# Mamo1031/Multimodal-MTRSSM

Measured on AMD Instinct MI355X. Metric: seq-steps/s (BxT) MoPoE-MRSSM train step, higher is better.
Workload: dtype bf16x2-split, fp32 accumulate; 1 GPU; BASELINE configs[1]: MoPoE-MRSSM train step, B=64/GPU T=50 deter=200 stoch=30, vision 1x64x64 + audio 1x128x32 + action 4; global_batch=64, seq_len=50, parallelism=dp1, hidden=200, embed=256, categoricals_x_classes=6x5, residual_blocks=3, activation=ELU, optimizer=AdamW lr 1e-3 + clip 10 (fused HIP), params=4151600, streams=1, launch=eager (host enqueues every launch), backend=none, rccl_ranks=0, collective_ranks=0, noise=uniforms keyed by global batch row (parallel.GlobalRowNoise)

## Files before the change

include/mtrssm.h:

```cpp
#ifndef MTRSSM_H
#define MTRSSM_H

#include <stddef.h>
#include <stdint.h>

#ifdef __cplusplus
extern "C" {
#endif

#define MTRSSM_VERSION 100

#define MTRSSM_OK 0
#define MTRSSM_EINVAL (-1)
#define MTRSSM_ELAUNCH (-2)
#define MTRSSM_ELDS (-3)

#define MTRSSM_ACT_IDENTITY 0
#define MTRSSM_ACT_RELU 1
#define MTRSSM_ACT_ELU 2
#define MTRSSM_ACT_TANH 3

int mtrssm_version(void);
const char* mtrssm_last_error(void);
const char* mtrssm_last_kernel(void);
// ... 259 lines not shown
  float* d_lpl;
  float* d_la;
  float* d_lv;
  float* d_lph;
  float* d_lqh;
  const int32_t* modality;
} MtrssmMmtrssmBwdIO;

int mtrssm_mmtrssm_rollout_bwd(const MtrssmMmtrssmDims* dims, const MtrssmMmtrssmBwdWeights* w,
                               const MtrssmMmtrssmBwdIO* io, void* stream);

int mtrssm_mmtrssm_wide_supported(const MtrssmMmtrssmDims* dims, int32_t pieces);
int64_t mtrssm_mmtrssm_wide_workspace_bytes(const MtrssmMmtrssmDims* dims, int32_t pieces);
int64_t mtrssm_mmtrssm_wide_bwd_workspace_bytes(const MtrssmMmtrssmDims* dims, int32_t pieces);
int mtrssm_mmtrssm_rollout_fwd_wide(const MtrssmMmtrssmDims* dims, const MtrssmMmtrssmFwdWeights* w, const MtrssmMmtrssmFwdIO* io,
                                    int32_t pieces, void* workspace, int64_t workspace_bytes, void* stream);
int mtrssm_mmtrssm_rollout_bwd_wide(const MtrssmMmtrssmDims* dims, const MtrssmMmtrssmBwdWeights* w, const MtrssmMmtrssmBwdIO* io,
                                    int32_t pieces, void* workspace, int64_t workspace_bytes, void* stream);

typedef struct MtrssmConvGeom {
  int32_t N;
  int32_t C, Hs, Ws;
  int32_t C2;
  int32_t Cpad;
  int32_t KH, KW;
  int32_t SS, TS, OFFY, OFFX;
  int32_t Hq, Wq;
  int32_t OS, QY, QX;
  int32_t Ho, Wo;
  int32_t Cout, CoutPad;
  int32_t pre_act;
  int32_t act;
  int32_t mfma_split;
} MtrssmConvGeom;

int mtrssm_conv_gather_gemm(const MtrssmConvGeom* g, const float* src, const float* src2, const float* wp, const uint16_t* wq,
                            const float* bias, const float* actgrad_in, const float* add_in, float* out, void* stream);
int mtrssm_conv_gather_gemm_pair(const MtrssmConvGeom* ga, const float* srca, const float* src2a, const float* wpa, const uint16_t* wqa,
                                 const float* biasa, const float* actgrada, const float* adda, float* outa,
                                 const MtrssmConvGeom* gb, const float* srcb, const float* src2b, const float* wpb, const uint16_t* wqb,
                                 const float* biasb, const float* actgradb, const float* addb, float* outb, void* stream);
int mtrssm_conv_gather_pair_merges(const MtrssmConvGeom* ga, const MtrssmConvGeom* gb, int32_t has_wq);
int mtrssm_residual_block_fwd_supported(const MtrssmConvGeom* g3);
int mtrssm_residual_block_fwd(const MtrssmConvGeom* ga, const float* xa, const uint16_t* wq3a, const float* b3a, const float* w1a,
                              const float* b1a, float* ha, float* ya, const MtrssmConvGeom* gb, const float* xb, const uint16_t* wq3b,
                              const float* b3b, const float* w1b, const float* b1b, float* hb, float* yb, void* stream);
int mtrssm_pack_conv_weight(const float* w, int32_t O, int32_t I, int32_t KH, int32_t KW, int64_t so, int64_t si, int64_t sh,
                            int64_t sw, int32_t OPad, int32_t IPad, int32_t pieces, float* wp, uint16_t* wq, void* stream);
#define MTRSSM_PACK_DESC_WORDS 16
int mtrssm_pack_conv_weights(const int64_t* table, int32_t count, int32_t blocks_per_weight, void* stream);
int mtrssm_conv_weight_grad(const MtrssmConvGeom* g, const float* a, const float* src, const float* src2,
                            int32_t pre_act_a, float* dwp, float* dbias, void* workspace, int64_t workspace_bytes, void* stream);
int mtrssm_conv_weight_grad_deferred(const MtrssmConvGeom* g, const float* a, const float* src, const float* src2,
                                     int32_t pre_act_a, float* dwp, float* dbias, void* workspace, int64_t workspace_bytes, void* stream);
int mtrssm_conv_weight_grad_reduce(void* stream);
int mtrssm_conv_weight_grad_src_bias_supported(const MtrssmConvGeom* g, int32_t pre_act_a);
int mtrssm_residual_bwd1x1_supported(const MtrssmConvGeom* g);
int mtrssm_residual_bwd1x1(const MtrssmConvGeom* g, const float* gy, const float* h, const uint16_t* wq1t, float* gh, float* dwp,
                           float* dbias, void* workspace, int64_t workspace_bytes, int32_t defer, void* stream);
int mtrssm_conv_weight_grad_src_bias(const MtrssmConvGeom* g, const float* a, const float* src, int32_t pre_act_a, float* dwp,
                                     float* dsrc_bias, void* workspace, int64_t workspace_bytes, int32_t defer, void* stream);
int64_t mtrssm_conv_weight_grad_workspace_bytes(const MtrssmConvGeom* g, int32_t pre_act_a);
int mtrssm_unpack_conv_grads(const int64_t* table, int32_t count, int32_t blocks_per_entry, void* stream);
int mtrssm_convt_quad_supported(const MtrssmConvGeom* g4);
int mtrssm_convt_quad(const MtrssmConvGeom* ga4, const float* srca, const uint16_t* const* wqa4, const float* biasa, const float* actgrada,
                      float* outa, const MtrssmConvGeom* gb4, const float* srcb, const uint16_t* const* wqb4, const float* biasb,
                      const float* actgradb, float* outb, void* stream);
int mtrssm_convt_k4s2_thin(int32_t N, int32_t C, int32_t Hs, int32_t Ws, int32_t Cout, const float* src, const float* w,
                           const float* bias, int32_t pre_act, int32_t act, float* out, void* stream);
int mtrssm_convt_k4s2_band_supported(int32_t N, int32_t C, int32_t Hs, int32_t Ws, int32_t Cout);
int mtrssm_convt_k4s2_band(int32_t N, int32_t C, int32_t Hs, int32_t Ws, int32_t Cout, const float* src, const float* w,
                           const float* bias, int32_t pre_act, int32_t act, float* out, void* stream);
int mtrssm_conv_tgather_thin(int32_t N, int32_t O, int32_t Hs, int32_t Ws, int32_t Cout, int32_t KH, int32_t KW, int32_t stride, int32_t pad,
                             int32_t Ho, int32_t Wo, const float* y, const float* w, const float* bias, int32_t pre_act, int32_t act,
                             const float* actgrad_in, const float* add_in, float* out, void* stream);
int mtrssm_channel_sum(const float* x, int32_t N, int32_t C, int32_t HW, float* out, void* stream);

int mtrssm_episode_gather(const float* store, const int64_t* idx, const float* noise, int64_t n_episodes, int64_t B, int64_t T,
                          int64_t Tfull, int64_t E, float std_, float* input, float* target, void* stream);
int mtrssm_episode_gather_window(const float* store, const int64_t* idx, const int32_t* start, const float* noise, int64_t n_episodes,
                                 int64_t B, int64_t T, int64_t Tfull, int64_t E, float std_, float* input, float* target, void* stream);
int mtrssm_episode_gather_ragged(const float* store, const int64_t* idx, const int32_t* start, const int32_t* lengths, const float* noise,
                                 int64_t n_episodes, int64_t B, int64_t T, int64_t Tfull, int64_t E, float std_, float* input, float* target,
                                 int32_t* valid_out, void* stream);
int mtrssm_episode_gather_seeded(const float* store, const int64_t* idx, const int32_t* start, const int32_t* lengths, int32_t* valid_out,
                                 uint32_t key0, uint32_t key1, uint32_t epoch, int64_t n_episodes, int64_t B, int64_t T, int64_t Tfull,
                                 int64_t E, float std_, float* input, float* target, void* stream);

#define MTRSSM_STATE_MAX 6
typedef struct MtrssmStateTable {
  int32_t count;
  int32_t width[MTRSSM_STATE_MAX];
// ... 73 lines not shown
```

multimodal_mtrssm_amd/_lib.py:

```python

from __future__ import annotations

import ctypes as C
import os
from pathlib import Path

import torch
from torch import Tensor

_HERE = Path(__file__).resolve().parent
LIB_PATH = _HERE / "libmtrssm_hip.so"

ACT_IDS = {"Identity": 0, "ReLU": 1, "ELU": 2, "Tanh": 3}

_f = C.c_float
_i = C.c_int32
_p = C.c_void_p


def _struct(name: str, fields: list[tuple[str, type]]) -> type:
    return type(name, (C.Structure,), {"_fields_": fields})


def _ptrs(*names: str) -> list[tuple[str, type]]:
# ... 14 lines not shown
    "w1s_t", "wf_t", "bf", "whh_t", "bhh", "wh1_t", "b3", "w4", "b4", "wa2", "ba2", "wv2", "bv2"))
MrssmBwdWeights = _struct("MtrssmMrssmBwdWeights", _ptrs("w1s_t", "w2", "wih", "whh", "wh1", "w4", "wa2", "wv2"))
MrssmBwdIO = _struct("MtrssmMrssmBwdIO", _ptrs(
    "deter0", "deter", "prior_logits", "post_logits", "sv_h1", "sv_h2", "sv_gates", "sv_heads", "sv_la", "sv_lv",
    "g_deter", "g_post_stoch", "g_prior_stoch", "g_post_logits", "g_prior_logits", "g_kl",
    "g_deter0", "g_stoch0", "d_z1", "d_h2", "d_gi", "d_gh", "d_zh", "d_lp", "d_la", "d_lv", "modality"))

MmtrssmDims = _struct("MtrssmMmtrssmDims", [
    ("B", _i), ("T", _i), ("LD", _i), ("HD", _i), ("H", _i), ("KL", _i), ("CL", _i), ("KH", _i), ("CH", _i),
    ("act", _i), ("post", _i), ("tau_l", _f), ("tau_h", _f), ("keep_l", _f), ("keep_h", _f),
    ("kl_w_post", _f), ("kl_w_prior", _f), ("rows_per_block", _i), ("threads", _i),
])
MmtrssmFwdWeights = _struct("MtrssmMmtrssmFwdWeights", _ptrs(
    "wxl_s_t", "wdl_t", "wxh_t", "wdh_t", "bh", "wl1_t", "bl1", "wh1_t", "bh1",
    "wlp2", "blp2", "wa2", "ba2", "wv2", "bv2", "whp2", "bhp2", "whq2", "bhq2"))
MmtrssmFwdIO = _struct("MtrssmMmtrssmFwdIO", _ptrs(
    "xl", "pa", "pv", "deter_l0", "deter_h0", "hidden_l0", "hidden_h0", "stoch_l0", "stoch_h0",
    "u_post_l", "u_post_h", "u_prior_l", "u_prior_h",
    "deter_l", "deter_h", "hidden_l", "hidden_h", "prior_logits_l", "prior_logits_h", "prior_stoch_l", "prior_stoch_h",
    "post_logits_l", "post_logits_h", "post_stoch_l", "post_stoch_h", "kl_l", "kl_h",
    "sv_l1", "sv_h1", "sv_la", "sv_lv", "modality"))
MmtrssmBwdWeights = _struct("MtrssmMmtrssmBwdWeights", _ptrs(
    "wxl_s_t", "wdl", "wxh_t", "wdh", "wl1", "wh1", "wlp2", "wa2", "wv2", "whp2", "whq2"))
MmtrssmBwdIO = _struct("MtrssmMmtrssmBwdIO", _ptrs(
    "deter_l0", "deter_h0", "deter_l", "deter_h", "prior_logits_l", "prior_logits_h", "post_logits_l", "post_logits_h",
    "sv_l1", "sv_h1", "sv_la", "sv_lv",
    "g_deter_l", "g_deter_h", "g_hidden_l", "g_hidden_h", "g_post_stoch_l", "g_post_stoch_h", "g_prior_stoch_l",
    "g_prior_stoch_h", "g_post_logits_l", "g_post_logits_h", "g_prior_logits_l", "g_prior_logits_h", "g_kl_l", "g_kl_h",
    "g_deter_l0", "g_deter_h0", "g_hidden_l0", "g_hidden_h0", "g_stoch_l0", "g_stoch_h0",
    "d_ul", "d_uh", "d_zl1", "d_zh1", "d_lpl", "d_la", "d_lv", "d_lph", "d_lqh", "modality"))

ConvGeom = _struct("MtrssmConvGeom", [(n, _i) for n in (
    "N", "C", "Hs", "Ws", "C2", "Cpad", "KH", "KW", "SS", "TS", "OFFY", "OFFX", "Hq", "Wq", "OS", "QY", "QX", "Ho", "Wo",
    "Cout", "CoutPad", "pre_act", "act", "mfma_split")])

Gemm = _struct("MtrssmGemm", _ptrs("A", "B", "C", "bias", "zgrad", "colsum") + [(n, _i) for n in (
    "M", "N", "R", "lda", "ldb", "ldc", "ldz", "a_rmajor", "b_rmajor", "act_a", "act_b", "act_out", "act_z", "accumulate", "split_r")]
    + [("tickets", _p), ("n_tickets", _i), ("mfma_split", _i)])

STATE_MAX = 6
StateTable = _struct("MtrssmStateTable", [
    ("count", _i), ("width", _i * STATE_MAX), ("src_stride", C.c_int64 * STATE_MAX), ("src", _p * STATE_MAX), ("alt", _p * STATE_MAX),
    ("dst", _p * STATE_MAX)])

SYMBOLS: dict[str, tuple[type | None, list[type]]] = {
    "mtrssm_version": (C.c_int, []),
    "mtrssm_last_error": (C.c_char_p, []),
    "mtrssm_last_kernel": (C.c_char_p, []),
    "mtrssm_mrssm_rollout_fwd": (C.c_int, [C.POINTER(MrssmDims), C.POINTER(MrssmFwdWeights), C.POINTER(MrssmFwdIO), _p]),
    "mtrssm_mrssm_cluster_supported": (C.c_int, [C.POINTER(MrssmDims)]),
    "mtrssm_mrssm_cluster_workspace_bytes": (C.c_int64, [C.POINTER(MrssmDims)]),
    "mtrssm_mrssm_rollout_fwd_cluster": (C.c_int, [C.POINTER(MrssmDims), C.POINTER(MrssmClusterWeights), C.POINTER(MrssmFwdIO), _p, C.c_int64, _p]),
    "mtrssm_mrssm_cluster_bwd_workspace_bytes": (C.c_int64, [C.POINTER(MrssmDims)]),
    "mtrssm_mrssm_rollout_bwd_cluster": (C.c_int, [C.POINTER(MrssmDims), C.POINTER(MrssmClusterWeights), C.POINTER(MrssmBwdIO), _p, C.c_int64, _p]),
    "mtrssm_mrssm_wide_supported": (C.c_int, [C.POINTER(MrssmDims), _i]),
    "mtrssm_mrssm_wide_workspace_bytes": (C.c_int64, [C.POINTER(MrssmDims), _i]),
    "mtrssm_mrssm_wide_bwd_workspace_bytes": (C.c_int64, [C.POINTER(MrssmDims), _i]),
    "mtrssm_mrssm_rollout_fwd_wide": (C.c_int, [C.POINTER(MrssmDims), C.POINTER(MrssmClusterWeights), C.POINTER(MrssmFwdIO), _i, _p, C.c_int64, _p]),
    "mtrssm_mrssm_rollout_bwd_wide": (C.c_int, [C.POINTER(MrssmDims), C.POINTER(MrssmClusterWeights), C.POINTER(MrssmBwdIO), _i, _p, C.c_int64, _p]),
    "mtrssm_mrssm_rollout_bwd": (C.c_int, [C.POINTER(MrssmDims), C.POINTER(MrssmBwdWeights), C.POINTER(MrssmBwdIO), _p]),
    "mtrssm_mmtrssm_rollout_fwd": (C.c_int, [C.POINTER(MmtrssmDims), C.POINTER(MmtrssmFwdWeights), C.POINTER(MmtrssmFwdIO), _p]),
    "mtrssm_mmtrssm_rollout_bwd": (C.c_int, [C.POINTER(MmtrssmDims), C.POINTER(MmtrssmBwdWeights), C.POINTER(MmtrssmBwdIO), _p]),
    "mtrssm_mmtrssm_wide_supported": (C.c_int, [C.POINTER(MmtrssmDims), _i]),
    "mtrssm_mmtrssm_wide_workspace_bytes": (C.c_int64, [C.POINTER(MmtrssmDims), _i]),
    "mtrssm_mmtrssm_wide_bwd_workspace_bytes": (C.c_int64, [C.POINTER(MmtrssmDims), _i]),
    "mtrssm_mmtrssm_rollout_fwd_wide": (C.c_int, [C.POINTER(MmtrssmDims), C.POINTER(MmtrssmFwdWeights), C.POINTER(MmtrssmFwdIO), _i, _p, C.c_int64, _p]),
    "mtrssm_mmtrssm_rollout_bwd_wide": (C.c_int, [C.POINTER(MmtrssmDims), C.POINTER(MmtrssmBwdWeights), C.POINTER(MmtrssmBwdIO), _i, _p, C.c_int64, _p]),
    "mtrssm_conv_gather_gemm": (C.c_int, [C.POINTER(ConvGeom), _p, _p, _p, _p, _p, _p, _p, _p, _p]),
    "mtrssm_conv_gather_gemm_pair": (C.c_int, [C.POINTER(ConvGeom), _p, _p, _p, _p, _p, _p, _p, _p,
                                               C.POINTER(ConvGeom), _p, _p, _p, _p, _p, _p, _p, _p, _p]),
    "mtrssm_conv_gather_pair_merges": (C.c_int, [C.POINTER(ConvGeom), C.POINTER(ConvGeom), _i]),
    "mtrssm_residual_block_fwd_supported": (C.c_int, [C.POINTER(ConvGeom)]),
    "mtrssm_residual_block_fwd": (C.c_int, [C.POINTER(ConvGeom), _p, _p, _p, _p, _p, _p, _p, C.POINTER(ConvGeom), _p, _p, _p, _p, _p, _p, _p, _p]),
    "mtrssm_pack_conv_weight": (C.c_int, [_p, _i, _i, _i, _i, C.c_int64, C.c_int64, C.c_int64, C.c_int64, _i, _i, _i, _p, _p, _p]),
    "mtrssm_pack_conv_weights": (C.c_int, [_p, _i, _i, _p]),
    "mtrssm_unpack_conv_grads": (C.c_int, [_p, _i, _i, _p]),
    "mtrssm_conv_weight_grad": (C.c_int, [C.POINTER(ConvGeom), _p, _p, _p, _i, _p, _p, _p, C.c_int64, _p]),
    "mtrssm_conv_weight_grad_deferred": (C.c_int, [C.POINTER(ConvGeom), _p, _p, _p, _i, _p, _p, _p, C.c_int64, _p]),
    "mtrssm_residual_bwd1x1_supported": (C.c_int, [C.POINTER(ConvGeom)]),
    "mtrssm_residual_bwd1x1": (C.c_int, [C.POINTER(ConvGeom), _p, _p, _p, _p, _p, _p, _p, C.c_int64, _i, _p]),
    "mtrssm_conv_weight_grad_src_bias_supported": (C.c_int, [C.POINTER(ConvGeom), _i]),
    "mtrssm_conv_weight_grad_src_bias": (C.c_int, [C.POINTER(ConvGeom), _p, _p, _i, _p, _p, _p, C.c_int64, _i, _p]),
    "mtrssm_conv_weight_grad_reduce": (C.c_int, [_p]),
    "mtrssm_conv_weight_grad_workspace_bytes": (C.c_int64, [C.POINTER(ConvGeom), _i]),
    "mtrssm_channel_sum": (C.c_int, [_p, _i, _i, _i, _p, _p]),
    "mtrssm_convt_k4s2_thin": (C.c_int, [_i, _i, _i, _i, _i, _p, _p, _p, _i, _i, _p, _p]),
    "mtrssm_convt_k4s2_band_supported": (C.c_int, [_i, _i, _i, _i, _i]),
    "mtrssm_convt_k4s2_band": (C.c_int, [_i, _i, _i, _i, _i, _p, _p, _p, _i, _i, _p, _p]),
    "mtrssm_convt_quad_supported": (C.c_int, [C.POINTER(ConvGeom)]),
    "mtrssm_convt_quad": (C.c_int, [C.POINTER(ConvGeom), _p, C.POINTER(C.c_void_p), _p, _p, _p, C.POINTER(ConvGeom), _p, C.POINTER(C.c_void_p),
                                    _p, _p, _p, _p]),
    "mtrssm_conv_tgather_thin": (C.c_int, [_i] * 11 + [_p, _p, _p, _i, _i, _p, _p, _p, _p]),
    "mtrssm_episode_gather": (C.c_int, [_p, _p, _p, C.c_int64, C.c_int64, C.c_int64, C.c_int64, C.c_int64, _f, _p, _p, _p]),
    "mtrssm_episode_gather_window": (C.c_int, [_p, _p, _p, _p, C.c_int64, C.c_int64, C.c_int64, C.c_int64, C.c_int64, _f, _p, _p, _p]),
    "mtrssm_state_select": (C.c_int, [C.POINTER(StateTable), _p, C.c_int64, _p]),
    "mtrssm_state_save": (C.c_int, [C.POINTER(StateTable), C.c_int64, C.c_int64, _p]),
    "mtrssm_state_save_at": (C.c_int, [C.POINTER(StateTable), _p, C.c_int64, C.c_int64, _p]),
    "mtrssm_episode_gather_ragged": (C.c_int, [_p, _p, _p, _p, _p, C.c_int64, C.c_int64, C.c_int64, C.c_int64, C.c_int64, _f, _p, _p, _p, _p]),
    "mtrssm_episode_gather_seeded": (C.c_int, [_p, _p, _p, _p, _p, C.c_uint32, C.c_uint32, C.c_uint32, C.c_int64, C.c_int64, C.c_int64, C.c_int64,
                                               C.c_int64, _f, _p, _p, _p]),
    "mtrssm_step_mask_ragged": (C.c_int, [_p, _p, C.c_int64, C.c_int64, C.c_int64, _f, _f, C.c_int64, C.c_int64, _p, _p, _p, _p, _p, _p, _p, _p]),
    "mtrssm_elbo_combine_counted_fwd": (C.c_int, [_p, _p, _p, _p, _p, _p, C.c_int64, C.c_float, C.c_float, _p, _p, _p, _p, _p]),
    "mtrssm_elbo_combine_counted_bwd": (C.c_int, [_p, _p, _p, _p, _p, _p, C.c_int64, C.c_float, C.c_float, _p, _p, _p, _p, _p]),
    "mtrssm_elbo_combine_fwd": (C.c_int, [_p, _p, _p, _p, C.c_int64, C.c_float, C.c_float, _p, _p, _p, _p, _p]),
    "mtrssm_elbo_combine_bwd": (C.c_int, [_p, _p, _p, _p, C.c_int64, C.c_float, C.c_float, _p, _p, _p, _p, _p]),
    "mtrssm_categorical_sample_fwd": (C.c_int, [_p, _p, C.c_int64, _i, _i, _p, _p, _p, _p]),
    "mtrssm_categorical_sample_bwd": (C.c_int, [_p, _p, _p, C.c_int64, _i, _i, _p, _p]),
    "mtrssm_gaussian_nll_fwd": (C.c_int, [_p, _p, C.c_int64, C.c_int64, _i, _p, _p]),
    "mtrssm_gaussian_nll_bwd": (C.c_int, [_p, _p, _p, C.c_int64, C.c_int64, _i, _p, _p]),
    "mtrssm_gaussian_nll_masked_fwd": (C.c_int, [_p, _p, _p, _p, C.c_int64, C.c_int64, _i, _p, _p]),
    "mtrssm_gaussian_nll_masked_bwd": (C.c_int, [_p, _p, _p, _p, _p, C.c_int64, C.c_int64, _i, _p, _p]),
    "mtrssm_modality_dropout": (C.c_int, [_p, C.c_int64, C.c_int64, C.c_int64, _f, _f, C.c_int64, C.c_int64, _p, _p, _p, _p, _p, _p]),
    "mtrssm_sumsq": (C.c_int, [_p, C.c_int64, _p, _p]),
# ... 128 lines not shown
```

multimodal_mtrssm_amd/conv.py:

```python

from __future__ import annotations

import ctypes as C
import os
import weakref

import torch
from torch import Tensor

from multimodal_mtrssm_amd import _lib
from multimodal_mtrssm_amd.linear import grad_target, grad_target_owner


def _pad_to(n: int, m: int) -> int:
    return (n + m - 1) // m * m


def _pads(cout: int, cin: int) -> tuple[int, int]:
    return _pad_to(cout, 64 if cout > 32 else 32), _pad_to(cin, 16)


_PACK_BUFFERS: dict[tuple, tuple[Tensor, Tensor | None]] = {}

PAIR_LAUNCH = os.environ.get("MTRSSM_PAIR_LAUNCH", "1") != "0"
# ... 130 lines not shown
def gemm_pieces() -> int:
    return {0: 0, 3: 3, 2: 2, 1: 2}[_MFMA_SPLIT]


def _geom(**kw: int) -> C.Structure:
    g = _lib.ConvGeom()
    for k, v in kw.items():
        setattr(g, k, int(v))
    g.mfma_split = _MFMA_SPLIT
    return g


def _gather_gemm(geom: C.Structure, src: Tensor, src2: Tensor | None, wpq: tuple[Tensor, Tensor | None], bias: Tensor | None,
                 actgrad_in: Tensor | None, out: Tensor, add_in: Tensor | None = None) -> None:
    wp, wq = wpq
    lib = _lib.load()
    job = (geom, src, src2, wp, wq, bias, actgrad_in, add_in, out)
    if _DEFER is not None:
        _DEFER.append(job)
        return
    _launch_gather(job)


def _job_work(job: tuple) -> tuple[float, float]:
    geom, actgrad_in, add_in = job[0], job[6], job[7]
    pixels = geom.N * geom.Hq * geom.Wq
    flops = 2.0 * pixels * geom.Cout * geom.KH * geom.KW * (geom.C + geom.C2)
    nbytes = 4.0 * (geom.N * geom.C * geom.Hs * geom.Ws + pixels * geom.Cout * (1 + (actgrad_in is not None) + (add_in is not None)))
    return flops, nbytes


def _job_args(job: tuple) -> tuple:
    geom, src, src2, wp, wq, bias, actgrad_in, add_in, out = job
    return (C.byref(geom), _lib.ptr(src), _lib.ptr(src2), _lib.ptr(wp), _lib.raw_ptr(wq), _lib.ptr(bias), _lib.ptr(actgrad_in),
            _lib.ptr(add_in), _lib.ptr(out))


def _quad_args(job: tuple) -> tuple:
    _, geoms, y, wqs, bias, out, actgrad = job
    arr = (C.c_void_p * 4)(*[_lib.raw_ptr(wq) for wq in wqs])
    return (geoms, _lib.ptr(y), arr, _lib.ptr(bias), _lib.ptr(actgrad), _lib.ptr(out))


def _quad_work(job: tuple) -> tuple[float, float]:
    g = job[1][0]
    pixels = g.N * g.Ho * g.Wo
    return 2.0 * pixels * g.Cout * 4 * g.C, 4.0 * (g.N * g.C * g.Hs * g.Ws + pixels * g.Cout * (2 if job[6] is not None else 1))


def _launch_quad(ja: tuple, jb: tuple | None) -> None:
    lib = _lib.load()
    fa, ba = _quad_work(ja)
    fb, bb = _quad_work(jb) if jb is not None else (0.0, 0.0)
    args_b = _quad_args(jb) if jb is not None else (None, None, None, None, None, None)
    _lib.check(_lib.TIMERS.call("mtrssm_convt_quad", lib.mtrssm_convt_quad, *_quad_args(ja), *args_b, _lib.stream_ptr(ja[2].device),
                                flops=fa + fb, nbytes=ba + bb), "mtrssm_convt_quad")


def _launch_gather(job: tuple) -> None:
    if job[0] == "quad":
        _launch_quad(job, None)
        return
    lib = _lib.load()
    flops, nbytes = _job_work(job)
    _lib.check(_lib.TIMERS.call("mtrssm_conv_gather_gemm", lib.mtrssm_conv_gather_gemm, *_job_args(job),
                                _lib.stream_ptr(job[1].device), flops=flops, nbytes=nbytes), "mtrssm_conv_gather_gemm")

# ... 25 lines not shown
                _launch_gather(jb)
            continue
        if not lib.mtrssm_conv_gather_pair_merges(C.byref(ja[0]), C.byref(jb[0]), int(ja[4] is not None and jb[4] is not None)):
            _launch_gather(ja)
            _launch_gather(jb)
            continue
        fa, ba = _job_work(ja)
        fb, bb = _job_work(jb)
        _lib.check(_lib.TIMERS.call("mtrssm_conv_gather_gemm_pair", lib.mtrssm_conv_gather_gemm_pair, *_job_args(ja), *_job_args(jb),
                                    _lib.stream_ptr(ja[1].device), flops=fa + fb, nbytes=ba + bb), "mtrssm_conv_gather_gemm_pair")
    return ra, rb


def _conv_forward_gather(x: Tensor, coords: Tensor | None, w: Tensor, bias: Tensor | None, stride: int, pad: int,
                         pre_act: bool, act: int, actgrad_in: Tensor | None = None, add_in: Tensor | None = None) -> Tensor:
    n, c, hs, ws = x.shape
    o, i, kh, kw = w.shape
    c2 = 0 if coords is None else coords.shape[0]
    if i != c + c2:
        msg = f"weight expects {i} input channels, got {c}+{c2}"
        raise ValueError(msg)
    ho = (hs + 2 * pad - kh) // stride + 1
    wo = (ws + 2 * pad - kw) // stride + 1
    wpq = pack_weight(w)
    wp = wpq[0]
    out = torch.empty(n, o, ho, wo, device=x.device, dtype=torch.float32)
    geom = _geom(N=n, C=c, Hs=hs, Ws=ws, C2=c2, Cpad=wp.shape[2], KH=kh, KW=kw, SS=stride, TS=1, OFFY=-pad, OFFX=-pad,
                 Hq=ho, Wq=wo, OS=1, QY=0, QX=0, Ho=ho, Wo=wo, Cout=o, CoutPad=wp.shape[0], pre_act=int(pre_act), act=act)
    _gather_gemm(geom, x, coords, wpq, bias, actgrad_in, out, add_in)
    return out


def _conv_transposed_gather(y: Tensor, w: Tensor, bias: Tensor | None, stride: int, pad: int, out_hw: tuple[int, int],
                            pre_act: bool, act: int, actgrad_in: Tensor | None = None, add_in: Tensor | None = None) -> Tensor:
    n, o, hs, ws = y.shape
    o2, c, kh, kw = w.shape
    if o2 != o:
        msg = f"weight expects {o2} gathered channels, got {o}"
        raise ValueError(msg)
    ho, wo = out_hw
    out = torch.empty(n, c, ho, wo, device=y.device, dtype=torch.float32)
    if (stride == 2 and kh == 4 and kw == 4 and pad == 1 and c <= 2 and (ho, wo) == (2 * hs, 2 * ws) and actgrad_in is None
            and add_in is None and o * ((8 + 2) * (32 + 2) + 1) * 4 <= 64 * 1024):
        lib = _lib.load()
        wc = w.contiguous()
        if _MFMA_SPLIT == 2 and CONVT_BAND and lib.mtrssm_convt_k4s2_band_supported(n, o, hs, ws, c):
            _lib.check(_lib.TIMERS.call(
                "mtrssm_convt_k4s2_band", lib.mtrssm_convt_k4s2_band, n, o, hs, ws, c, _lib.ptr(y), _lib.ptr(wc), _lib.ptr(bias),
                int(pre_act), act, _lib.ptr(out), _lib.stream_ptr(y.device), flops=2.0 * n * ho * wo * c * 4 * o,
                nbytes=4.0 * (y.numel() + out.numel())), "mtrssm_convt_k4s2_band")
            return out
        _lib.check(_lib.TIMERS.call(
            "mtrssm_convt_k4s2_thin", lib.mtrssm_convt_k4s2_thin, n, o, hs, ws, c, _lib.ptr(y), _lib.ptr(wc), _lib.ptr(bias),
            int(pre_act), act, _lib.ptr(out), _lib.stream_ptr(y.device), flops=2.0 * n * ho * wo * c * 4 * o,
            nbytes=4.0 * (y.numel() + out.numel())), "mtrssm_convt_k4s2_thin")
        return out
    quad_fwd = kh == 4 and kw == 4 and actgrad_in is None and (o, c, hs * ws) in ((64, 32, 64), (32, 16, 256))
    quad_bwd = (CONVT_QUAD_BWD and kh == 3 and kw == 3 and actgrad_in is not None and bias is None
                and (o, c, hs * ws) in ((32, 16, 64), (16, 8, 256)))
    if (stride == 2 and pad == 1 and (ho, wo) == (2 * hs, 2 * ws) and add_in is None and _MFMA_SPLIT == 2 and CONVT_QUAD
            and (quad_fwd or quad_bwd)):
        geoms = (_lib.ConvGeom * 4)()
        wqs = []
        for q in range(4):
            qy, qx = q >> 1, q & 1
            ky0, kx0 = (qy + pad) % stride, (qx + pad) % stride
            wsub = w[:, :, ky0::stride, kx0::stride].permute(1, 0, 2, 3)
            wp, wq = pack_weight(wsub, sub=q, grid=(2, 2))
            geoms[q] = _geom(N=n, C=o, Hs=hs, Ws=ws, C2=0, Cpad=wp.shape[2], KH=2, KW=2, SS=1, TS=-1,
                             OFFY=(qy + pad - ky0) // stride, OFFX=(qx + pad - kx0) // stride, Hq=hs, Wq=ws, OS=stride, QY=qy, QX=qx,
                             Ho=ho, Wo=wo, Cout=c, CoutPad=wp.shape[0], pre_act=int(pre_act), act=act)
            wqs.append(wq)
        if _lib.load().mtrssm_convt_quad_supported(geoms):
            job = ("quad", geoms, y, wqs, bias, out, actgrad_in)
            if _DEFER is not None:
                _DEFER.append(job)
            else:
                _launch_gather(job)
            return out
    if stride == 2 and c <= 8 and kh * kw * o <= 256 and ho % 2 == 0 and wo % 2 == 0 and TGATHER_THIN:
        lib = _lib.load()
        wc = w.contiguous()
        taps_used = kh * kw / (stride * stride)
        _lib.check(_lib.TIMERS.call(
            "mtrssm_conv_tgather_thin", lib.mtrssm_conv_tgather_thin, n, o, hs, ws, c, kh, kw, stride, pad, ho, wo, _lib.ptr(y),
            _lib.ptr(wc), _lib.ptr(bias), int(pre_act), act, _lib.ptr(actgrad_in), _lib.ptr(add_in), _lib.ptr(out),
            _lib.stream_ptr(y.device), flops=2.0 * n * ho * wo * c * taps_used * o,
            nbytes=4.0 * (y.numel() + out.numel() * (1 + (actgrad_in is not None) + (add_in is not None)))), "mtrssm_conv_tgather_thin")
        return out
    for qy in range(min(stride, ho)):
        ky0 = (qy + pad) % stride
        for qx in range(min(stride, wo)):
            kx0 = (qx + pad) % stride
            wsub = w[:, :, ky0::stride, kx0::stride].permute(1, 0, 2, 3)
            wpq = pack_weight(wsub)
            wp = wpq[0]
            geom = _geom(N=n, C=o, Hs=hs, Ws=ws, C2=0, Cpad=wp.shape[2], KH=wsub.shape[2], KW=wsub.shape[3], SS=1, TS=-1,
                         OFFY=(qy + pad - ky0) // stride, OFFX=(qx + pad - kx0) // stride,
                         Hq=(ho - qy + stride - 1) // stride, Wq=(wo - qx + stride - 1) // stride, OS=stride, QY=qy, QX=qx,
                         Ho=ho, Wo=wo, Cout=c, CoutPad=wp.shape[0], pre_act=int(pre_act), act=act)
            _gather_gemm(geom, y, None, wpq, bias, actgrad_in, out, add_in)
    return out


TGATHER_THIN = os.environ.get("MTRSSM_TGATHER_THIN", "1") != "0"
CONVT_QUAD = os.environ.get("MTRSSM_CONVT_QUAD", "1") != "0"
CONVT_QUAD_BWD = os.environ.get("MTRSSM_CONVT_QUAD_BWD", "1") != "0"
CONVT_BAND = os.environ.get("MTRSSM_CONVT_BAND", "1") != "0"
_ZERO_CHUNK_FLOATS = 2 << 20
_ZERO_CHUNKS: dict[tuple, list] = {}


def _zeros(n: int, device: torch.device) -> Tensor:
    need = (n + 63) // 64 * 64
    key = (device, torch.cuda.current_stream(device).cuda_stream if device.type == "cuda" else 0)
    st = _ZERO_CHUNKS.get(key)
    if st is None or st[1] + need > st[0].numel():
        st = _ZERO_CHUNKS[key] = [torch.zeros(max(_ZERO_CHUNK_FLOATS, need), device=device, dtype=torch.float32), 0]
    out = st[0][st[1] : st[1] + n]
    st[1] += need
    return out


class _ConvGradSink:

    def __init__(self) -> None:
        self.entries: dict[tuple, tuple] = {}
        self.table: Tensor | None = None
        self.retired: list[Tensor] = []
        self.pending = False

    def target(self, weight: Tensor | None, o: int, i: int, taps: int, opad: int, ipad: int) -> Tensor | None:
        if weight is None or not weight.is_contiguous():
# ... 78 lines not shown
            _WGRAD_SLOT_NEXT[(device, stream)] = 0
            _lib.check(_lib.TIMERS.call("mtrssm_conv_weight_grad_reduce", _lib.load().mtrssm_conv_weight_grad_reduce, C.c_void_p(stream)),
                       "mtrssm_conv_weight_grad_reduce")


def _wgrad_workspace(geom: C.Structure, pre_act_a: int, device: torch.device, *, own: bool = False) -> Tensor | None:
    gkey = (tuple(getattr(geom, n) for n, _ in geom._fields_), pre_act_a)
    need = _WGRAD_NEED.get(gkey)
    if need is None:
        need = _WGRAD_NEED[gkey] = max(0, int(_lib.load().mtrssm_conv_weight_grad_workspace_bytes(C.byref(geom), pre_act_a)))
    if need == 0:
        return None
    key = (device, torch.cuda.current_stream(device).cuda_stream)
    if own:
        slots = _WGRAD_SLOTS.setdefault(key, [])
        k = _WGRAD_SLOT_NEXT.get(key, 0)
        _WGRAD_SLOT_NEXT[key] = k + 1
        if k == len(slots):
            slots.append(torch.empty((need + 3) // 4 + 64, device=device, dtype=torch.float32))
        elif slots[k].numel() * 4 < need:
            _WGRAD_WS_RETIRED.append(slots[k])
            slots[k] = torch.empty((need + 3) // 4 + 64, device=device, dtype=torch.float32)
        return slots[k]
    ws = _WGRAD_WS.get(key)
    if ws is None or ws.numel() * 4 < need:
        if ws is not None:
            _WGRAD_WS_RETIRED.append(ws)
        ws = _WGRAD_WS[key] = torch.empty((need + 3) // 4 + 64, device=device, dtype=torch.float32)
    return ws


def _weight_grad(a: Tensor, src: Tensor, coords: Tensor | None, kh: int, kw: int, stride: int, pad: int, pre_act_a: bool,
                 pre_act_src: bool, act: int, *, want_bias: bool = False, weight: Tensor | None = None,
                 bias: Tensor | None = None, want_src_bias: bool = False) -> tuple[Tensor | None, Tensor | None]:
    lib = _lib.load()
    n, o, hq, wq = a.shape
    _, c, hs, ws = src.shape
    c2 = 0 if coords is None else coords.shape[0]
    opad, ipad = _pads(o, c + c2)
    sunk = _GRAD_SINK.target(weight, o, c + c2, kh * kw, opad, ipad)
    dwp = sunk if sunk is not None else _zeros(opad * kh * kw * ipad, a.device).view(opad, kh * kw, ipad)
    fuse_src_bias = want_src_bias and CONVT_BIAS_FUSE and coords is None and a.data_ptr() % 16 == 0 and src.data_ptr() % 16 == 0
    dbias = bias_sunk = None
    if want_bias or fuse_src_bias:
        bias_sunk = grad_target(bias) if bias is not None and bias.is_contiguous() else None
    geom = _geom(N=n, C=c, Hs=hs, Ws=ws, C2=c2, Cpad=ipad, KH=kh, KW=kw, SS=stride, TS=1, OFFY=-pad, OFFX=-pad, Hq=hq, Wq=wq,
                 OS=1, QY=0, QX=0, Ho=hq, Wo=wq, Cout=o, CoutPad=opad, pre_act=int(pre_act_src), act=act)
    flops = 2.0 * n * hq * wq * o * kh * kw * (c + c2)
    nbytes = 4.0 * (a.numel() + src.numel())
    fuse_src_bias = fuse_src_bias and bool(lib.mtrssm_conv_weight_grad_src_bias_supported(C.byref(geom), int(pre_act_a)))
    if want_bias or fuse_src_bias:
        dbias = bias_sunk if bias_sunk is not None else _zeros(c if fuse_src_bias else o, a.device)
    defer = DEFER_WGRAD_REDUCE and sunk is not None and (dbias is None or bias_sunk is not None)
    ws = _wgrad_workspace(geom, int(pre_act_a), a.device, own=defer)
    if fuse_src_bias:
        _lib.check(_lib.TIMERS.call(
            "mtrssm_conv_weight_grad", lib.mtrssm_conv_weight_grad_src_bias, C.byref(geom), _lib.ptr(a), _lib.ptr(src), int(pre_act_a),
            _lib.ptr(dwp), _lib.ptr(dbias), _lib.raw_ptr(ws), 0 if ws is None else ws.numel() * 4, int(defer and ws is not None),
            _lib.stream_ptr(a.device), flops=flops, nbytes=nbytes), "mtrssm_conv_weight_grad_src_bias")
        g_w = None if sunk is not None else dwp[:o, :, : c + c2].reshape(o, kh, kw, c + c2).permute(0, 3, 1, 2)
        return g_w, (None if bias_sunk is not None else dbias)
    entry = lib.mtrssm_conv_weight_grad_deferred if defer and ws is not None else lib.mtrssm_conv_weight_grad
    _lib.check(_lib.TIMERS.call(
        "mtrssm_conv_weight_grad", entry, C.byref(geom), _lib.ptr(a), _lib.ptr(src), _lib.ptr(coords),
        int(pre_act_a), _lib.ptr(dwp), _lib.ptr(dbias), _lib.raw_ptr(ws), 0 if ws is None else ws.numel() * 4, _lib.stream_ptr(a.device),
        flops=flops, nbytes=nbytes), "mtrssm_conv_weight_grad")
    g_w = None if sunk is not None else dwp[:o, :, : c + c2].reshape(o, kh, kw, c + c2).permute(0, 3, 1, 2)
    if want_src_bias:
        return g_w, _channel_sum(src, bias)
    return g_w, (None if bias_sunk is not None else dbias)


def _channel_sum(x: Tensor, bias: Tensor | None = None) -> Tensor | None:
    lib = _lib.load()
    n, c, h, w = x.shape
    sunk = grad_target(bias) if bias is not None and bias.is_contiguous() else None
    out = sunk if sunk is not None else _zeros(c, x.device)
    _lib.check(_lib.TIMERS.call("mtrssm_channel_sum", lib.mtrssm_channel_sum, _lib.ptr(x), n, c, h * w, _lib.ptr(out),
                                _lib.stream_ptr(x.device)), "mtrssm_channel_sum")
    return None if sunk is not None else out


class _Conv2d(torch.autograd.Function):
    @staticmethod
    def forward(ctx, x, weight, bias, coords, stride, pad, pre_act, act):
        x, weight = x.contiguous(), weight.contiguous()
        bias = None if bias is None else bias.contiguous()
        coords = None if coords is None else coords.contiguous()
        out = _conv_forward_gather(x, coords, weight, bias, stride, pad, pre_act, act)
        ctx.save_for_backward(x, weight, coords if coords is not None else x.new_zeros(0))
        ctx.cfg = (stride, pad, pre_act, act, coords is not None, bias is not None)
        ctx.bias = bias
        return out

    @staticmethod
    def backward(ctx, g_out):
        x, weight, coords = ctx.saved_tensors
# ... 74 lines not shown
        g = job[0]
        pixels = g.N * g.Hq * g.Wq
        return 2.0 * pixels * g.Cout * (9 * g.C + g.C), 4.0 * pixels * (2 * g.C + g.Cout)

    def args(job: tuple | None) -> tuple:
        if job is None:
            return (None,) * 8
        geom, x, wq, b3, w1, b1, h, y = job
        return (C.byref(geom), _lib.ptr(x), _lib.raw_ptr(wq), _lib.ptr(b3), _lib.ptr(w1), _lib.ptr(b1), _lib.ptr(h), _lib.ptr(y))

    fa, ba = work(ja)
    fb, bb = work(jb) if jb is not None else (0.0, 0.0)
    lib = _lib.load()
    _lib.check(_lib.TIMERS.call("mtrssm_residual_block_fwd", lib.mtrssm_residual_block_fwd, *args(ja), *args(jb),
                                _lib.stream_ptr(ja[1].device), flops=fa + fb, nbytes=ba + bb), "mtrssm_residual_block_fwd")


RESBLOCK_BWD1X1_FUSE = True


def _bwd1x1_geom(g_y: Tensor, h: Tensor, w1: Tensor, act: int) -> C.Structure | None:
    if not RESBLOCK_BWD1X1_FUSE or _MFMA_SPLIT != 2 or w1.shape[2:] != (1, 1) or not g_y.is_cuda:
        return None
    n, o, hq, wq = g_y.shape
    c = h.shape[1]
    if w1.shape[:2] != (o, c) or h.shape != (n, c, hq, wq) or g_y.data_ptr() % 16 or h.data_ptr() % 16:
        return None
    opad, ipad = _pads(o, c)
    geom = _geom(N=n, C=c, Hs=hq, Ws=wq, C2=0, Cpad=ipad, KH=1, KW=1, SS=1, TS=1, OFFY=0, OFFX=0, Hq=hq, Wq=wq, OS=1, QY=0, QX=0,
                 Ho=hq, Wo=wq, Cout=o, CoutPad=opad, pre_act=1, act=act)
    return geom if _lib.load().mtrssm_residual_bwd1x1_supported(C.byref(geom)) else None


def _bwd1x1_fused(geom: C.Structure, g_y: Tensor, h: Tensor, w1: Tensor, b1: Tensor) -> tuple[Tensor, Tensor | None, Tensor | None]:
    lib = _lib.load()
    n, o, hq, wq = g_y.shape
    c = h.shape[1]
    _, wq1t = pack_weight(w1.permute(1, 0, 2, 3))
    sunk = _GRAD_SINK.target(w1, o, c, 1, geom.CoutPad, geom.Cpad)
    dwp = sunk if sunk is not None else _zeros(geom.CoutPad * geom.Cpad, g_y.device).view(geom.CoutPad, 1, geom.Cpad)
    bias_sunk = grad_target(b1) if b1.is_contiguous() else None
    dbias = bias_sunk if bias_sunk is not None else _zeros(o, g_y.device)
    defer = DEFER_WGRAD_REDUCE and sunk is not None and bias_sunk is not None
    ws = _wgrad_workspace(geom, 0, g_y.device, own=defer)
    g_h = torch.empty_like(h)
    pixels = n * hq * wq
    _lib.check(_lib.TIMERS.call(
        "mtrssm_residual_bwd1x1", lib.mtrssm_residual_bwd1x1, C.byref(geom), _lib.ptr(g_y), _lib.ptr(h), _lib.raw_ptr(wq1t), _lib.ptr(g_h),
        _lib.ptr(dwp), _lib.ptr(dbias), _lib.raw_ptr(ws), 0 if ws is None else ws.numel() * 4, int(defer and ws is not None),
        _lib.stream_ptr(g_y.device), flops=2.0 * 2.0 * pixels * o * c, nbytes=4.0 * (g_y.numel() + 2 * h.numel())), "mtrssm_residual_bwd1x1")
    g_w = None if sunk is not None else dwp[:o, :, :c].reshape(o, 1, 1, c).permute(0, 3, 1, 2)
    return g_h, g_w, (None if bias_sunk is not None else dbias)


class _ResidualBlock(torch.autograd.Function):

    @staticmethod
    def forward(ctx, x, w3, b3, w1, b1, act):
        x, w3, b3, w1, b1 = (t.contiguous() for t in (x, w3, b3, w1, b1))
        p3, p1 = w3.shape[2] // 2, w1.shape[2] // 2
        job = _residual_job(x, w3, b3, w1, b1, act)
        if job is not None:
            _residual_launch(job, None)
            h, y = job[6], job[7]
        else:
            h = _conv_forward_gather(x, None, w3, b3, 1, p3, True, act)
            y = _conv_forward_gather(h, None, w1, b1, 1, p1, True, act, add_in=x)
        ctx.save_for_backward(x, h, w3, w1)
        ctx.act, ctx.biases = act, (b3, b1)
        return y

    @staticmethod
    def backward(ctx, g_y):
        x, h, w3, w1 = ctx.saved_tensors
        act = ctx.act
        g_y = g_y.contiguous()
        p3, p1 = w3.shape[2] // 2, w1.shape[2] // 2
        b3, b1 = ctx.biases
        g1 = _bwd1x1_geom(g_y, h, w1, act)
        if g1 is not None:
            g_h, g_w1, g_b1 = _bwd1x1_fused(g1, g_y, h, w1, b1)
        else:
            g_h = _conv_transposed_gather(g_y, w1, None, 1, p1, (h.shape[2], h.shape[3]), False, act, actgrad_in=h)
            g_w1, g_b1 = _weight_grad(g_y, h, None, w1.shape[2], w1.shape[3], 1, p1, False, True, act, want_bias=True, weight=w1, bias=b1)
        g_x = None
        if ctx.needs_input_grad[0]:
            g_x = _conv_transposed_gather(g_h, w3, None, 1, p3, (x.shape[2], x.shape[3]), False, act, actgrad_in=x, add_in=g_y)
        g_w3, g_b3 = _weight_grad(g_h, x, None, w3.shape[2], w3.shape[3], 1, p3, False, True, act, want_bias=True, weight=w3, bias=b3)
        return g_x, g_w3, g_b3, g_w1, g_b1, None


class _PairResidualBlock(torch.autograd.Function):

    @staticmethod
    def forward(ctx, xa, w3a, b3a, w1a, b1a, xv, w3v, b3v, w1v, b1v, act):
        xa, w3a, b3a, w1a, b1a, xv, w3v, b3v, w1v, b1v = (t.contiguous() for t in (xa, w3a, b3a, w1a, b1a, xv, w3v, b3v, w1v, b1v))
        p3, p1 = w3a.shape[2] // 2, w1a.shape[2] // 2
        ja = _residual_job(xa, w3a, b3a, w1a, b1a, act)
        jv = _residual_job(xv, w3v, b3v, w1v, b1v, act, sub=1) if ja is not None else None
        if ja is not None and jv is not None:
            _residual_launch(ja, jv)
            ha, ya, hv, yv = ja[6], ja[7], jv[6], jv[7]
        else:
            ha, hv = paired(lambda: _conv_forward_gather(xa, None, w3a, b3a, 1, p3, True, act),
                            lambda: _conv_forward_gather(xv, None, w3v, b3v, 1, p3, True, act))
            ya, yv = paired(lambda: _conv_forward_gather(ha, None, w1a, b1a, 1, p1, True, act, add_in=xa),
                            lambda: _conv_forward_gather(hv, None, w1v, b1v, 1, p1, True, act, add_in=xv))
        ctx.save_for_backward(xa, ha, w3a, w1a, xv, hv, w3v, w1v)
        ctx.act, ctx.biases = act, (b3a, b1a, b3v, b1v)
        return ya, yv

    @staticmethod
    def backward(ctx, g_ya, g_yv):
        xa, ha, w3a, w1a, xv, hv, w3v, w1v = ctx.saved_tensors
        act = ctx.act
        g_ya, g_yv = g_ya.contiguous(), g_yv.contiguous()
        p3, p1 = w3a.shape[2] // 2, w1a.shape[2] // 2
        b3a, b1a, b3v, b1v = ctx.biases
        g1a = _bwd1x1_geom(g_ya, ha, w1a, act)
        g1v = _bwd1x1_geom(g_yv, hv, w1v, act) if g1a is not None else None
        if g1a is not None and g1v is not None:
            g_ha, g_w1a, g_b1a = _bwd1x1_fused(g1a, g_ya, ha, w1a, b1a)
            g_hv, g_w1v, g_b1v = _bwd1x1_fused(g1v, g_yv, hv, w1v, b1v)
        else:
            g_ha, g_hv = paired(lambda: _conv_transposed_gather(g_ya, w1a, None, 1, p1, (ha.shape[2], ha.shape[3]), False, act, actgrad_in=ha),
                                lambda: _conv_transposed_gather(g_yv, w1v, None, 1, p1, (hv.shape[2], hv.shape[3]), False, act, actgrad_in=hv))
            g_w1a, g_b1a = _weight_grad(g_ya, ha, None, w1a.shape[2], w1a.shape[3], 1, p1, False, True, act, want_bias=True, weight=w1a, bias=b1a)
            g_w1v, g_b1v = _weight_grad(g_yv, hv, None, w1v.shape[2], w1v.shape[3], 1, p1, False, True, act, want_bias=True, weight=w1v, bias=b1v)
        g_xa, g_xv = paired(
            lambda: _conv_transposed_gather(g_ha, w3a, None, 1, p3, (xa.shape[2], xa.shape[3]), False, act, actgrad_in=xa, add_in=g_ya),
            lambda: _conv_transposed_gather(g_hv, w3v, None, 1, p3, (xv.shape[2], xv.shape[3]), False, act, actgrad_in=xv, add_in=g_yv))
        g_w3a, g_b3a = _weight_grad(g_ha, xa, None, w3a.shape[2], w3a.shape[3], 1, p3, False, True, act, want_bias=True, weight=w3a, bias=b3a)
        g_w3v, g_b3v = _weight_grad(g_hv, xv, None, w3v.shape[2], w3v.shape[3], 1, p3, False, True, act, want_bias=True, weight=w3v, bias=b3v)
        return g_xa, g_w3a, g_b3a, g_w1a, g_b1a, g_xv, g_w3v, g_b3v, g_w1v, g_b1v, None


def residual_block_pair(xa: Tensor, pa: tuple[Tensor, Tensor, Tensor, Tensor], xv: Tensor, pv: tuple[Tensor, Tensor, Tensor, Tensor],
                        *, act: int) -> tuple[Tensor, Tensor]:
    return _PairResidualBlock.apply(xa, *pa, xv, *pv, int(act))


def residual_block(x: Tensor, w3: Tensor, b3: Tensor, w1: Tensor, b1: Tensor, *, act: int) -> Tensor:
    return _ResidualBlock.apply(x, w3, b3, w1, b1, int(act))


class _BranchCtx:

    def __init__(self, needs: tuple = ()) -> None:
        self.needs_input_grad = needs
        self.saved_tensors: tuple = ()
        self.cfg: tuple = ()

    def save_for_backward(self, *tensors: Tensor) -> None:
        self.saved_tensors = tensors


def _pair_function(base: type) -> type:

    class _Pair(torch.autograd.Function):
        @staticmethod
        def forward(ctx, n, *args):
            ca, cb = _BranchCtx(), _BranchCtx()
            ya, yb = paired(lambda: base.forward(ca, *args[:n]), lambda: base.forward(cb, *args[n:]))
            ctx.n, ctx.na, ctx.cfgs = n, len(ca.saved_tensors), (ca.cfg, cb.cfg)
            ctx.biases = (getattr(ca, "bias", None), getattr(cb, "bias", None))
            ctx.save_for_backward(*ca.saved_tensors, *cb.saved_tensors)
# ... 41 lines not shown
```

multimodal_mtrssm_amd/csrc/capi.hip:

```cpp
#include <stdarg.h>
#include <stdio.h>

#include "scan_common.h"

namespace mtrssm {

static thread_local char g_err[512] = "";
static thread_local const char* g_kernel = "";

void set_last_kernel(const char* name) { g_kernel = name; }

void set_error(const char* fmt, ...) {
  va_list ap;
  va_start(ap, fmt);
  vsnprintf(g_err, sizeof(g_err), fmt, ap);
  va_end(ap);
}

int mrssm_fwd_launch(const MtrssmMrssmDims*, const MtrssmMrssmFwdWeights*, const MtrssmMrssmFwdIO*, hipStream_t);
int mrssm_bwd_launch(const MtrssmMrssmDims*, const MtrssmMrssmBwdWeights*, const MtrssmMrssmBwdIO*, hipStream_t);
int mmtrssm_fwd_launch(const MtrssmMmtrssmDims*, const MtrssmMmtrssmFwdWeights*, const MtrssmMmtrssmFwdIO*, hipStream_t);
int mmtrssm_bwd_launch(const MtrssmMmtrssmDims*, const MtrssmMmtrssmBwdWeights*, const MtrssmMmtrssmBwdIO*, hipStream_t);
int conv_gather_gemm_launch(const MtrssmConvGeom*, const float*, const float*, const float*, const unsigned short*, const float*, const float*, const float*, float*, hipStream_t);
int episode_gather_launch(const float*, const int64_t*, const float*, int64_t, int64_t, int64_t, int64_t, int64_t, float, float*, float*, hipStream_t);
int episode_gather_window_launch(const float*, const int64_t*, const int32_t*, const float*, int64_t, int64_t, int64_t, int64_t, int64_t, float, float*,
                                 float*, hipStream_t);
int state_select_launch(const MtrssmStateTable*, const unsigned char*, int64_t, hipStream_t);
int state_save_launch(const MtrssmStateTable*, int64_t, int64_t, hipStream_t);
int state_save_at_launch(const MtrssmStateTable*, const int32_t*, int64_t, int64_t, hipStream_t);
int episode_gather_ragged_launch(const float*, const int64_t*, const int32_t*, const int32_t*, const float*, int64_t, int64_t, int64_t, int64_t,
                                 int64_t, float, float*, float*, int32_t*, hipStream_t);
int episode_gather_seeded_launch(const float*, const int64_t*, const int32_t*, const int32_t*, int32_t*, uint32_t, uint32_t, uint32_t, int64_t, int64_t,
                                 int64_t, int64_t, int64_t, float, float*, float*, hipStream_t);
int step_mask_ragged_launch(const int32_t*, const float*, int64_t, int64_t, int64_t, float, float, int64_t, int64_t, int32_t*, float*, float*, float*,
                            unsigned char*, int32_t*, float*, hipStream_t);
int elbo_combine_counted_fwd_launch(const float*, const float*, const float*, const float*, const float*, const float*, int64_t, float, float, float*,
                                    float*, float*, float*, hipStream_t);
int elbo_combine_counted_bwd_launch(const float*, const float*, const float*, const float*, const float*, const float*, int64_t, float, float, float*,
                                    float*, float*, float*, hipStream_t);
int conv_gather_gemm_pair_launch(const MtrssmConvGeom*, const float*, const float*, const float*, const unsigned short*, const float*, const float*, const float*, float*,
                                 const MtrssmConvGeom*, const float*, const float*, const float*, const unsigned short*, const float*, const float*, const float*, float*, hipStream_t);
int conv_residual_fwd_supported(const MtrssmConvGeom*);
int conv_residual_fwd_launch(const MtrssmConvGeom*, const float*, const unsigned short*, const float*, const float*, const float*, float*, float*,
                             const MtrssmConvGeom*, const float*, const unsigned short*, const float*, const float*, const float*, float*, float*, hipStream_t);
int pack_conv_weight_launch(const float*, int, int, int, int, long, long, long, long, int, int, int, float*, unsigned short*, hipStream_t);
int pack_conv_weights_launch(const int64_t*, int, int, hipStream_t);
int conv_gather_pair_merges(const MtrssmConvGeom*, const MtrssmConvGeom*, bool);
int conv_weight_grad_launch(const MtrssmConvGeom*, const float*, const float*, const float*, int, float*, float*, void*, size_t, size_t*, hipStream_t);
int conv_weight_grad_deferred_launch(const MtrssmConvGeom*, const float*, const float*, const float*, int, float*, float*, void*, size_t, hipStream_t);
int conv_weight_grad_reduce_flush(hipStream_t);
int conv_residual_bwd1x1_supported(const MtrssmConvGeom*);
int conv_residual_bwd1x1_launch(const MtrssmConvGeom*, const float*, const float*, const unsigned short*, float*, float*, float*, void*, size_t, int,
                                hipStream_t);
int conv_weight_grad_src_bias_supported(const MtrssmConvGeom*, int);
int conv_weight_grad_src_bias_launch(const MtrssmConvGeom*, const float*, const float*, int, float*, float*, void*, size_t, int, hipStream_t);
int channel_sum_launch(const float*, int, int, int, float*, hipStream_t);
int convt_k4s2_band_supported(int, int, int, int, int);
int convt_k4s2_band_launch(int, int, int, int, int, const float*, const float*, const float*, int, int, float*, hipStream_t);
int convt_k4s2_thin_launch(int, int, int, int, int, const float*, const float*, const float*, int, int, float*, hipStream_t);
int conv_convt_quad_supported(const MtrssmConvGeom*);
int conv_convt_quad_launch(const MtrssmConvGeom*, const float*, const unsigned short* const*, const float*, const float*, float*,
                           const MtrssmConvGeom*, const float*, const unsigned short* const*, const float*, const float*, float*, hipStream_t);
int conv_tgather_thin_launch(int, int, int, int, int, int, int, int, int, int, int, const float*, const float*, const float*, int, int, const float*,
                             const float*, float*, hipStream_t);
int categorical_sample_fwd_launch(const float*, const float*, int64_t, int, int, float*, float*, float*, hipStream_t);
int categorical_sample_bwd_launch(const float*, const float*, const float*, int64_t, int, int, float*, hipStream_t);
int elbo_combine_fwd_launch(const float*, const float*, const float*, const float*, int64_t, float, float, float*, float*, float*, float*, hipStream_t);
int elbo_combine_bwd_launch(const float*, const float*, const float*, const float*, int64_t, float, float, float*, float*, float*, float*, hipStream_t);
int nll_fwd_launch(const float*, const float*, int64_t, int64_t, int, float*, hipStream_t);
int nll_bwd_launch(const float*, const float*, const float*, int64_t, int64_t, int, float*, hipStream_t);
int nll_masked_fwd_launch(const float*, const float*, const float*, const float*, int64_t, int64_t, int, float*, hipStream_t);
int nll_masked_bwd_launch(const float*, const float*, const float*, const float*, const float*, int64_t, int64_t, int, float*, hipStream_t);
int modality_dropout_launch(const float*, int64_t, int64_t, int64_t, float, float, int64_t, int64_t, int32_t*, float*, float*, unsigned char*, float*,
                            hipStream_t);
int sumsq_launch(const float*, int64_t, float*, hipStream_t);
int adamw_launch(float*, const float*, float*, float*, int64_t, const float*, float, float, float, float, float, float, float, int, hipStream_t);
int gemm_launch(const MtrssmGemm*, hipStream_t);
int gemm_group_launch(const MtrssmGemm*, int, hipStream_t);
int debug_set_cluster_profile(void*);
int debug_set_resident_profile(void*);
int debug_set_wide_profile(void*);
int debug_set_mmt_profile(void*);
int mrssm_cluster_supported(const MtrssmMrssmDims*);
size_t mrssm_cluster_workspace_bytes(const MtrssmMrssmDims*);
size_t mrssm_cluster_bwd_workspace_bytes(const MtrssmMrssmDims*);
// ... 212 lines not shown
                                            const float* biasb, const float* actgradb, const float* addb, float* outb, void* stream) {
  return conv_gather_gemm_pair_launch(ga, srca, src2a, wpa, wqa, biasa, actgrada, adda, outa, gb, srcb, src2b, wpb, wqb, biasb, actgradb, addb,
                                      outb, static_cast<hipStream_t>(stream));
}
MTRSSM_API int mtrssm_residual_block_fwd_supported(const MtrssmConvGeom* g3) { return conv_residual_fwd_supported(g3) != 0; }
MTRSSM_API int mtrssm_residual_block_fwd(const MtrssmConvGeom* ga, const float* xa, const uint16_t* wq3a, const float* b3a, const float* w1a,
                                         const float* b1a, float* ha, float* ya, const MtrssmConvGeom* gb, const float* xb, const uint16_t* wq3b,
                                         const float* b3b, const float* w1b, const float* b1b, float* hb, float* yb, void* stream) {
  return conv_residual_fwd_launch(ga, xa, wq3a, b3a, w1a, b1a, ha, ya, gb, xb, wq3b, b3b, w1b, b1b, hb, yb, static_cast<hipStream_t>(stream));
}
MTRSSM_API int mtrssm_pack_conv_weight(const float* w, int32_t O, int32_t I, int32_t KH, int32_t KW, int64_t so, int64_t si, int64_t sh,
                                       int64_t sw, int32_t OPad, int32_t IPad, int32_t pieces, float* wp, uint16_t* wq, void* stream) {
  return pack_conv_weight_launch(w, O, I, KH, KW, so, si, sh, sw, OPad, IPad, pieces, wp, wq, static_cast<hipStream_t>(stream));
}
MTRSSM_API int mtrssm_conv_gather_pair_merges(const MtrssmConvGeom* ga, const MtrssmConvGeom* gb, int32_t has_wq) {
  return conv_gather_pair_merges(ga, gb, has_wq != 0);
}
MTRSSM_API int mtrssm_pack_conv_weights(const int64_t* table, int32_t count, int32_t blocks_per_weight, void* stream) {
  return pack_conv_weights_launch(table, count, blocks_per_weight, static_cast<hipStream_t>(stream));
}
MTRSSM_API int mtrssm_conv_weight_grad(const MtrssmConvGeom* g, const float* a, const float* src, const float* src2, int32_t pre_act_a,
                                       float* dwp, float* dbias, void* workspace, int64_t workspace_bytes, void* stream) {
  return conv_weight_grad_launch(g, a, src, src2, pre_act_a, dwp, dbias, workspace, workspace_bytes < 0 ? 0 : (size_t)workspace_bytes, nullptr,
                                 static_cast<hipStream_t>(stream));
}
MTRSSM_API int mtrssm_conv_weight_grad_deferred(const MtrssmConvGeom* g, const float* a, const float* src, const float* src2, int32_t pre_act_a,
                                               float* dwp, float* dbias, void* workspace, int64_t workspace_bytes, void* stream) {
  return conv_weight_grad_deferred_launch(g, a, src, src2, pre_act_a, dwp, dbias, workspace, workspace_bytes < 0 ? 0 : (size_t)workspace_bytes,
                                          static_cast<hipStream_t>(stream));
}
MTRSSM_API int mtrssm_residual_bwd1x1_supported(const MtrssmConvGeom* g) { return conv_residual_bwd1x1_supported(g) != 0; }
MTRSSM_API int mtrssm_residual_bwd1x1(const MtrssmConvGeom* g, const float* gy, const float* h, const uint16_t* wq1t, float* gh, float* dwp,
                                      float* dbias, void* workspace, int64_t workspace_bytes, int32_t defer, void* stream) {
  return conv_residual_bwd1x1_launch(g, gy, h, wq1t, gh, dwp, dbias, workspace, workspace_bytes < 0 ? 0 : (size_t)workspace_bytes, defer,
                                     static_cast<hipStream_t>(stream));
}
MTRSSM_API int mtrssm_conv_weight_grad_src_bias_supported(const MtrssmConvGeom* g, int32_t pre_act_a) {
  return conv_weight_grad_src_bias_supported(g, pre_act_a);
}
MTRSSM_API int mtrssm_conv_weight_grad_src_bias(const MtrssmConvGeom* g, const float* a, const float* src, int32_t pre_act_a, float* dwp,
                                                float* dsrc_bias, void* workspace, int64_t workspace_bytes, int32_t defer, void* stream) {
  return conv_weight_grad_src_bias_launch(g, a, src, pre_act_a, dwp, dsrc_bias, workspace, workspace_bytes < 0 ? 0 : (size_t)workspace_bytes,
                                          defer, static_cast<hipStream_t>(stream));
}
MTRSSM_API int mtrssm_conv_weight_grad_reduce(void* stream) { return conv_weight_grad_reduce_flush(static_cast<hipStream_t>(stream)); }
MTRSSM_API int64_t mtrssm_conv_weight_grad_workspace_bytes(const MtrssmConvGeom* g, int32_t pre_act_a) {
  size_t need = 0;
  if (conv_weight_grad_launch(g, nullptr, nullptr, nullptr, pre_act_a, nullptr, nullptr, nullptr, 0, &need, nullptr) != MTRSSM_OK) return -1;
  return (int64_t)need;
}
MTRSSM_API int mtrssm_channel_sum(const float* x, int32_t N, int32_t C, int32_t HW, float* out, void* stream) {
  return channel_sum_launch(x, N, C, HW, out, static_cast<hipStream_t>(stream));
}
MTRSSM_API int mtrssm_conv_tgather_thin(int32_t N, int32_t O, int32_t Hs, int32_t Ws, int32_t Cout, int32_t KH, int32_t KW, int32_t stride,
                                        int32_t pad, int32_t Ho, int32_t Wo, const float* y, const float* w, const float* bias, int32_t pre_act,
                                        int32_t act, const float* actgrad_in, const float* add_in, float* out, void* stream) {
  return conv_tgather_thin_launch(N, O, Hs, Ws, Cout, KH, KW, stride, pad, Ho, Wo, y, w, bias, pre_act, act, actgrad_in, add_in, out,
                                  static_cast<hipStream_t>(stream));
}
MTRSSM_API int mtrssm_convt_quad_supported(const MtrssmConvGeom* g4) { return conv_convt_quad_supported(g4); }
MTRSSM_API int mtrssm_convt_quad(const MtrssmConvGeom* ga4, const float* srca, const uint16_t* const* wqa4, const float* biasa,
                                 const float* actgrada, float* outa, const MtrssmConvGeom* gb4, const float* srcb,
                                 const uint16_t* const* wqb4, const float* biasb, const float* actgradb, float* outb, void* stream) {
  return conv_convt_quad_launch(ga4, srca, reinterpret_cast<const unsigned short* const*>(wqa4), biasa, actgrada, outa, gb4, srcb,
                                reinterpret_cast<const unsigned short* const*>(wqb4), biasb, actgradb, outb,
                                static_cast<hipStream_t>(stream));
}
MTRSSM_API int mtrssm_convt_k4s2_band_supported(int32_t N, int32_t C, int32_t Hs, int32_t Ws, int32_t Cout) {
  return convt_k4s2_band_supported(N, C, Hs, Ws, Cout);
// ... 10 lines not shown
```

multimodal_mtrssm_amd/csrc/conv.hip:

```cpp
#include <map>
#include <mutex>
#include <unordered_map>
#include <utility>

#include "scan_common.h"

namespace mtrssm {

void set_error(const char* fmt, ...);
void set_last_kernel(const char* name);

using f32x16 = __attribute__((ext_vector_type(16))) float;

constexpr int kKC = 16;
constexpr int kTP = 128;
constexpr int kConvThreads = 256;

__device__ __forceinline__ float act_grad_from_in(float x, int act) {
  switch (act) {
    case MTRSSM_ACT_RELU: return x > 0.f ? 1.f : 0.f;
    case MTRSSM_ACT_ELU: return x > 0.f ? 1.f : expf(x);
    case MTRSSM_ACT_TANH: { const float t = tanhf(x); return 1.f - t * t; }
    default: return 1.f;
  }
// ... 538 lines not shown
      const size_t base = (size_t)n * g.Cout * plane_o + (size_t)(oy * g.OS + g.QY) * g.Wo + (ox * g.OS + g.QX);
#pragma unroll
      for (int j = 0; j < NT; ++j) {
#pragma unroll
        for (int r = 0; r < 16; ++r) {
          const int co = co0 + j * 32 + (r & 3) + 8 * (r >> 2) + 4 * kl;
          if (co < g.Cout) {
            float v = acc[i][j][r] + (bias ? bias[co] : 0.f);
            const size_t o = base + (size_t)co * plane_o;
            if (actgrad_in) v *= act_grad_from_in(actgrad_in[o], g.act);
            if (add_in) v += add_in[o];
            out[o] = v;
          }
        }
      }
    }
  }
}

}
#include "conv_split.h"
#include "conv_resident.h"
#include "conv_s2_band.h"
#include "conv_wgrad_resident.h"

namespace mtrssm {

static int launched(const char* who);
enum ReduceVariant { kRedRes64, kRedRes32, kRed1x1_64, kRed1x1_128, kRedThin, kRedThinT, kRedS2, kRedT4, kRedT4b, kRedS2c };
struct ReduceJob {
  const float4* part;
  float* dwp;
  float* dbias;
  int S, cpad, variant, gx, gy;
  __host__ int variant_gy() const { return gy; }
};
constexpr int kReduceBatchMax = 48;
struct ReduceBatch {
  int count;
  int first[kReduceBatchMax + 1];
  ReduceJob job[kReduceBatchMax];
};
__device__ __forceinline__ void wgrad_reduce_dispatch(const ReduceJob& j, int bx, int by) {
  switch (j.variant) {
    case kRedRes64: wgrad_reduce_partials_body<64>(j.part, j.S, j.cpad, j.dwp, j.dbias, bx, by); break;
    case kRedRes32: wgrad_reduce_partials_body<32>(j.part, j.S, j.cpad, j.dwp, j.dbias, bx, by); break;
    case kRed1x1_64: wgrad_reduce_partials1x1_body<64>(j.part, j.S, j.cpad, j.dwp, j.dbias, bx, by); break;
    case kRed1x1_128: wgrad_reduce_partials1x1_body<128>(j.part, j.S, j.cpad, j.dwp, j.dbias, bx, by); break;
    case kRedThin: wgrad_reduce_partials_thin_body(j.part, j.S, j.cpad, j.dwp, j.dbias, bx, by); break;
    case kRedThinT: wgrad_reduce_partials_thint_body(j.part, j.S, j.cpad, j.dwp, j.dbias, bx, by); break;
    case kRedS2: wgrad_reduce_partials_s2_body(j.part, j.S, j.cpad, j.dwp, j.dbias, bx, by); break;
    case kRedT4: wgrad_reduce_partials_t4_body(j.part, j.S, j.cpad, j.dwp, j.dbias, bx, by); break;
    case kRedT4b: wgrad_reduce_partials_t4b_body(j.part, j.S, j.cpad, j.dwp, j.dbias, bx, by); break;
    default: wgrad_reduce_partials_s2c_body(j.part, j.S, j.cpad, j.dwp, j.dbias, bx, by); break;
  }
}
__global__ __launch_bounds__(256) void wgrad_reduce_batch_kernel(const ReduceBatch b) {
  int j = 0;
  while (j + 1 < b.count && (int)blockIdx.x >= b.first[j + 1]) ++j;
  const int lb = (int)blockIdx.x - b.first[j], gx = b.job[j].gx;
  wgrad_reduce_dispatch(b.job[j], lb % gx, lb / gx);
}

static thread_local bool tl_defer_reduce = false;
static std::mutex g_reduce_mutex;
static std::map<std::pair<int, hipStream_t>, std::vector<ReduceJob>> g_reduce_jobs;
static std::pair<int, hipStream_t> reduce_key(hipStream_t stream) {
  int dev = 0;
  (void)hipGetDevice(&dev);
  return {dev, stream};
}

static int reduce_flush_locked(std::vector<ReduceJob>& jobs, hipStream_t stream) {
  size_t at = 0;
  while (at < jobs.size()) {
    ReduceBatch b{};
    int blocks = 0;
    while (at < jobs.size() && b.count < kReduceBatchMax) {
      b.first[b.count] = blocks;
      b.job[b.count] = jobs[at];
      blocks += jobs[at].gx * jobs[at].variant_gy();
      ++b.count;
      ++at;
    }
    b.first[b.count] = blocks;
    set_last_kernel("mtrssm::wgrad_reduce_batch_kernel");
    hipLaunchKernelGGL(wgrad_reduce_batch_kernel, dim3((unsigned)blocks), dim3(256), 0, stream, b);
  }
  jobs.clear();
  return launched("conv_weight_grad_reduce");
}

int conv_weight_grad_reduce_flush(hipStream_t stream) {
  std::lock_guard<std::mutex> lock(g_reduce_mutex);
  auto it = g_reduce_jobs.find(reduce_key(stream));
  if (it == g_reduce_jobs.end() || it->second.empty()) return MTRSSM_OK;
  return reduce_flush_locked(it->second, stream);
}

static int reduce_now_or_later(int variant, dim3 rgrid, const float* part, int S, int cpad, float* dwp, float* dbias, hipStream_t stream) {
  ReduceJob j{reinterpret_cast<const float4*>(part), dwp, dbias, S, cpad, variant, (int)rgrid.x, (int)rgrid.y};
  if (tl_defer_reduce) {
    std::lock_guard<std::mutex> lock(g_reduce_mutex);
    auto& jobs = g_reduce_jobs[reduce_key(stream)];
    for (const ReduceJob& o : jobs)
      if (o.dwp == dwp || o.part == j.part) {
        if (int rc = reduce_flush_locked(jobs, stream)) return rc;
        break;
      }
    jobs.push_back(j);
    return MTRSSM_OK;
  }
  ReduceBatch b{};
  b.count = 1;
  b.first[0] = 0;
  b.first[1] = (int)(rgrid.x * rgrid.y);
  b.job[0] = j;
  hipLaunchKernelGGL(wgrad_reduce_batch_kernel, dim3(rgrid.x * rgrid.y), dim3(256), 0, stream, b);
  return MTRSSM_OK;
}

}
namespace mtrssm {

constexpr int kThinMaxK = 256;

template <int COT>
__global__ __launch_bounds__(kConvThreads) void conv_gather_thin_kernel(
    const MtrssmConvGeom g, const float* __restrict__ src, const float* __restrict__ src2, const float* __restrict__ wp,
    const float* __restrict__ bias, const float* __restrict__ actgrad_in, const float* __restrict__ add_in, float* __restrict__ out) {
  __shared__ __attribute__((aligned(16))) float w_lds[kThinMaxK * COT];
  const int tid = threadIdx.x;
  const int taps = g.KH * g.KW, ctot = g.C + g.C2;
  const int K = taps * ctot;
// ... 461 lines not shown
  if ((threadIdx.x & 63) == 0) red[threadIdx.x >> 6] = acc;
  __syncthreads();
  if (threadIdx.x == 0) atomicAdd(&out[c], red[0] + red[1] + red[2] + red[3]);
}

static bool plane_fits_26bit(const MtrssmConvGeom* g) { return (long)g->Hs * g->Ws < (1L << 26); }

static int check_geom(const MtrssmConvGeom* g, const char* who) {
  if (!g || g->N <= 0 || g->C <= 0 || g->Hs <= 0 || g->Ws <= 0 || g->C2 < 0 || g->KH < 0 || g->KW < 0 || g->Hq <= 0 || g->Wq <= 0 ||
      g->Ho <= 0 || g->Wo <= 0 || g->Cout <= 0 || g->OS <= 0) {
    set_error("%s: bad geometry", who);
    return MTRSSM_EINVAL;
  }
  if (g->Cpad % kKC || g->Cpad < g->C + g->C2 || g->CoutPad % 32 || g->CoutPad < g->Cout) {
    set_error("%s: Cpad must be a multiple of 16 covering C+C2, CoutPad a multiple of 32 covering Cout", who);
    return MTRSSM_EINVAL;
  }
  if ((g->Hq - 1) * g->OS + g->QY >= g->Ho || (g->Wq - 1) * g->OS + g->QX >= g->Wo || g->QY < 0 || g->QX < 0) {
    set_error("%s: output sub-grid exceeds the output plane", who);
    return MTRSSM_EINVAL;
  }
  if (g->Cout > 32 && g->CoutPad % 64) {
    set_error("%s: CoutPad must be a multiple of 64 when Cout > 32", who);
    return MTRSSM_EINVAL;
  }
  if (g->act < MTRSSM_ACT_IDENTITY || g->act > MTRSSM_ACT_TANH) {
    set_error("%s: unknown activation id %d", who, g->act);
    return MTRSSM_EINVAL;
  }
  if (g->mfma_split < 0 || g->mfma_split > 3) {
    set_error("%s: mfma_split must be 0 (fp32 MFMA) or 1..3 bf16 pieces, got %d", who, g->mfma_split);
    return MTRSSM_EINVAL;
  }
  return MTRSSM_OK;
}

static int launched(const char* who) {
  hipError_t e = hipGetLastError();
  if (e != hipSuccess) {
    set_error("%s launch failed: %s", who, hipGetErrorString(e));
    return MTRSSM_ELAUNCH;
  }
  return MTRSSM_OK;
}

struct SplitPlan {
  int kind = 0;
  int tco = 0, ny = 0, nx = 0, sp = 0, pit = 0, tgs = 0, ngroups = 0;
  int res = 0;
  int stream = 0;
  size_t lds = 0;
  bool same_kernel(const SplitPlan& o) const {
    if (kind == 3) return o.kind == 3 && res == o.res;
    return kind == o.kind && kind != 0 && tco == o.tco && ny == o.ny && sp == o.sp && pit == o.pit && tgs == o.tgs && ngroups == o.ngroups;
  }
};

static bool resident_enabled() {
  static const bool on = [] { const char* e = getenv("MTRSSM_CONV_RESIDENT"); return !(e && e[0] == '0'); }();
  return on;
}

static bool patch_limit_768() {
  static const bool on = [] { const char* e = getenv("MTRSSM_PATCH_768"); return !(e && e[0] == '0'); }();
  return on;
}

static int device_slot() {
  int dev = 0;
  (void)hipGetDevice(&dev);
  return dev & 63;
}

static int cu_count() {
  static const int n = [] {
    int dev = 0, v = 0;
    if (hipGetDevice(&dev) != hipSuccess || hipDeviceGetAttribute(&v, hipDeviceAttributeMultiprocessorCount, dev) != hipSuccess || v <= 0) v = 256;
    return v;
  }();
  return n;
}

static SplitPlan plan_split(const MtrssmConvGeom* g, bool has_wq) {
  SplitPlan pl;
  if (!(g->mfma_split > 0 && has_wq) || !((g->TS == 1 || g->TS == -1) && g->KH * g->KW > 0 && plane_fits_26bit(g))) return pl;
  if (g->Wq > kTP || kTP % g->Wq) return pl;
  const PatchGeom pg(*g, kTP);
  const bool tiles = (g->Hq % pg.rpg == 0) || (pg.rpg % g->Hq == 0);
  if (!tiles || pg.ipg >= 32) return pl;
  const long ptot = (long)g->N * g->Hq * g->Wq;
  const int sp = g->mfma_split, taps = g->KH * g->KW;
  pl.tco = g->Cout > 32 ? 64 : 32;
  pl.ny = g->CoutPad / pl.tco;
  pl.nx = (int)((ptot + kTP - 1) / kTP);
  pl.sp = sp;
  if ((long)g->N * g->Cout * g->Ho * g->Wo >= (1L << 31)) return pl;
  if (sp == 2 && resident_enabled() && g->KH == 3 && g->KW == 3 && g->SS == 1 && g->OS == 1 && g->QY == 0 && g->QX == 0 && g->C2 == 0 &&
      (g->Ws == 4 || g->Ws == 8 || g->Ws == 16) && g->Hs * g->Ws == 64 && g->Hq == g->Hs && g->Wq == g->Ws && g->Ho == g->Hs && g->Wo == g->Ws && g->Cpad == g->C && g->OFFY == -g->TS &&
      g->OFFX == -g->TS && (long)g->N * g->C * 64 < (1L << 31) && g->act != MTRSSM_ACT_TANH) {
    const int key = g->C * 1000 + g->Cout;
    const int fpt = key == 64064 || key == 32064 || key == 64032 ? 2 : 1;
    if ((key == 64064 || key == 64128 || key == 128064 || key == 32064 || key == 64032) && g->N % fpt == 0) {
      pl.kind = 3;
      pl.res = key;
      pl.nx = g->N;
      pl.lds = key == 64032 ? res_lds_bytes<64, 1, 2>() : key == 64064 ? res_lds_bytes<64, 2, 1>() : key == 64128 ? res_lds_bytes<64, 4, 1>() : key == 128064 ? res_lds_bytes<128, 2, 2>()
                                                                                                     : res_lds_bytes<32, 2, 1>();
      return pl;
    }
  }
  if (taps == 1 && g->SS == 1 && g->OS == 1 && g->OFFY == 0 && g->OFFX == 0 && g->C2 == 0 && g->Hs == g->Hq && g->Ws == g->Wq &&
      g->Ho == g->Hq && g->Wo == g->Wq && g->Cpad % 64 == 0) {
    pl.kind = 1;
    pl.lds = (size_t)sp * (kTP + pl.tco) * 128;
    const int key = g->C * 1000 + g->Cout;
    if (sp == 2 && resident_enabled() && (key == 64064 || key == 128064 || key == 64128) && g->Cpad == g->C && g->CoutPad == g->Cout &&
        (g->Hq * g->Wq) % 32 == 0 && g->act != MTRSSM_ACT_TANH && (long)g->N * g->C * g->Hq * g->Wq < (1L << 31))
      pl.stream = key;
    return pl;
  }
  auto lds_of = [&](int t) { return (size_t)sp * ((size_t)pg.ps_raw * kRowB + (size_t)t * pl.tco * kRowB); };
  int tgs = 1;
  for (int t = 1; t <= split_tg(sp) && t <= taps; ++t)
    if (taps % t == 0 && lds_of(t) <= 80 * 1024) tgs = t;
  pl.tgs = tgs;
  pl.ngroups = taps / tgs;
  pl.lds = lds_of(tgs);
  pl.pit = pg.ps_raw <= 384 ? 3 : 6;
  if (pl.lds <= 80 * 1024 && pg.ps_raw <= (patch_limit_768() ? 768 : 640) && (long)pg.ipg * g->C * g->Hs * g->Ws < (1L << 31) &&
      (long)sp * g->CoutPad * taps * g->Cpad < (1L << 31))
    pl.kind = 2;
  return pl;
}

static GatherProblem make_problem(const MtrssmConvGeom* g, const SplitPlan& pl, const float* src, const float* src2, const unsigned short* wq,
                                  const float* bias, const float* actgrad_in, const float* add_in, float* out) {
  GatherProblem p;
  p.g = *g; p.src = src; p.src2 = src2; p.wq = wq; p.bias = bias; p.actgrad_in = actgrad_in; p.add_in = add_in; p.out = out;
  p.tg = pl.tgs; p.ngroups = pl.ngroups; p.nx = pl.nx;
  return p;
}

static int launch_split(const SplitPlan& pl, size_t lds, const GatherProblem& pa, const GatherProblem& pb, hipStream_t stream) {
  if (pl.kind == 3) {
    const bool epi_a = pa.actgrad_in || pa.add_in, epi_b = pb.actgrad_in || pb.add_in;
    if (pb.nx > 0 && epi_a != epi_b) {
      GatherProblem none{};
      none.nx = 0;
      if (int rc = launch_split(pl, lds, pa, none, stream)) return rc;
      return launch_split(pl, lds, pb, none, stream);
    }
    const int fpt = pl.res == 64064 || pl.res == 32064 || pl.res == 64032 ? 2 : 1;
    const long ta = (pa.nx + fpt - 1) / fpt, tb = (pb.nx + fpt - 1) / fpt;
    const int ncu = cu_count();
    GatherProblem qa = pa, qb = pb;
    if (tb == 0) {
      qa.nx = (int)(ta < ncu ? ta : ncu);
      qb.nx = 0;
    } else {
      long na = (ncu * ta + (ta + tb) / 2) / (ta + tb);
      na = na < 1 ? 1 : (na > ncu - 1 ? ncu - 1 : na);
      qa.nx = (int)(na < ta ? na : ta);
      qb.nx = (int)(ncu - na < tb ? ncu - na : tb);
    }
    const dim3 rgrid((unsigned)(qa.nx + qb.nx));
#define MTRSSM_RES_LAUNCH_E(CIN_, NCT_, KS_, EPI_)                                                                   \
  {                                                                                                                   \
    static bool attr_done_dev[64] = {}; bool& attr_done = attr_done_dev[device_slot()];                                                                                    \
    const size_t rl = res_lds_bytes<CIN_, NCT_, KS_>();                                                               \
    if (!attr_done) {                                                                                                 \
      (void)hipFuncSetAttribute(reinterpret_cast<const void*>(conv3x3_resident_kernel<CIN_, NCT_, KS_, EPI_>),        \
                                hipFuncAttributeMaxDynamicSharedMemorySize, (int)rl);                                 \
      attr_done = true;                                                                                               \
    }                                                                                                                 \
    set_last_kernel("mtrssm::conv3x3_resident_kernel<" #CIN_ ", " #NCT_ ", " #KS_ ", " #EPI_ ">");                      \
    hipLaunchKernelGGL((conv3x3_resident_kernel<CIN_, NCT_, KS_, EPI_>), rgrid, dim3(kResThreads), rl, stream, qa, qb); \
    return launched("conv_gather_gemm(resident)");                                                                    \
  }
#define MTRSSM_RES_LAUNCH(CIN_, NCT_, KS_) \
  { if (epi_a) MTRSSM_RES_LAUNCH_E(CIN_, NCT_, KS_, true) else MTRSSM_RES_LAUNCH_E(CIN_, NCT_, KS_, false) }
    if (pl.res == 64064) MTRSSM_RES_LAUNCH(64, 2, 1)
    if (pl.res == 64128) MTRSSM_RES_LAUNCH(64, 4, 1)
    if (pl.res == 128064) MTRSSM_RES_LAUNCH(128, 2, 2)
    if (pl.res == 32064) MTRSSM_RES_LAUNCH(32, 2, 1)
    if (pl.res == 64032) MTRSSM_RES_LAUNCH(64, 1, 2)
#undef MTRSSM_RES_LAUNCH_E
#undef MTRSSM_RES_LAUNCH
    set_error("conv_gather_gemm: no resident kernel for this plan");
    return MTRSSM_EINVAL;
  }
  if (pl.kind == 1 && pl.stream != 0) {
    auto dir = [](const GatherProblem& q) { return q.add_in && !q.actgrad_in ? 1 : (q.actgrad_in && !q.add_in && !q.bias ? 2 : 0); };
    const int da = dir(pa), db = pb.nx > 0 ? dir(pb) : da;
    const bool same_shape = pb.nx == 0 || (pb.g.C == pa.g.C && pb.g.Cout == pa.g.Cout);
    if (da != 0 && da == db && same_shape) {
      const long ta = (long)pa.g.N * (pa.g.Hq * pa.g.Wq / 32), tb = pb.nx > 0 ? (long)pb.g.N * (pb.g.Hq * pb.g.Wq / 32) : 0;
      const long wa = (ta + 3) / 4, wb = (tb + 3) / 4;
      const int ncu = cu_count();
      GatherProblem qa = pa, qb = pb;
      if (tb == 0) {
        qa.nx = (int)(wa < ncu ? wa : ncu);
        qb.nx = 0;
      } else {
        long na = (ncu * ta + (ta + tb) / 2) / (ta + tb);
        na = na < 1 ? 1 : (na > ncu - 1 ? ncu - 1 : na);
        qa.nx = (int)(na < wa ? na : wa);
        qb.nx = (int)(ncu - na < wb ? ncu - na : wb);
      }
      const dim3 sgrid((unsigned)(qa.nx + qb.nx));
#define MTRSSM_STREAM_LAUNCH(CIN_, COUT_, FWD_)                                                                      \
  {                                                                                                                   \
    set_last_kernel("mtrssm::conv1x1_stream_kernel<" #CIN_ ", " #COUT_ ", " #FWD_ ">");                                \
    hipLaunchKernelGGL((conv1x1_stream_kernel<CIN_, COUT_, FWD_>), sgrid, dim3(kResThreads), 0, stream, qa, qb);      \
// ... 136 lines not shown
    qa.nx = (int)(ta < slots ? ta : slots);
    qb.nx = 0;
  } else {
    long na = (slots * ta + (ta + tb) / 2) / (ta + tb);
    na = na < 1 ? 1 : (na > slots - 1 ? slots - 1 : na);
    qa.nx = (int)(na < ta ? na : ta);
    qb.nx = (int)(slots - na < tb ? slots - na : tb);
  }
  const int kind = s2k4_band_covers(&pa.g, true, false);
  const int oct = pa.g.C / 8;
  auto lds_of = [&](const MtrssmConvGeom& q) { return 2 * oct * ((q.Hs + 2) * (q.Ws + 2) + 1) * 16; };
  const int la = lds_of(pa.g), lb = pb ? lds_of(pb->g) : 0;
  const size_t lds = (size_t)(la > lb ? la : lb);
  static bool attr_done_dev[64][2] = {};
  bool& attr_done = attr_done_dev[device_slot()][kind - 1];
  if (kind == 1) {
    if (!attr_done) {
      (void)hipFuncSetAttribute(reinterpret_cast<const void*>(conv4s2_band_kernel<16, 32, 1024>), hipFuncAttributeMaxDynamicSharedMemorySize, 80 * 1024);
      attr_done = true;
    }
    set_last_kernel("mtrssm::conv4s2_band_kernel<16, 32, 1024>");
    hipLaunchKernelGGL((conv4s2_band_kernel<16, 32, 1024>), dim3((unsigned)(qa.nx + qb.nx)), dim3(512), lds, stream, qa, qb);
  } else {
    if (!attr_done) {
      (void)hipFuncSetAttribute(reinterpret_cast<const void*>(conv4s2_band_kernel<32, 64, 256>), hipFuncAttributeMaxDynamicSharedMemorySize, 80 * 1024);
      attr_done = true;
    }
    set_last_kernel("mtrssm::conv4s2_band_kernel<32, 64, 256>");
    hipLaunchKernelGGL((conv4s2_band_kernel<32, 64, 256>), dim3((unsigned)(qa.nx + qb.nx)), dim3(256), lds, stream, qa, qb);
  }
  return launched("conv_gather_gemm(s2 k4 band)");
}

int conv_gather_gemm_launch(const MtrssmConvGeom* g, const float* src, const float* src2, const float* wp, const unsigned short* wq,
                            const float* bias, const float* actgrad_in, const float* add_in, float* out, hipStream_t stream) {
  if (int rc = check_geom(g, "conv_gather_gemm")) return rc;
  if (!src || !wp || !out || (g->C2 > 0 && !src2)) { set_error("conv_gather_gemm: null pointer"); return MTRSSM_EINVAL; }
  if ((uintptr_t)wp & 15) { set_error("conv_gather_gemm: packed weights must be 16-byte aligned"); return MTRSSM_EINVAL; }
  const long ptot = (long)g->N * g->Hq * g->Wq;
  if (s2_band_covers(g, wq != nullptr, actgrad_in || add_in)) {
    GatherProblem p{};
    p.g = *g; p.src = src; p.src2 = src2; p.wq = wq; p.bias = bias; p.out = out;
    return launch_s2_band(p, nullptr, stream);
  }
  if (s2k4_band_covers(g, wq != nullptr, add_in != nullptr)) {
    GatherProblem p{};
    p.g = *g; p.src = src; p.wq = wq; p.bias = bias; p.actgrad_in = actgrad_in; p.out = out;
    return launch_s2k4_band(p, nullptr, stream);
  }
  static const bool thin16_pairs = [] { const char* e = getenv("MTRSSM_THIN16_PAIRS"); return !(e && e[0] == '0'); }();
  if (thin16_pairs && g->C == 1 && g->C2 == 0 && g->Cout == 16 && g->KH == 4 && g->KW == 4 && g->SS == 2 && g->TS == 1 && g->OFFY == -1 && g->OFFX == -1 &&
      g->OS == 1 && g->QY == 0 && g->QX == 0 && g->pre_act == 0 && !add_in && g->Hs == 2 * g->Hq && g->Ws == 2 * g->Wq && g->Ho == g->Hq &&
      g->Wo == g->Wq && g->Wq % 2 == 0 && g->Ws % 2 == 0 && g->act != MTRSSM_ACT_TANH && !((uintptr_t)src & 7) && !((uintptr_t)out & 7) && !((uintptr_t)actgrad_in & 7) &&
      kConvThreads == 256) {
    const long pairs = (long)g->N * g->Hq * (g->Wq / 2);
    set_last_kernel("mtrssm::conv4s2_c1_thin16_kernel");
    hipLaunchKernelGGL(conv4s2_c1_thin16_kernel, dim3((unsigned)((pairs + 255) / 256)), dim3(256), 0, stream, *g, src, wp, bias, actgrad_in, out);
    return launched("conv_gather_gemm(thin16 pairs)");
  }
  if ((g->Cout <= 8 || g->C + g->C2 <= 2) && g->Cout <= 16 && g->KH * g->KW * (g->C + g->C2) <= kThinMaxK) {
    const dim3 grid((unsigned)((ptot + kConvThreads - 1) / kConvThreads));
    if (g->Cout <= 2)
      { set_last_kernel("mtrssm::conv_gather_thin_kernel<2>"); hipLaunchKernelGGL(conv_gather_thin_kernel<2>, grid, dim3(kConvThreads), 0, stream, *g, src, src2, wp, bias, actgrad_in, add_in, out); }
    else if (g->Cout <= 8)
      { set_last_kernel("mtrssm::conv_gather_thin_kernel<8>"); hipLaunchKernelGGL(conv_gather_thin_kernel<8>, grid, dim3(kConvThreads), 0, stream, *g, src, src2, wp, bias, actgrad_in, add_in, out); }
    else
      { set_last_kernel("mtrssm::conv_gather_thin_kernel<16>"); hipLaunchKernelGGL(conv_gather_thin_kernel<16>, grid, dim3(kConvThreads), 0, stream, *g, src, src2, wp, bias, actgrad_in, add_in, out); }
    return launched("conv_gather_gemm(thin)");
  }
  const int gx = (int)((ptot + kTP - 1) / kTP);
  if ((g->TS == 1 || g->TS == -1) && g->KH * g->KW > 0 && plane_fits_26bit(g)) {
    const int tco = g->Cout > 32 ? 64 : 32;
// ... 209 lines not shown
}
int conv_weight_grad_src_bias_supported(const MtrssmConvGeom* g, int pre_act_a) {
  WgradSrcBias sb;
  size_t need = 0;
  const int rc = conv_weight_grad_launch_ex(g, nullptr, nullptr, nullptr, pre_act_a, nullptr, nullptr, nullptr, 0, &need, &sb, nullptr);
  return rc == MTRSSM_OK && sb.fused;
}
int conv_weight_grad_src_bias_launch(const MtrssmConvGeom* g, const float* a, const float* src, int pre_act_a, float* dwp,
                                     float* dsrcbias, void* workspace, size_t workspace_bytes, int defer, hipStream_t stream) {
  if (!dsrcbias) { set_error("conv_weight_grad_src_bias: null dsrc_bias"); return MTRSSM_EINVAL; }
  if (((uintptr_t)a & 15) || ((uintptr_t)src & 15)) {
    set_error("conv_weight_grad_src_bias: a and src must be 16-byte aligned");
    return MTRSSM_EINVAL;
  }
  if (!conv_weight_grad_src_bias_supported(g, pre_act_a)) {
    set_error("conv_weight_grad_src_bias: this geometry's kernel has no fused source sums (query mtrssm_conv_weight_grad_src_bias_supported first)");
    return MTRSSM_EINVAL;
  }
  WgradSrcBias sb;
  sb.target = dsrcbias;
  tl_defer_reduce = defer != 0;
  const int rc = conv_weight_grad_launch_ex(g, a, src, nullptr, pre_act_a, dwp, nullptr, workspace, workspace_bytes, nullptr, &sb, stream);
  tl_defer_reduce = false;
  return rc;
}
int conv_weight_grad_deferred_launch(const MtrssmConvGeom* g, const float* a, const float* src, const float* src2, int pre_act_a,
                                     float* dwp, float* dbias, void* workspace, size_t workspace_bytes, hipStream_t stream) {
  tl_defer_reduce = true;
  const int rc = conv_weight_grad_launch(g, a, src, src2, pre_act_a, dwp, dbias, workspace, workspace_bytes, nullptr, stream);
  tl_defer_reduce = false;
  return rc;
}

int conv_residual_bwd1x1_supported(const MtrssmConvGeom* g) {
  static const bool on = [] { const char* e = getenv("MTRSSM_BWD1X1_FUSED"); return !(e && e[0] == '0'); }();
  if (!g || !on || !wgrad_1x1_staged_enabled()) return 0;
  return g->mfma_split == 2 && g->KH == 1 && g->KW == 1 && g->SS == 1 && g->OFFY == 0 && g->OFFX == 0 && g->C2 == 0 && g->Hs == g->Hq &&
         g->Ws == g->Wq && g->Hq * g->Wq == 64 && (g->C == 64 || g->C == 128) && g->Cout == 64 && g->Cpad >= g->C && g->N >= 1 &&
         g->OS == 1 && g->QY == 0 && g->QX == 0 && g->pre_act != 0 &&
         (g->act == MTRSSM_ACT_IDENTITY || g->act == MTRSSM_ACT_ELU || g->act == MTRSSM_ACT_RELU);
}
int conv_residual_bwd1x1_launch(const MtrssmConvGeom* g, const float* gy, const float* h, const unsigned short* wq1t, float* gh, float* dwp,
                                float* dbias, void* workspace, size_t workspace_bytes, int defer, hipStream_t stream) {
  if (!conv_residual_bwd1x1_supported(g)) {
    set_error("residual_bwd1x1: shape without a fused kernel (query mtrssm_residual_bwd1x1_supported first)");
    return MTRSSM_EINVAL;
  }
  if (!gy || !h || !wq1t || !gh || !dwp) { set_error("residual_bwd1x1: null pointer"); return MTRSSM_EINVAL; }
  if (((uintptr_t)gy & 15) || ((uintptr_t)h & 15) || ((uintptr_t)wq1t & 15) || ((uintptr_t)gh & 3) || ((uintptr_t)workspace & 255)) {
    set_error("residual_bwd1x1: g_y, h and the weight pieces must be 16-byte aligned, the workspace 256-byte aligned");
    return MTRSSM_EINVAL;
  }
  int wgs = cu_count();
  if (wgs > g->N) wgs = g->N;
  const int per = (g->N + wgs - 1) / wgs;
  const dim3 grid((unsigned)((g->N + per - 1) / per));
  float* part = nullptr;
  if (wgrad_partials_enabled() && workspace && workspace_bytes >= (size_t)grid.x * kWg1x1SetFloats * sizeof(float)) part = static_cast<float*>(workspace);
#define MTRSSM_BW1_LAUNCH(C_)                                                                                                   \
  {                                                                                                                             \
    static bool attr_done_dev[64] = {}; bool& attr_done = attr_done_dev[device_slot()];                                         \
    constexpr int lds_b = bwd1x1_lds_bytes<C_>();                                                                               \
    if (!attr_done) {                                                                                                           \
      (void)hipFuncSetAttribute(reinterpret_cast<const void*>(conv1x1_bwd_fused_kernel<C_>),                                    \
                                hipFuncAttributeMaxDynamicSharedMemorySize, lds_b);                                             \
      attr_done = true;                                                                                                         \
    }                                                                                                                           \
    set_last_kernel("mtrssm::conv1x1_bwd_fused_kernel<" #C_ ">");                                                               \
    hipLaunchKernelGGL((conv1x1_bwd_fused_kernel<C_>), grid, dim3(512), lds_b, stream, *g, gy, h, wq1t, gh, dwp, part, dbias,   \
                       per);                                                                                                    \
  }
  if (g->C == 64) MTRSSM_BW1_LAUNCH(64) else MTRSSM_BW1_LAUNCH(128)
#undef MTRSSM_BW1_LAUNCH
  if (part) {
    const dim3 rgrid((unsigned)(2 * (g->C / 32) * 256 / 32 + (dbias ? 1 : 0)), 1);
    tl_defer_reduce = defer != 0;
    const int rc = reduce_now_or_later(g->C == 64 ? kRed1x1_64 : kRed1x1_128, rgrid, part, (int)grid.x, g->Cpad, dwp, dbias, stream);
    tl_defer_reduce = false;
    if (rc) return rc;
  }
  return launched("residual_bwd1x1");
}

int conv_weight_grad_launch_ex(const MtrssmConvGeom* g, const float* a, const float* src, const float* src2, int pre_act_a, float* dwp,
                               float* dbias, void* workspace, size_t workspace_bytes, size_t* query, WgradSrcBias* sb, hipStream_t stream) {
  if (int rc = check_geom(g, "conv_weight_grad")) return rc;
  if (!query && (!a || !src || !dwp || (g->C2 > 0 && !src2))) { set_error("conv_weight_grad: null pointer"); return MTRSSM_EINVAL; }
  if (workspace && ((uintptr_t)workspace & 255)) { set_error("conv_weight_grad: workspace must be 256-byte aligned"); return MTRSSM_EINVAL; }
  if (dbias && pre_act_a) { set_error("conv_weight_grad: the fused bias gradient sums the RAW a tensor; pass dbias only with pre_act_a = 0"); return MTRSSM_EINVAL; }
  if (g->OS != 1 || g->QY != 0 || g->QX != 0 || g->KH * g->KW <= 0) { set_error("conv_weight_grad: needs a plain (OS=1) geometry with taps"); return MTRSSM_EINVAL; }
  const long ptot = (long)g->N * g->Hq * g->Wq;
  const int taps = g->KH * g->KW;
  const int ctot = g->C + g->C2;
  if ((g->mfma_split == 1 || g->mfma_split == 2) && taps == 1 && g->SS == 1 && g->OFFY == 0 && g->OFFX == 0 && g->C2 == 0 && g->Hs == g->Hq &&
      g->Ws == g->Wq && g->Hq * g->Wq == 64 && (g->C == 64 || g->C == 128) && g->Cout % 64 == 0 && g->Cout <= 65535 * 64 && g->Cpad >= g->C &&
      !pre_act_a && (g->act == MTRSSM_ACT_IDENTITY || g->act == MTRSSM_ACT_ELU || g->act == MTRSSM_ACT_RELU) && !((uintptr_t)a & 15) &&
      !((uintptr_t)src & 15) && wgrad_1x1_staged_enabled()) {
    const int cogroups = g->Cout / 64;
    int wgs = cu_count() / cogroups;
    if (wgs < 1) wgs = 1;
    if (wgs > g->N) wgs = g->N;
    const int per = (g->N + wgs - 1) / wgs;
    const dim3 grid((unsigned)((g->N + per - 1) / per), cogroups);
    MTRSSM_WGRAD_PART((size_t)grid.x * cogroups * kWg1x1SetFloats * sizeof(float))
#define MTRSSM_WG1_LAUNCH(SP_, C_)                                                                                              \
  {                                                                                                                             \
    static bool attr_done_dev[64] = {}; bool& attr_done = attr_done_dev[device_slot()];        \
    constexpr int lds_b = wg1x1_lds_bytes<SP_, C_>();                                                                           \
    if (!attr_done) {                                                                                                           \
      (void)hipFuncSetAttribute(reinterpret_cast<const void*>(conv1x1_wgrad_staged_kernel<SP_, C_>),                            \
                                hipFuncAttributeMaxDynamicSharedMemorySize, lds_b);                                             \
      attr_done = true;                                                                                                         \
    }                                                                                                                           \
    set_last_kernel("mtrssm::conv1x1_wgrad_staged_kernel<" #SP_ ", " #C_ ">");                                                  \
    hipLaunchKernelGGL((conv1x1_wgrad_staged_kernel<SP_, C_>), grid, dim3(512), lds_b, stream, *g, a, src, dwp, part, dbias,    \
                       per);                                                                                                    \
  }
    const int sp = g->mfma_split;
    if (g->C == 64) { if (sp == 2) MTRSSM_WG1_LAUNCH(2, 64) else MTRSSM_WG1_LAUNCH(1, 64) }
    else { if (sp == 2) MTRSSM_WG1_LAUNCH(2, 128) else MTRSSM_WG1_LAUNCH(1, 128) }
#undef MTRSSM_WG1_LAUNCH
    if (part) {
      const dim3 rgrid((unsigned)(2 * (g->C / 32) * 256 / 32 + (dbias ? 1 : 0)), cogroups);
      if (int rc = reduce_now_or_later(g->C == 64 ? kRed1x1_64 : kRed1x1_128, rgrid, part, (int)grid.x, g->Cpad, dwp, dbias, stream)) return rc;
    }
    return launched("conv_weight_grad(1x1 staged)");
  }
  if (g->mfma_split >= 1 && taps == 1 && g->SS == 1 && g->OFFY == 0 && g->OFFX == 0 && g->C2 == 0 && g->Hs == g->Hq && g->Ws == g->Wq &&
      (g->Hq * g->Wq) % 16 == 0 && g->Cout <= 128 && g->C <= 128 && g->C >= 8 && !((uintptr_t)a & 15) && !((uintptr_t)src & 15) &&
      ptot < (1L << 31)) {
    MTRSSM_WGRAD_NO_PART
    const int tiles_co = (g->Cout + 31) / 32, tiles_ci = (g->C + 31) / 32;
    const int total = (int)(ptot / 16);
    int splits = 256;
    if (splits > total) splits = total;
    const int per = (total + splits - 1) / splits;
    const dim3 grid((unsigned)((total + per - 1) / per));
    const dim3 block(64 * tiles_co * tiles_ci);
    const int sp = g->mfma_split;
    set_last_kernel(sp == 3 ? "mtrssm::conv1x1_weight_grad_split_kernel<3>" : sp == 2 ? "mtrssm::conv1x1_weight_grad_split_kernel<2>" : "mtrssm::conv1x1_weight_grad_split_kernel<1>");
    if (sp == 3) hipLaunchKernelGGL((conv1x1_weight_grad_split_kernel<3>), grid, block, 0, stream, *g, a, src, pre_act_a, dwp, dbias, tiles_ci, per);
    else if (sp == 2) hipLaunchKernelGGL((conv1x1_weight_grad_split_kernel<2>), grid, block, 0, stream, *g, a, src, pre_act_a, dwp, dbias, tiles_ci, per);
    else hipLaunchKernelGGL((conv1x1_weight_grad_split_kernel<1>), grid, block, 0, stream, *g, a, src, pre_act_a, dwp, dbias, tiles_ci, per);
    return launched("conv_weight_grad(1x1 split)");
  }
  if ((g->mfma_split == 1 || g->mfma_split == 2) && g->KH == 3 && g->KW == 3 && g->SS == 1 && g->TS == 1 && g->OFFY == -1 && g->OFFX == -1 &&
      g->C2 == 0 && g->Hs == g->Hq && g->Ws == g->Wq && (g->Wq == 8 || g->Wq == 4) && g->Hq * g->Wq == 64 && (g->C == 64 || (g->C == 32 && wgrad_resident_c32())) &&
      g->Cout % 64 == 0 && g->Cout <= 65535 * 64 && g->Cpad >= g->C && !pre_act_a &&
      (g->act == MTRSSM_ACT_IDENTITY || g->act == MTRSSM_ACT_ELU || g->act == MTRSSM_ACT_RELU) && !((uintptr_t)a & 15) &&
      !((uintptr_t)src & 15) && !((uintptr_t)dwp & 15) && wgrad_resident_enabled() && !no_direct_wgrad()) {
    const int cogroups = g->Cout / 64;
    int wgs = (g->C == 64 ? cu_count() : 2 * cu_count()) / cogroups;
    if (wgs < 1) wgs = 1;
    if (wgs > g->N) wgs = g->N;
    const int per = (g->N + wgs - 1) / wgs;
    const dim3 grid((unsigned)((g->N + per - 1) / per), cogroups);
    const size_t set_floats = (size_t)wgres_set_floats(g->C);
    MTRSSM_WGRAD_PART((size_t)grid.x * cogroups * set_floats * sizeof(float))
#define MTRSSM_WGRES_LAUNCH(SP_, C_, W_)                                                                                         \
  {                                                                                                                             \
    static bool attr_done_dev[64] = {}; bool& attr_done = attr_done_dev[device_slot()];        \
    constexpr int lds_b = wgres_lds_bytes<SP_, C_, W_>();                                                                       \
    if (!attr_done) {                                                                                                           \
      (void)hipFuncSetAttribute(reinterpret_cast<const void*>(conv3x3_wgrad_resident_kernel<SP_, C_, W_>),                       \
                                hipFuncAttributeMaxDynamicSharedMemorySize, lds_b);                                             \
      attr_done = true;                                                                                                         \
    }                                                                                                                           \
    set_last_kernel("mtrssm::conv3x3_wgrad_resident_kernel<" #SP_ ", " #C_ ", " #W_ ">");                                        \
    hipLaunchKernelGGL((conv3x3_wgrad_resident_kernel<SP_, C_, W_>), grid, dim3(64 * 2 * (C_ / 32)), lds_b, stream, *g, a, src,  \
                       dwp, part, dbias, per);                                                                                  \
  }
    const int sp = g->mfma_split;
    if (g->C == 64) {
      if (g->Wq == 8) { if (sp == 2) MTRSSM_WGRES_LAUNCH(2, 64, 8) else MTRSSM_WGRES_LAUNCH(1, 64, 8) }
      else { if (sp == 2) MTRSSM_WGRES_LAUNCH(2, 64, 4) else MTRSSM_WGRES_LAUNCH(1, 64, 4) }
    } else {
      if (g->Wq == 8) { if (sp == 2) MTRSSM_WGRES_LAUNCH(2, 32, 8) else MTRSSM_WGRES_LAUNCH(1, 32, 8) }
      else { if (sp == 2) MTRSSM_WGRES_LAUNCH(2, 32, 4) else MTRSSM_WGRES_LAUNCH(1, 32, 4) }
    }
#undef MTRSSM_WGRES_LAUNCH
    if (part) {
      const dim3 rgrid((unsigned)(wgres_tile_floats(g->C) / 4 / 32 + (dbias ? 1 : 0)), cogroups);
      if (int rc = reduce_now_or_later(g->C == 64 ? kRedRes64 : kRedRes32, rgrid, part, (int)grid.x, g->Cpad, dwp, dbias, stream)) return rc;
    }
    return launched("conv_weight_grad(3x3 resident)");
  }
  if (g->mfma_split >= 1 && g->KH == 3 && g->KW == 3 && g->SS == 1 && g->TS == 1 && g->OFFY == -1 && g->OFFX == -1 && g->C2 == 0 &&
      g->Hs == g->Hq && g->Ws == g->Wq && (g->Wq == 8 || g->Wq == 4) && (g->Hq * g->Wq) % 16 == 0 && g->C <= 64 && g->C >= 8 &&
      g->Cout <= 65535 * 64 && !((uintptr_t)a & 15) && !((uintptr_t)src & 15) && ptot < (1L << 31) && !no_direct_wgrad()) {
    MTRSSM_WGRAD_NO_PART
    const int cogroups = (g->Cout + 63) / 64;
    const int tiles_co = g->Cout > 32 ? 2 : 1, tiles_ci = (g->C + 31) / 32;
    const int nt = tiles_co * tiles_ci;
    const int total = (int)(ptot / 16);
    int splits = 1024 / (nt * cogroups);
    if (splits < 1) splits = 1;
    if (splits > total) splits = total;
    const int per = (total + splits - 1) / splits;
    const dim3 grid((unsigned)((total + per - 1) / per), cogroups);
    const dim3 block(64 * nt);
    const int sp = g->mfma_split;
#define MTRSSM_W33_LAUNCH(SP_, W_)                                                                                               \
  {                                                                                                                             \
    set_last_kernel("mtrssm::conv3x3_weight_grad_split_kernel<" #SP_ ", " #W_ ">");                                              \
    hipLaunchKernelGGL((conv3x3_weight_grad_split_kernel<SP_, W_>), grid, block, 0, stream, *g, a, src, pre_act_a, dwp, dbias, tiles_ci, per); \
  }
    if (g->Wq == 8) { if (sp == 3) MTRSSM_W33_LAUNCH(3, 8) else if (sp == 2) MTRSSM_W33_LAUNCH(2, 8) else MTRSSM_W33_LAUNCH(1, 8) }
    else { if (sp == 3) MTRSSM_W33_LAUNCH(3, 4) else if (sp == 2) MTRSSM_W33_LAUNCH(2, 4) else MTRSSM_W33_LAUNCH(1, 4) }
#undef MTRSSM_W33_LAUNCH
    return launched("conv_weight_grad(3x3 split)");
  }
  if ((g->mfma_split == 1 || g->mfma_split == 2) && g->KH == 3 && g->KW == 3 && g->SS == 2 && g->TS == 1 && g->OFFY == -1 && g->OFFX == -1 &&
      g->C == 1 && g->C2 == 2 && g->Cout == 8 && g->Hq * g->Wq == 1024 && (g->Wq == 32 || g->Wq == 16) && g->Hs == 2 * g->Hq && g->Ws == 2 * g->Wq &&
// ... 488 lines not shown
```

multimodal_mtrssm_amd/csrc/conv_resident.h:

```cpp
#pragma once

namespace mtrssm {

constexpr int kResThreads = 256;
constexpr int kResPos = 108;

__device__ unsigned long long* g_res_prof = nullptr;
#define MTRSSM_RES_STAMP(i)                                                          \
  do {                                                                               \
    if (prof && it_no < 6) prof[2 + it_no * 8 + (i)] = __builtin_readcyclecounter(); \
  } while (0)
#define MTRSSM_SGB(mask_, n_) __builtin_amdgcn_sched_group_barrier(mask_, n_, 0)

__host__ __device__ constexpr int res_row_bytes(int cin) { return cin * 2 + 16; }

__host__ __device__ constexpr int res_wrow_bytes(int cin) { return 9 * cin * 2 + 16; }
__host__ __device__ constexpr int res_group_rows(int cin) { return cin >= 128 ? 32 : 64; }

template <int IMGB>
__device__ __forceinline__ void res_read_pair(bf16x8& hi, bf16x8& lo, unsigned addr, int cb) {
  switch (cb) {
    case 0: asm volatile("ds_read_b128 %0, %2\n\tds_read_b128 %1, %2 offset:%3" : "=&v"(hi), "=&v"(lo) : "v"(addr), "n"(IMGB)); break;
    case 1: asm volatile("ds_read_b128 %0, %2 offset:32\n\tds_read_b128 %1, %2 offset:%3" : "=&v"(hi), "=&v"(lo) : "v"(addr), "n"(IMGB + 32)); break;
    case 2: asm volatile("ds_read_b128 %0, %2 offset:64\n\tds_read_b128 %1, %2 offset:%3" : "=&v"(hi), "=&v"(lo) : "v"(addr), "n"(IMGB + 64)); break;
    default: asm volatile("ds_read_b128 %0, %2 offset:96\n\tds_read_b128 %1, %2 offset:%3" : "=&v"(hi), "=&v"(lo) : "v"(addr), "n"(IMGB + 96)); break;
  }
}
template <int N>
__device__ __forceinline__ void res_wait(bf16x8& b0, bf16x8& b1) {
  asm volatile("s_waitcnt lgkmcnt(%2)" : "+v"(b0), "+v"(b1) : "n"(N));
}

template <int CIN, int NCT, int KS>
__host__ __device__ constexpr size_t res_lds_bytes() {
  constexpr int NPG = 4 / (NCT * KS);
  constexpr size_t run = (size_t)4 * NPG * kResPos * res_row_bytes(CIN) + (size_t)NCT * 32 * sizeof(float) +
                         (KS == 2 ? (size_t)NPG * NCT * 2 * 16 * 64 * sizeof(float) : 0);
  constexpr size_t stage = (size_t)res_group_rows(CIN) * res_wrow_bytes(CIN);
  return run > stage ? run : stage;
}

template <int CIN, int NCT>
__host__ __device__ constexpr size_t res_fuse_bytes() {
  return (size_t)NCT * (CIN / 32) * 2 * 2 * 64 * 16 + (size_t)4 * (NCT == 2 ? 16 : CIN / 2) * 64 * sizeof(float);
}

template <int CIN, int NCT, int KS, bool EPI, bool FUSE = false>
__global__ __launch_bounds__(kResThreads, 1) void conv3x3_resident_kernel(const GatherProblem pa, const GatherProblem pb) {
  static_assert(NCT * KS == 4 || NCT * KS == 2 || NCT * KS == 1, "4 waves");
  static_assert(!FUSE || (KS == 1 && !EPI && CIN % 32 == 0), "fused block: whole K per wave, no epilogue operands");
  constexpr int NPG = 4 / (NCT * KS);
  constexpr int CW = CIN / KS;
  constexpr int CB = CW / 16;
  constexpr int KB = 9 * CB;
  constexpr int RB = res_row_bytes(CIN);
  constexpr int IMG = NPG * kResPos * RB;
  constexpr int OCT = CIN / 8;
  constexpr int NIT = NPG * OCT / 4;
  static_assert(NIT >= 1 && CB >= 1, "shape");
  const bool second = blockIdx.x >= (unsigned)pa.nx;
  const GatherProblem P = second ? pb : pa;
  const MtrssmConvGeom g = P.g;
  const float* __restrict__ src = P.src;
  const unsigned short* __restrict__ wq = P.wq;
  const float* __restrict__ bias = P.bias;
  const float* __restrict__ actgrad_in = P.actgrad_in;
  const float* __restrict__ add_in = P.add_in;
  float* __restrict__ out = P.out;
  const int wg = second ? (int)blockIdx.x - pa.nx : (int)blockIdx.x, nwg = P.nx;
  const int nframes = g.N;
  const int ntiles = nframes / NPG;
  if (wg >= ntiles) return;

  extern __shared__ __attribute__((aligned(16))) unsigned char lds_raw[];
  unsigned char* patch = lds_raw;
  float* red = reinterpret_cast<float*>(lds_raw + (size_t)4 * IMG);
  const int tid = threadIdx.x, lane = tid & 63, wave = __builtin_amdgcn_readfirstlane(tid >> 6);
  const int kl = lane >> 5, il = lane & 31;
  const int ct = wave % NCT;
  const int kh = (wave / NCT) % KS;
  const int pgi = wave / (NCT * KS);

  unsigned long long* prof = (blockIdx.x == 0 && tid == 0) ? g_res_prof : nullptr;
// ... 99 lines not shown
    asm volatile("" : "+v"(e));
    const float neg = act_elu ? e : (act_relu ? 0.f : x);
    return (x > 0.f || !pre) ? x : neg;
  };
  auto act_grad_sel = [&](float x) {
    float e = __expf(x);
    asm volatile("" : "+v"(e));
    const float neg = act_elu ? e : (act_relu ? 0.f : 1.f);
    return x > 0.f ? 1.f : neg;
  };
  auto act_mid_sel = [&](float x) {
    const float e = __expf(x) - 1.f;
    const float neg = act_elu ? e : (act_relu ? 0.f : x);
    return x > 0.f ? x : neg;
  };

  float pv[NIT][8];
  auto stage_load_part = [&](int tile, int part, int nparts) {
    constexpr int TOT = NIT * 8;
    const int per = TOT / nparts;
    int opaque = 0;
    asm volatile("" : "+s"(opaque));
#pragma unroll
    for (int j = 0; j < TOT; ++j) {
      if (j / per != part) continue;
      const int it = j / 8, u = j % 8;
      const int q = wave * NIT + it, fi = q / OCT, o = q % OCT;
      pv[it][u] = src[((size_t)(tile * NPG + fi + opaque) * CIN + o * 8 + u) * 64 + lane];
    }
  };
  auto stage_store_chunk = [&](int buf, int c) {
    const int it = c / 4, u2 = c % 4;
    const int q = wave * NIT + it, fi = q / OCT, o = q % OCT;
    unsigned short p0[2], p1[2];
    split_bf16<2>(act_fwd_sel(pv[it][2 * u2]), p0);
    split_bf16<2>(act_fwd_sel(pv[it][2 * u2 + 1]), p1);
    int opaque = 0;
    asm volatile("" : "+s"(opaque));
    unsigned char* dst = patch + (size_t)buf * 2 * IMG + (fi * kResPos + spos + opaque) * RB + o * 16 + u2 * 4;
    *reinterpret_cast<unsigned*>(dst) = (unsigned)p0[0] | ((unsigned)p1[0] << 16);
    *reinterpret_cast<unsigned*>(dst + IMG) = (unsigned)p0[1] | ((unsigned)p1[1] << 16);
  };
  constexpr int NSC = NIT * 4;

  if (prof) prof[57] = __builtin_readcyclecounter();
  stage_load_part(wg, 0, 1);
  __syncthreads();
#pragma unroll
  for (int c = 0; c < NSC; ++c) stage_store_chunk(0, c);
  __syncthreads();
  if (prof) prof[1] = __builtin_readcyclecounter();

  constexpr int ROWS = KS == 2 ? 8 : 16;
  constexpr int RPE = (EPI && KB >= 36) ? 1 : 2;
  constexpr int NES = ROWS / RPE;
  constexpr int NLD = EPI ? 4 : 0;
  constexpr int S0 = 1 + NES;
  constexpr int CPS = KB >= 36 ? 1 : 2;
  static_assert((1 + (KB - S0)) * CPS >= NSC, "the staging chunks fit in one unit");
  static_assert(S0 <= KB, "the epilogue fits in one unit");
  f32x16 acc;
  float fin[ROWS];
  float gvs[2][16], avs[2][16], part[8];
  unsigned ob_prev = (unsigned)(wg * NPG + pgi) * (unsigned)(NCT * 32 * 64) + (unsigned)(cbase * 64 + il) + 32u;
#pragma unroll
  for (int r = 0; r < 16; ++r) gvs[0][r] = gvs[1][r] = avs[0][r] = avs[1][r] = 0.f;
#pragma unroll
  for (int r = 0; r < ROWS; ++r) fin[r] = 0.f;
#pragma unroll
  for (int r = 0; r < 8; ++r) part[r] = 0.f;
  const float* gsrc = EPI ? (actgrad_in ? actgrad_in : add_in) : nullptr;
  const float* asrc = EPI ? (add_in ? add_in : actgrad_in) : nullptr;
  const bool has_g = actgrad_in != nullptr, has_a = add_in != nullptr;
  auto row_off = [](int r) { return (unsigned)(((r & 3) + 8 * (r >> 2)) * 64); };
// ... 529 lines not shown
```

multimodal_mtrssm_amd/csrc/conv_wgrad_resident.h:

```cpp
#pragma once

namespace mtrssm {

template <int W>
__host__ __device__ constexpr int wgres_pitch() { return (64 / W + 1) * 2 * W; }
constexpr int kWgresAPitch = 144;
template <int SPLIT, int C, int W>
__host__ __device__ constexpr int wgres_xbuf_bytes() { return SPLIT * C * wgres_pitch<W>() + 16; }
template <int SPLIT>
__host__ __device__ constexpr int wgres_abuf_bytes() { return SPLIT * 64 * kWgresAPitch; }
template <int SPLIT, int C, int W>
__host__ __device__ constexpr int wgres_lds_bytes() { return 2 * (wgres_xbuf_bytes<SPLIT, C, W>() + wgres_abuf_bytes<SPLIT>()); }
__host__ __device__ constexpr int wgres_tile_floats(int c) { return 2 * (c / 32) * 9 * 1024; }
__host__ __device__ constexpr int wgres_set_floats(int c) { return wgres_tile_floats(c) + 64; }
constexpr int kWg1x1SetFloats = 8 * 1024 + 64;

using wg_bf16x2 = __attribute__((ext_vector_type(2))) __bf16;
using wg_f32x2 = __attribute__((ext_vector_type(2))) float;
using wg_f32x4 = __attribute__((ext_vector_type(4))) float;
template <int SPLIT>
__device__ __forceinline__ void wg_split_pair(const float f0, const float f1, unsigned (&d)[SPLIT]) {
  d[0] = __builtin_bit_cast(unsigned, __builtin_convertvector(wg_f32x2{f0, f1}, wg_bf16x2));
  if constexpr (SPLIT >= 2) {
    const float r0 = f0 - __builtin_bit_cast(float, d[0] << 16), r1 = f1 - __builtin_bit_cast(float, d[0] & 0xffff0000u);
    d[1] = __builtin_bit_cast(unsigned, __builtin_convertvector(wg_f32x2{r0, r1}, wg_bf16x2));
  }
}

template <int SPLIT, int C, int W>
__global__ __launch_bounds__(64 * 2 * (C / 32), 1) void conv3x3_wgrad_resident_kernel(
    const MtrssmConvGeom g, const float* __restrict__ a, const float* __restrict__ src, float* __restrict__ dwp,
    float* __restrict__ part, float* __restrict__ dbias, const int frames_per_wg) {
  static_assert(SPLIT == 1 || SPLIT == 2, "one or two bf16 pieces");
  constexpr int NW = 2 * (C / 32), NT = 64 * NW;
  constexpr int RB = 2 * W;
  constexpr int PITCH = wgres_pitch<W>(), COPYB = C * PITCH, XBUFB = wgres_xbuf_bytes<SPLIT, C, W>();
  constexpr int APIECEB = 64 * kWgresAPitch, ABUFB = wgres_abuf_bytes<SPLIT>();
  constexpr int XI = 4, AI = 1024 / NT;
  extern __shared__ __attribute__((aligned(16))) unsigned char wgres_lds[];
  unsigned char* const lds = wgres_lds;
  unsigned char* const lds_a = wgres_lds + 2 * XBUFB;
  const int tid = threadIdx.x, lane = tid & 63, wave = tid >> 6;
  const int il = lane & 31, kl = lane >> 5;
  const int tci = wave >> 1, half = wave & 1;
  const int n0 = blockIdx.x * frames_per_wg;
  const int n1 = n0 + frames_per_wg < g.N ? n0 + frames_per_wg : g.N;
  if (n0 >= n1) return;
  const int nlast = n1 - 1;
  const int cob = blockIdx.y * 64;
  unsigned long long* const prof = (tid == 0 && blockIdx.y == 0 && g_res_prof) ? (blockIdx.x == 0 ? g_res_prof + 32 : (blockIdx.x == gridDim.x / 2 ? g_res_prof + 40 : nullptr)) : nullptr;
  if (prof) prof[0] = __builtin_readcyclecounter();

  const bool act_elu = g.act == MTRSSM_ACT_ELU, act_relu = g.act == MTRSSM_ACT_RELU, pre = g.pre_act != 0;
  auto act_sel = [&](float x) __attribute__((always_inline)) {
    float e = __expf(x) - 1.f;
    asm volatile("" : "+v"(e));
    const float neg = act_elu ? e : (act_relu ? 0.f : x);
    return (x > 0.f || !pre) ? x : neg;
  };

  for (int o = tid * 16; o < wgres_lds_bytes<SPLIT, C, W>(); o += NT * 16) *reinterpret_cast<uint4*>(lds + o) = make_uint4(0u, 0u, 0u, 0u);

  const float4* const xsrc = reinterpret_cast<const float4*>(src) + tid;
  const float4* const asrc = reinterpret_cast<const float4*>(a + (size_t)cob * 64) + tid;
  const size_t xfr = (size_t)C * 16, afr = (size_t)g.Cout * 16;
  const int xi = tid & 15;
  const int xrow = (xi * 4) / W, xcol = (xi * 4) % W;
  const unsigned wofs = (unsigned)((tid >> 4) * PITCH + (xrow + 1) * RB + xcol * 2);
  const unsigned wofs_a = (unsigned)((tid >> 4) * kWgresAPitch + xi * 8);
  auto stage_x = [&](const float4 v, const int j, const unsigned bufoff) __attribute__((always_inline)) {
    unsigned d0[SPLIT], d1[SPLIT];
    wg_split_pair<SPLIT>(act_sel(v.x), act_sel(v.y), d0);
    wg_split_pair<SPLIT>(act_sel(v.z), act_sel(v.w), d1);
#pragma unroll
    for (int p = 0; p < SPLIT; ++p)
      *reinterpret_cast<uint2*>(lds + bufoff + wofs + (unsigned)(j * (NT / 16) * PITCH) + (unsigned)(p * COPYB)) = make_uint2(d0[p], d1[p]);
  };
  float bsum[AI];
#pragma unroll
  for (int j = 0; j < AI; ++j) bsum[j] = 0.f;
  auto stage_a = [&](const float4 v, const int j, const unsigned bufoff, const float keep) __attribute__((always_inline)) {
    bsum[j] += keep * ((v.x + v.y) + (v.z + v.w));
    unsigned d0[SPLIT], d1[SPLIT];
    wg_split_pair<SPLIT>(v.x, v.y, d0);
    wg_split_pair<SPLIT>(v.z, v.w, d1);
#pragma unroll
    for (int p = 0; p < SPLIT; ++p)
      *reinterpret_cast<uint2*>(lds_a + bufoff + wofs_a + (unsigned)(j * (NT / 16) * kWgresAPitch) + (unsigned)(p * APIECEB)) = make_uint2(d0[p], d1[p]);
  };

  const int coA = half, coB = half ^ 1;
  const int tyo = half ? 2 : 0;
  const unsigned lane_b = (unsigned)((tci * 32 + il) * PITCH + kl * 16);
  const unsigned lane_a0 = (unsigned)((coA * 32 + il) * kWgresAPitch + kl * 16), lane_a1 = (unsigned)((coB * 32 + il) * kWgresAPitch + kl * 16);
  const unsigned outer_off = lane_b + (unsigned)(tyo * RB);
  const unsigned ext_off = lane_b + (W == 8 ? 16u : (half ? 8u : 16u));

  f32x16 acc[9];
#pragma unroll
  for (int t = 0; t < 9; ++t)
#pragma unroll
    for (int r = 0; r < 16; ++r) acc[t][r] = 0.f;

  u32x4 qa[2][2][SPLIT];
  u32x4 ro[2][SPLIT], rc[2][SPLIT];
  auto operands = [&](const int q, const int set, const unsigned xoff, const unsigned aoff) __attribute__((always_inline)) {
#pragma unroll
    for (int p = 0; p < SPLIT; ++p) {
      qa[set][0][p] = *reinterpret_cast<const u32x4*>(lds_a + aoff + lane_a0 + (unsigned)(p * APIECEB + q * 32));
      qa[set][1][p] = *reinterpret_cast<const u32x4*>(lds_a + aoff + lane_a1 + (unsigned)(p * APIECEB + q * 32));
      ro[set][p] = *reinterpret_cast<const u32x4*>(lds + xoff + outer_off + (unsigned)(p * COPYB + q * 32));
      if (W == 8) {
        rc[set][p] = *reinterpret_cast<const u32x4*>(lds + xoff + ext_off + (unsigned)(p * COPYB + q * 32));
      } else {
        const uint2 e = *reinterpret_cast<const uint2*>(lds + xoff + ext_off + (unsigned)(p * COPYB + q * 32));
        rc[set][p] = u32x4{e.x, e.y, 0u, 0u};
      }
    }
// ... 90 lines not shown
        __builtin_amdgcn_sched_group_barrier(0x402, 5, 0);
        if ((i & 1) == 0) __builtin_amdgcn_sched_group_barrier(0x080, 1, 0);
      }
    }
  };
#pragma unroll 1
  for (int n = n0; n < n1; n += 2) {
    frame(n, 0);
    if (n + 1 < n1) frame(n + 1, 1);
  }
  asm volatile("s_waitcnt vmcnt(0)" ::: "memory");
  if (prof) prof[2] = __builtin_readcyclecounter();

  if (part) {
    float4* const ps = reinterpret_cast<float4*>(part) + ((size_t)blockIdx.y * gridDim.x + blockIdx.x) * (wgres_set_floats(C) / 4) + (size_t)wave * (9 * 4 * 64) + lane;
#pragma unroll
    for (int j = 0; j < 9; ++j)
#pragma unroll
      for (int gq = 0; gq < 4; ++gq) ps[(j * 4 + gq) * 64] = make_float4(acc[j][4 * gq], acc[j][4 * gq + 1], acc[j][4 * gq + 2], acc[j][4 * gq + 3]);
  } else {
    const int ci = tci * 32 + il;
#pragma unroll
    for (int j = 0; j < 9; ++j) {
      const int k = j < 5 ? j : j - 5;
      const int tap = k < 3 ? tyo * 3 + k : (k == 3 ? (half ? 5 : 3) : 4);
      const int cot = cob + (j < 5 ? coA : coB) * 32;
#pragma unroll
      for (int r = 0; r < 16; ++r) {
        const int row = cot + (r & 3) + 8 * (r >> 2) + 4 * kl;
        atomicAdd(&dwp[((size_t)row * 9 + tap) * g.Cpad + ci], acc[j][r]);
      }
    }
  }
  if (dbias != nullptr) {
#pragma unroll
    for (int j = 0; j < AI; ++j) {
      float v = bsum[j];
      v += dpp_move<0xB1, 0xF>(0.f, v);
      v += dpp_move<0x4E, 0xF>(0.f, v);
      v += dpp_move<0x141, 0xF>(0.f, v);
      v += dpp_move<0x140, 0xF>(0.f, v);
      if (xi == 0) {
        const int ch = (tid >> 4) + j * (NT / 16);
        if (part) part[((size_t)blockIdx.y * gridDim.x + blockIdx.x) * wgres_set_floats(C) + wgres_tile_floats(C) + ch] = v;
        else atomicAdd(&dbias[cob + ch], v);
      }
    }
  }
  if (prof) {
    asm volatile("s_waitcnt vmcnt(0)" ::: "memory");
    prof[3] = __builtin_readcyclecounter();
  }
}

template <int C>
__device__ __forceinline__ void wgrad_reduce_partials_body(const float4* __restrict__ part, const int S, const int cpad,
                                                                    float* __restrict__ dwp, float* __restrict__ dbias, const int bx, const int by) {
  constexpr int SET4 = wgres_set_floats(C) / 4, TILE4 = wgres_tile_floats(C) / 4;
  constexpr int NL = 32, NG = 8;
  static_assert(TILE4 % NL == 0, "whole blocks");
  __shared__ float4 red[NG][NL];
  const int li = threadIdx.x & (NL - 1), sg = threadIdx.x / NL;
  const int f = bx * NL + li;
  const float4* const p = part + (size_t)by * S * SET4 + (f < SET4 ? f : SET4 - 1);
  float4 acc4[4];
#pragma unroll
  for (int u = 0; u < 4; ++u) acc4[u] = make_float4(0.f, 0.f, 0.f, 0.f);
// ... 161 lines not shown
#pragma unroll
    for (int gq = 0; gq < 4; ++gq) ps[gq * 64] = make_float4(acc[4 * gq], acc[4 * gq + 1], acc[4 * gq + 2], acc[4 * gq + 3]);
  } else {
    const int ci = tci * 32 + il;
#pragma unroll
    for (int r = 0; r < 16; ++r) {
      const int row = cob + tco * 32 + (r & 3) + 8 * (r >> 2) + 4 * kl;
      atomicAdd(&dwp[(size_t)row * g.Cpad + ci], acc[r]);
    }
  }
  if (dbias != nullptr) {
#pragma unroll
    for (int j = 0; j < AI; ++j) {
      float v = bsum[j];
      v += dpp_move<0xB1, 0xF>(0.f, v);
      v += dpp_move<0x4E, 0xF>(0.f, v);
      v += dpp_move<0x141, 0xF>(0.f, v);
      v += dpp_move<0x140, 0xF>(0.f, v);
      if ((tid & 15) == 0) {
        const int ch = (tid >> 4) + j * 32;
        if (part) part[((size_t)blockIdx.y * gridDim.x + blockIdx.x) * kWg1x1SetFloats + 8 * 1024 + ch] = v;
        else atomicAdd(&dbias[cob + ch], v);
      }
    }
  }
  if (prof) {
    asm volatile("s_waitcnt vmcnt(0)" ::: "memory");
    prof[3] = __builtin_readcyclecounter();
  }
}

template <int C>
__device__ __forceinline__ void wgrad_reduce_partials1x1_body(const float4* __restrict__ part, const int S, const int cpad,
                                                                       float* __restrict__ dwp, float* __restrict__ dbias, const int bx, const int by) {
  constexpr int NTILE = 2 * (C / 32), KS = 8 / NTILE, TILE4 = 256, SET4 = kWg1x1SetFloats / 4;
  constexpr int NL = 32, NG = 8;
  __shared__ float4 red[NG][NL];
  const int li = threadIdx.x & (NL - 1), sg = threadIdx.x / NL;
  const int f = bx * NL + li;
  const bool bias = f >= NTILE * TILE4;
  const int tile = f / TILE4, ft = f - tile * TILE4;
  const float4* const p = part + (size_t)by * S * SET4 + (bias ? (size_t)(8 * TILE4 + (f - NTILE * TILE4 < 16 ? f - NTILE * TILE4 : 15)) : (size_t)tile * TILE4 + ft);
  float4 acc4[4];
#pragma unroll
  for (int u = 0; u < 4; ++u) acc4[u] = make_float4(0.f, 0.f, 0.f, 0.f);
  const int ks = bias ? 1 : KS;
  const int slices = S * ks;
  int i = sg;
  for (; i + 3 * NG < slices; i += 4 * NG) {
#pragma unroll
    for (int u = 0; u < 4; ++u) {
      const int ii = i + NG * u;
      const float4 v = p[(size_t)(ii / ks) * SET4 + (size_t)(ii % ks) * (NTILE * TILE4)];
      acc4[u].x += v.x; acc4[u].y += v.y; acc4[u].z += v.z; acc4[u].w += v.w;
    }
  }
  for (; i < slices; i += NG) {
    const float4 v = p[(size_t)(i / ks) * SET4 + (size_t)(i % ks) * (NTILE * TILE4)];
    acc4[0].x += v.x; acc4[0].y += v.y; acc4[0].z += v.z; acc4[0].w += v.w;
  }
  red[sg][li] = make_float4((acc4[0].x + acc4[1].x) + (acc4[2].x + acc4[3].x), (acc4[0].y + acc4[1].y) + (acc4[2].y + acc4[3].y),
                            (acc4[0].z + acc4[1].z) + (acc4[2].z + acc4[3].z), (acc4[0].w + acc4[1].w) + (acc4[2].w + acc4[3].w));
  __syncthreads();
  if (sg == 0) {
    float4 v = red[0][li];
#pragma unroll
    for (int k = 1; k < NG; ++k) { v.x += red[k][li].x; v.y += red[k][li].y; v.z += red[k][li].z; v.w += red[k][li].w; }
    if (bias) {
      if (f - NTILE * TILE4 < 16) {
        float* const o = dbias + by * 64 + 4 * (f - NTILE * TILE4);
        o[0] += v.x; o[1] += v.y; o[2] += v.z; o[3] += v.w;
      }
      return;
    }
    const int lane = ft & 63, gq = ft >> 6, il = lane & 31, kl = lane >> 5;
    const int tco = tile & 1, tci = tile >> 1;
    float* const o = dwp + (size_t)(by * 64 + tco * 32 + 8 * gq + 4 * kl) * cpad + tci * 32 + il;
    o[0] += v.x; o[cpad] += v.y; o[2 * (size_t)cpad] += v.z; o[3 * (size_t)cpad] += v.w;
  }
}
template <int C>
__global__ __launch_bounds__(256) void wgrad_reduce_partials1x1_kernel(const float4* __restrict__ part, const int S, const int cpad,
                                                                       float* __restrict__ dwp, float* __restrict__ dbias) {
  wgrad_reduce_partials1x1_body<C>(part, S, cpad, dwp, dbias, (int)blockIdx.x, (int)blockIdx.y);
}

template <int C>
__host__ __device__ constexpr int bwd1x1_lds_bytes() { return wg1x1_lds_bytes<2, C>() + 2 * 2 * 64 * kWgresAPitch; }

template <int C>
__global__ __launch_bounds__(512, 1) void conv1x1_bwd_fused_kernel(
    const MtrssmConvGeom g, const float* __restrict__ a, const float* __restrict__ src, const unsigned short* __restrict__ wq,
    float* __restrict__ gh, float* __restrict__ dwp, float* __restrict__ part, float* __restrict__ dbias, const int frames_per_wg) {
  static_assert(C == 64 || C == 128, "mid channels");
  constexpr int SPLIT = 2, NT = 512, P = kWgresAPitch;
  constexpr int XI = C * 16 / NT, AI = 2, NI = XI + AI;
  constexpr int NTILE = 2 * (C / 32), KS = 8 / NTILE;
  constexpr int APB = 64 * P, XPB = C * P;
  constexpr int BUFB = SPLIT * (APB + XPB);
  constexpr int PMB = 64 * P, PMBUF = SPLIT * PMB;
  constexpr int PM0 = 2 * BUFB;
  extern __shared__ __attribute__((aligned(16))) unsigned char bw1_lds[];
  unsigned char* const lds = bw1_lds;
  const int tid = threadIdx.x, lane = tid & 63, wave = tid >> 6;
  const int il = lane & 31, kl = lane >> 5;
  const int tile = wave % NTILE, kpart = wave / NTILE;
  const int tco = tile & 1, tci = tile >> 1;
  const int n0 = blockIdx.x * frames_per_wg;
  const int n1 = n0 + frames_per_wg < g.N ? n0 + frames_per_wg : g.N;
  if (n0 >= n1) return;
  const int nlast = n1 - 1;

  const bool act_elu = g.act == MTRSSM_ACT_ELU, act_relu = g.act == MTRSSM_ACT_RELU;
  auto act_sel = [&](float x) __attribute__((always_inline)) {
    float e = __expf(x) - 1.f;
    asm volatile("" : "+v"(e));
    const float neg = act_elu ? e : (act_relu ? 0.f : x);
    return x > 0.f ? x : neg;
  };

  const int bct = (wave >> 1) % (C / 32), bhalf = wave & 1;
  const bool bstore = C == 128 || wave < 4;
  u32x4 wa[4][2];
#pragma unroll
  for (int cb = 0; cb < 4; ++cb)
#pragma unroll
    for (int sp = 0; sp < 2; ++sp) {
      wa[cb][sp] = *reinterpret_cast<const u32x4*>(wq + (size_t)sp * (C * 64) + (size_t)(bct * 32 + il) * 64 + cb * 16 + 8 * kl);
      asm volatile("" : "+v"(wa[cb][sp]));
    }

  const float4* const xsrc = reinterpret_cast<const float4*>(src) + tid;
  const float4* const asrc = reinterpret_cast<const float4*>(a) + tid;
  constexpr size_t xfr = (size_t)C * 16, afr = (size_t)64 * 16;
  const unsigned wofs = (unsigned)((tid >> 4) * P + (tid & 15) * 8);
  const unsigned pofs = (unsigned)(PM0 + 4 * (tid & 15) * P + (tid >> 4) * 2);
  float bsum[AI];
#pragma unroll
  for (int j = 0; j < AI; ++j) bsum[j] = 0.f;
  wg_f32x4 raw[3][NI];
  auto raw_load = [&](const int rs, const int n) __attribute__((always_inline)) {
#pragma unroll
    for (int it = 0; it < NI; ++it) {
      const float4* const ptr = it < AI ? asrc + (size_t)n * afr + NT * it : xsrc + (size_t)n * xfr + NT * (it - AI);
      asm volatile("global_load_dwordx4 %0, %1, off" : "=v"(raw[rs][it]) : "v"(ptr));
    }
  };
  auto raw_wait = [&](const int rs) __attribute__((always_inline)) {
    if constexpr (NI == 4) asm volatile("s_waitcnt vmcnt(40)" : "+v"(raw[rs][0]), "+v"(raw[rs][1]), "+v"(raw[rs][2]), "+v"(raw[rs][3]));
    else asm volatile("s_waitcnt vmcnt(44)" : "+v"(raw[rs][0]), "+v"(raw[rs][1]), "+v"(raw[rs][2]), "+v"(raw[rs][3]), "+v"(raw[rs][4]), "+v"(raw[rs][5]));
  };
  const float* const hop = src + (size_t)(bct * 32 + 4 * kl) * 64 + bhalf * 32 + il;
  float* const ghp = gh + (size_t)(bct * 32 + 4 * kl) * 64 + bhalf * 32 + il;
  float opv[2][16];
  auto op_load = [&](const int os, const int n) __attribute__((always_inline)) {
#pragma unroll
    for (int r = 0; r < 16; ++r) {
      const float* const ptr = hop + (size_t)n * (C * 64) + ((r & 3) + 8 * (r >> 2)) * 64;
      asm volatile("global_load_dword %0, %1, off" : "=v"(opv[os][r]) : "v"(ptr));
    }
  };
  auto op_wait = [&](const int os) __attribute__((always_inline)) {
#define MTRSSM_OPV(os_, b_) "+v"(opv[os_][b_]), "+v"(opv[os_][b_ + 1]), "+v"(opv[os_][b_ + 2]), "+v"(opv[os_][b_ + 3]), "+v"(opv[os_][b_ + 4]), \
                            "+v"(opv[os_][b_ + 5]), "+v"(opv[os_][b_ + 6]), "+v"(opv[os_][b_ + 7])
    if constexpr (NI == 4) asm volatile("s_waitcnt vmcnt(24)" : MTRSSM_OPV(os, 0));
    else asm volatile("s_waitcnt vmcnt(28)" : MTRSSM_OPV(os, 0));
    asm volatile("" : MTRSSM_OPV(os, 8));
#undef MTRSSM_OPV
  };
  auto stage = [&](const int rs, const unsigned bufoff, const unsigned pmoff) __attribute__((always_inline)) {
#pragma unroll
    for (int it = 0; it < NI; ++it) {
      const wg_f32x4 v = raw[rs][it];
      unsigned d0[SPLIT], d1[SPLIT];
      if (it < AI) {
        bsum[it] += (v.x + v.y) + (v.z + v.w);
        wg_split_pair<SPLIT>(v.x, v.y, d0);
        wg_split_pair<SPLIT>(v.z, v.w, d1);
#pragma unroll
        for (int p = 0; p < SPLIT; ++p) {
          unsigned char* const q = lds + pmoff + pofs + (unsigned)(it * 64 + p * PMB);
          *reinterpret_cast<unsigned short*>(q) = (unsigned short)(d0[p] & 0xffffu);
          *reinterpret_cast<unsigned short*>(q + P) = (unsigned short)(d0[p] >> 16);
          *reinterpret_cast<unsigned short*>(q + 2 * P) = (unsigned short)(d1[p] & 0xffffu);
          *reinterpret_cast<unsigned short*>(q + 3 * P) = (unsigned short)(d1[p] >> 16);
        }
      } else {
// ... 23 lines not shown
    raw_load((rs + 2) % 3, n + 2 < nlast ? n + 2 : nlast);
    raw_wait(rs);
    stage(rs, bufoff, pmoff);
    lds_barrier();
#pragma unroll
    for (int qq = 0; qq < 4 / KS; ++qq) {
      const int q = kpart * (4 / KS) + qq;
      u32x4 qa[SPLIT], qb[SPLIT];
#pragma unroll
      for (int p = 0; p < SPLIT; ++p) {
        qa[p] = *reinterpret_cast<const u32x4*>(lds + bufoff + lane_a + (unsigned)(p * APB) + (unsigned)(q * 32));
        qb[p] = *reinterpret_cast<const u32x4*>(lds + bufoff + lane_b + (unsigned)(p * XPB) + (unsigned)(q * 32));
      }
#pragma unroll
      for (int ord = SPLIT - 1; ord >= 0; --ord)
#pragma unroll
        for (int sa = 0; sa <= ord; ++sa)
          acc = __builtin_amdgcn_mfma_f32_32x32x16_bf16(__builtin_bit_cast(bf16x8, qa[sa]), __builtin_bit_cast(bf16x8, qb[ord - sa]), acc, 0, 0, 0);
    }
    f32x16 accb;
#pragma unroll
    for (int r = 0; r < 16; ++r) accb[r] = 0.f;
#pragma unroll
    for (int cb = 0; cb < 4; ++cb) {
      const bf16x8 bh = __builtin_bit_cast(bf16x8, *reinterpret_cast<const u32x4*>(lds + pmoff + lane_p + (unsigned)(cb * 32)));
      const bf16x8 bl = __builtin_bit_cast(bf16x8, *reinterpret_cast<const u32x4*>(lds + pmoff + lane_p + (unsigned)(PMB + cb * 32)));
      accb = __builtin_amdgcn_mfma_f32_32x32x16_bf16(__builtin_bit_cast(bf16x8, wa[cb][0]), bl, accb, 0, 0, 0);
      accb = __builtin_amdgcn_mfma_f32_32x32x16_bf16(__builtin_bit_cast(bf16x8, wa[cb][1]), bh, accb, 0, 0, 0);
      accb = __builtin_amdgcn_mfma_f32_32x32x16_bf16(__builtin_bit_cast(bf16x8, wa[cb][0]), bh, accb, 0, 0, 0);
    }
    op_wait(par);
    if (bstore) {
      float* const o = ghp + (size_t)n * (C * 64);
#pragma unroll
      for (int r = 0; r < 16; ++r) {
        const float x = opv[par][r];
        const float e = __expf(x);
        const float neg = act_elu ? e : (act_relu ? 0.f : 1.f);
        o[((r & 3) + 8 * (r >> 2)) * 64] = accb[r] * (x > 0.f ? 1.f : neg);
      }
    }
  };
#pragma unroll 1
  for (int n = n0; n < n1; n += 6) {
    frame(n, 0, 0);
    if (n + 1 < n1) frame(n + 1, 1, 1);
    if (n + 2 < n1) frame(n + 2, 2, 0);
    if (n + 3 < n1) frame(n + 3, 0, 1);
    if (n + 4 < n1) frame(n + 4, 1, 0);
    if (n + 5 < n1) frame(n + 5, 2, 1);
  }
  asm volatile("s_waitcnt vmcnt(0)" ::: "memory");

  if (part) {
    float4* const ps = reinterpret_cast<float4*>(part) + (size_t)blockIdx.x * (kWg1x1SetFloats / 4) + (size_t)wave * 256 + lane;
#pragma unroll
    for (int gq = 0; gq < 4; ++gq) ps[gq * 64] = make_float4(acc[4 * gq], acc[4 * gq + 1], acc[4 * gq + 2], acc[4 * gq + 3]);
  } else {
    const int ci = tci * 32 + il;
#pragma unroll
    for (int r = 0; r < 16; ++r) {
      const int row = tco * 32 + (r & 3) + 8 * (r >> 2) + 4 * kl;
      atomicAdd(&dwp[(size_t)row * g.Cpad + ci], acc[r]);
    }
  }
  if (dbias != nullptr) {
#pragma unroll
    for (int j = 0; j < AI; ++j) {
      float v = bsum[j];
      v += dpp_move<0xB1, 0xF>(0.f, v);
      v += dpp_move<0x4E, 0xF>(0.f, v);
      v += dpp_move<0x141, 0xF>(0.f, v);
      v += dpp_move<0x140, 0xF>(0.f, v);
      if ((tid & 15) == 0) {
        const int ch = (tid >> 4) + j * 32;
        if (part) part[(size_t)blockIdx.x * kWg1x1SetFloats + 8 * 1024 + ch] = v;
        else atomicAdd(&dbias[ch], v);
      }
    }
  }
}

constexpr int kWgS2SetFloats = 8 * 2 * 64 * 4 + 16;
template <int WO>
__host__ __device__ constexpr int wgs2_cip() { return (((256 / WO * 2 + 1) * (2 * WO)) / 16 | 1) * 16; }
template <int SPLIT, int WO>
__host__ __device__ constexpr int wgs2_lds_bytes() { return 2 * SPLIT * (2 * 8 * wgs2_cip<WO>() + 16 * 528); }

template <int SPLIT, int WO>
__global__ __launch_bounds__(512, 1) void conv3x3s2_wgrad_staged_kernel(
    const MtrssmConvGeom g, const float* __restrict__ a, const float* __restrict__ src, float* __restrict__ dwp,
    float* __restrict__ part, float* __restrict__ dbias, const int frames_per_wg) {
  static_assert(SPLIT == 1 || SPLIT == 2, "one or two bf16 pieces");
  static_assert(WO == 16 || WO == 8, "output plane 16x16 or 32x8");
  constexpr int NT = 512, C = 8, CO = 16, HO = 256 / WO, HS = 2 * HO, WS = 2 * WO;
  constexpr int ROWB = WS;
  constexpr int CIP = wgs2_cip<WO>();
  constexpr int XCOPY = C * CIP;
  constexpr int AP = 528, APB = CO * AP;
  constexpr int BUFB = SPLIT * (2 * XCOPY + APB);
  constexpr int XI = C * HS * WS / 4 / NT, AI = CO * 256 / 4 / NT, NI = XI + AI;
  extern __shared__ __attribute__((aligned(16))) unsigned char wgs2_lds[];
  unsigned char* const lds = wgs2_lds;
  const int tid = threadIdx.x, lane = tid & 63, wave = tid >> 6;
  const int il = lane & 31, kl = lane >> 5;
  const int ct = wave & 3, kh = wave >> 2;
  const int n0 = blockIdx.x * frames_per_wg;
  const int n1 = n0 + frames_per_wg < g.N ? n0 + frames_per_wg : g.N;
  if (n0 >= n1) return;
  const int nlast = n1 - 1;
// ... 1261 lines not shown
```

Measured before the change: 368,900 seq-steps/s.

## Emit residual 3x3 backward gradient as pre-split bf16 pieces with fused bias sum

The fused 1x1 residual backward kernel now writes the hidden gradient as packed bf16 hi/lo piece words instead of fp32. It also accumulates the 3x3 bias gradient during that same pass. The downstream 3x3 transposed gather and the resident weight-grad kernel read these words directly, which skips their own fp32-to-bf16 splitting and the separate bias reduction. The path is on by default through an environment flag and falls back when the geometry is unsupported. It adds template variants, an extra reduction slot in the partials, and some risk of bias-sum ordering differences.

Result: no change. 371,800 seq-steps/s (median of 6 runs) (+0.8%).

```diff
diff --git a/include/mtrssm.h b/include/mtrssm.h
--- a/include/mtrssm.h
+++ b/include/mtrssm.h
@@ -315,6 +315,7 @@
   int32_t pre_act;
   int32_t act;
   int32_t mfma_split;
+  int32_t src_pieces;
 } MtrssmConvGeom;
 
 int mtrssm_conv_gather_gemm(const MtrssmConvGeom* g, const float* src, const float* src2, const float* wp, const uint16_t* wq,
@@ -341,6 +342,12 @@
 int mtrssm_residual_bwd1x1_supported(const MtrssmConvGeom* g);
 int mtrssm_residual_bwd1x1(const MtrssmConvGeom* g, const float* gy, const float* h, const uint16_t* wq1t, float* gh, float* dwp,
                            float* dbias, void* workspace, int64_t workspace_bytes, int32_t defer, void* stream);
+int mtrssm_residual_bwd1x1_pieces(const MtrssmConvGeom* g, const float* gy, const float* h, const uint16_t* wq1t, uint32_t* gh_pieces,
+                                  float* dwp, float* dbias, float* dbias3, void* workspace, int64_t workspace_bytes, int32_t defer,
+                                  void* stream);
+int mtrssm_conv_gather_pieces_supported(const MtrssmConvGeom* g);
+int mtrssm_conv_resident_raw(int32_t on);
+int mtrssm_conv_weight_grad_pieces_supported(const MtrssmConvGeom* g);
 int mtrssm_conv_weight_grad_src_bias(const MtrssmConvGeom* g, const float* a, const float* src, int32_t pre_act_a, float* dwp,
                                      float* dsrc_bias, void* workspace, int64_t workspace_bytes, int32_t defer, void* stream);
 int64_t mtrssm_conv_weight_grad_workspace_bytes(const MtrssmConvGeom* g, int32_t pre_act_a);
diff --git a/multimodal_mtrssm_amd/_lib.py b/multimodal_mtrssm_amd/_lib.py
--- a/multimodal_mtrssm_amd/_lib.py
+++ b/multimodal_mtrssm_amd/_lib.py
@@ -70,7 +70,7 @@
 
 ConvGeom = _struct("MtrssmConvGeom", [(n, _i) for n in (
     "N", "C", "Hs", "Ws", "C2", "Cpad", "KH", "KW", "SS", "TS", "OFFY", "OFFX", "Hq", "Wq", "OS", "QY", "QX", "Ho", "Wo",
-    "Cout", "CoutPad", "pre_act", "act", "mfma_split")])
+    "Cout", "CoutPad", "pre_act", "act", "mfma_split", "src_pieces")])
 
 Gemm = _struct("MtrssmGemm", _ptrs("A", "B", "C", "bias", "zgrad", "colsum") + [(n, _i) for n in (
     "M", "N", "R", "lda", "ldb", "ldc", "ldz", "a_rmajor", "b_rmajor", "act_a", "act_b", "act_out", "act_z", "accumulate", "split_r")]
@@ -117,6 +117,10 @@
     "mtrssm_conv_weight_grad_deferred": (C.c_int, [C.POINTER(ConvGeom), _p, _p, _p, _i, _p, _p, _p, C.c_int64, _p]),
     "mtrssm_residual_bwd1x1_supported": (C.c_int, [C.POINTER(ConvGeom)]),
     "mtrssm_residual_bwd1x1": (C.c_int, [C.POINTER(ConvGeom), _p, _p, _p, _p, _p, _p, _p, C.c_int64, _i, _p]),
+    "mtrssm_residual_bwd1x1_pieces": (C.c_int, [C.POINTER(ConvGeom), _p, _p, _p, _p, _p, _p, _p, _p, C.c_int64, _i, _p]),
+    "mtrssm_conv_gather_pieces_supported": (C.c_int, [C.POINTER(ConvGeom)]),
+    "mtrssm_conv_resident_raw": (C.c_int, [_i]),
+    "mtrssm_conv_weight_grad_pieces_supported": (C.c_int, [C.POINTER(ConvGeom)]),
     "mtrssm_conv_weight_grad_src_bias_supported": (C.c_int, [C.POINTER(ConvGeom), _i]),
     "mtrssm_conv_weight_grad_src_bias": (C.c_int, [C.POINTER(ConvGeom), _p, _p, _i, _p, _p, _p, C.c_int64, _i, _p]),
     "mtrssm_conv_weight_grad_reduce": (C.c_int, [_p]),
diff --git a/multimodal_mtrssm_amd/conv.py b/multimodal_mtrssm_amd/conv.py
--- a/multimodal_mtrssm_amd/conv.py
+++ b/multimodal_mtrssm_amd/conv.py
@@ -186,7 +186,7 @@
 
 def _job_args(job: tuple) -> tuple:
     geom, src, src2, wp, wq, bias, actgrad_in, add_in, out = job
-    return (C.byref(geom), _lib.ptr(src), _lib.ptr(src2), _lib.ptr(wp), _lib.raw_ptr(wq), _lib.ptr(bias), _lib.ptr(actgrad_in),
+    return (C.byref(geom), _lib.raw_ptr(src) if geom.src_pieces else _lib.ptr(src), _lib.ptr(src2), _lib.ptr(wp), _lib.raw_ptr(wq), _lib.ptr(bias), _lib.ptr(actgrad_in),
             _lib.ptr(add_in), _lib.ptr(out))
 
 
@@ -278,7 +278,11 @@
 
 
 def _conv_transposed_gather(y: Tensor, w: Tensor, bias: Tensor | None, stride: int, pad: int, out_hw: tuple[int, int],
-                            pre_act: bool, act: int, actgrad_in: Tensor | None = None, add_in: Tensor | None = None) -> Tensor:
+                            pre_act: bool, act: int, actgrad_in: Tensor | None = None, add_in: Tensor | None = None, *,
+                            y_pieces: bool = False) -> Tensor:
+    if y_pieces and (stride != 1 or pre_act or y.dtype != torch.int32):
+        msg = "a piece-word source needs a stride-1 gather without pre-activation"
+        raise ValueError(msg)
     n, o, hs, ws = y.shape
     o2, c, kh, kw = w.shape
     if o2 != o:
@@ -344,7 +348,7 @@
             geom = _geom(N=n, C=o, Hs=hs, Ws=ws, C2=0, Cpad=wp.shape[2], KH=wsub.shape[2], KW=wsub.shape[3], SS=1, TS=-1,
                          OFFY=(qy + pad - ky0) // stride, OFFX=(qx + pad - kx0) // stride,
                          Hq=(ho - qy + stride - 1) // stride, Wq=(wo - qx + stride - 1) // stride, OS=stride, QY=qy, QX=qx,
-                         Ho=ho, Wo=wo, Cout=c, CoutPad=wp.shape[0], pre_act=int(pre_act), act=act)
+                         Ho=ho, Wo=wo, Cout=c, CoutPad=wp.shape[0], pre_act=int(pre_act), act=act, src_pieces=int(y_pieces))
             _gather_gemm(geom, y, None, wpq, bias, actgrad_in, out, add_in)
     return out
 
@@ -489,7 +493,10 @@
 
 def _weight_grad(a: Tensor, src: Tensor, coords: Tensor | None, kh: int, kw: int, stride: int, pad: int, pre_act_a: bool,
                  pre_act_src: bool, act: int, *, want_bias: bool = False, weight: Tensor | None = None,
-                 bias: Tensor | None = None, want_src_bias: bool = False) -> tuple[Tensor | None, Tensor | None]:
+                 bias: Tensor | None = None, want_src_bias: bool = False, a_pieces: bool = False) -> tuple[Tensor | None, Tensor | None]:
+    if a_pieces and (want_bias or want_src_bias or pre_act_a or a.dtype != torch.int32):
+        msg = "a piece-word operand carries no bias sums and no pre-activation"
+        raise ValueError(msg)
     lib = _lib.load()
     n, o, hq, wq = a.shape
     _, c, hs, ws = src.shape
@@ -502,7 +509,7 @@
     if want_bias or fuse_src_bias:
         bias_sunk = grad_target(bias) if bias is not None and bias.is_contiguous() else None
     geom = _geom(N=n, C=c, Hs=hs, Ws=ws, C2=c2, Cpad=ipad, KH=kh, KW=kw, SS=stride, TS=1, OFFY=-pad, OFFX=-pad, Hq=hq, Wq=wq,
-                 OS=1, QY=0, QX=0, Ho=hq, Wo=wq, Cout=o, CoutPad=opad, pre_act=int(pre_act_src), act=act)
+                 OS=1, QY=0, QX=0, Ho=hq, Wo=wq, Cout=o, CoutPad=opad, pre_act=int(pre_act_src), act=act, src_pieces=int(a_pieces))
     flops = 2.0 * n * hq * wq * o * kh * kw * (c + c2)
     nbytes = 4.0 * (a.numel() + src.numel())
     fuse_src_bias = fuse_src_bias and bool(lib.mtrssm_conv_weight_grad_src_bias_supported(C.byref(geom), int(pre_act_a)))
@@ -519,7 +526,7 @@
         return g_w, (None if bias_sunk is not None else dbias)
     entry = lib.mtrssm_conv_weight_grad_deferred if defer and ws is not None else lib.mtrssm_conv_weight_grad
     _lib.check(_lib.TIMERS.call(
-        "mtrssm_conv_weight_grad", entry, C.byref(geom), _lib.ptr(a), _lib.ptr(src), _lib.ptr(coords),
+        "mtrssm_conv_weight_grad", entry, C.byref(geom), _lib.raw_ptr(a) if a_pieces else _lib.ptr(a), _lib.ptr(src), _lib.ptr(coords),
         int(pre_act_a), _lib.ptr(dwp), _lib.ptr(dbias), _lib.raw_ptr(ws), 0 if ws is None else ws.numel() * 4, _lib.stream_ptr(a.device),
         flops=flops, nbytes=nbytes), "mtrssm_conv_weight_grad")
     g_w = None if sunk is not None else dwp[:o, :, : c + c2].reshape(o, kh, kw, c + c2).permute(0, 3, 1, 2)
@@ -660,7 +667,28 @@
     return geom if _lib.load().mtrssm_residual_bwd1x1_supported(C.byref(geom)) else None
 
 
-def _bwd1x1_fused(geom: C.Structure, g_y: Tensor, h: Tensor, w1: Tensor, b1: Tensor) -> tuple[Tensor, Tensor | None, Tensor | None]:
+BWD3X3_PIECES = os.environ.get("MTRSSM_BWD3X3_PIECES", "1") != "0"
+
+
+def _bwd3x3_pieces(h: Tensor, x: Tensor, w3: Tensor, act: int) -> bool:
+    if not BWD3X3_PIECES or _MFMA_SPLIT != 2 or w3.shape[2:] != (3, 3) or x.data_ptr() % 16:
+        return False
+    n, o, hs, ws = h.shape
+    c = x.shape[1]
+    if w3.shape[:2] != (o, c) or x.shape != (n, c, hs, ws):
+        return False
+    lib = _lib.load()
+    opad, ipad = _pads(c, o)
+    gg = _geom(N=n, C=o, Hs=hs, Ws=ws, C2=0, Cpad=ipad, KH=3, KW=3, SS=1, TS=-1, OFFY=1, OFFX=1, Hq=hs, Wq=ws, OS=1, QY=0, QX=0,
+               Ho=hs, Wo=ws, Cout=c, CoutPad=opad, pre_act=0, act=act)
+    opad, ipad = _pads(o, c)
+    gw = _geom(N=n, C=c, Hs=hs, Ws=ws, C2=0, Cpad=ipad, KH=3, KW=3, SS=1, TS=1, OFFY=-1, OFFX=-1, Hq=hs, Wq=ws, OS=1, QY=0, QX=0,
+               Ho=hs, Wo=ws, Cout=o, CoutPad=opad, pre_act=1, act=act)
+    return bool(lib.mtrssm_conv_gather_pieces_supported(C.byref(gg))) and bool(lib.mtrssm_conv_weight_grad_pieces_supported(C.byref(gw)))
+
+
+def _bwd1x1_fused(geom: C.Structure, g_y: Tensor, h: Tensor, w1: Tensor, b1: Tensor,
+                  b3: Tensor | None = None) -> tuple[Tensor, Tensor | None, Tensor | None, Tensor | None]:
     lib = _lib.load()
     n, o, hq, wq = g_y.shape
     c = h.shape[1]
@@ -669,16 +697,27 @@
     dwp = sunk if sunk is not None else _zeros(geom.CoutPad * geom.Cpad, g_y.device).view(geom.CoutPad, 1, geom.Cpad)
     bias_sunk = grad_target(b1) if b1.is_contiguous() else None
     dbias = bias_sunk if bias_sunk is not None else _zeros(o, g_y.device)
-    defer = DEFER_WGRAD_REDUCE and sunk is not None and bias_sunk is not None
+    pieces = b3 is not None
+    bias3_sunk = grad_target(b3) if pieces and b3.is_contiguous() else None
+    dbias3 = (bias3_sunk if bias3_sunk is not None else _zeros(c, g_y.device)) if pieces else None
+    defer = DEFER_WGRAD_REDUCE and sunk is not None and bias_sunk is not None and (not pieces or bias3_sunk is not None)
     ws = _wgrad_workspace(geom, 0, g_y.device, own=defer)
-    g_h = torch.empty_like(h)
     pixels = n * hq * wq
-    _lib.check(_lib.TIMERS.call(
-        "mtrssm_residual_bwd1x1", lib.mtrssm_residual_bwd1x1, C.byref(geom), _lib.ptr(g_y), _lib.ptr(h), _lib.raw_ptr(wq1t), _lib.ptr(g_h),
-        _lib.ptr(dwp), _lib.ptr(dbias), _lib.raw_ptr(ws), 0 if ws is None else ws.numel() * 4, int(defer and ws is not None),
-        _lib.stream_ptr(g_y.device), flops=2.0 * 2.0 * pixels * o * c, nbytes=4.0 * (g_y.numel() + 2 * h.numel())), "mtrssm_residual_bwd1x1")
+    flops, nbytes = 2.0 * 2.0 * pixels * o * c, 4.0 * (g_y.numel() + 2 * h.numel())
+    if pieces:
+        g_h = torch.empty(h.shape, device=h.device, dtype=torch.int32)
+        _lib.check(_lib.TIMERS.call(
+            "mtrssm_residual_bwd1x1", lib.mtrssm_residual_bwd1x1_pieces, C.byref(geom), _lib.ptr(g_y), _lib.ptr(h), _lib.raw_ptr(wq1t),
+            _lib.raw_ptr(g_h), _lib.ptr(dwp), _lib.ptr(dbias), _lib.ptr(dbias3), _lib.raw_ptr(ws), 0 if ws is None else ws.numel() * 4,
+            int(defer and ws is not None), _lib.stream_ptr(g_y.device), flops=flops, nbytes=nbytes), "mtrssm_residual_bwd1x1_pieces")
+    else:
+        g_h = torch.empty_like(h)
+        _lib.check(_lib.TIMERS.call(
+            "mtrssm_residual_bwd1x1", lib.mtrssm_residual_bwd1x1, C.byref(geom), _lib.ptr(g_y), _lib.ptr(h), _lib.raw_ptr(wq1t), _lib.ptr(g_h),
+            _lib.ptr(dwp), _lib.ptr(dbias), _lib.raw_ptr(ws), 0 if ws is None else ws.numel() * 4, int(defer and ws is not None),
+            _lib.stream_ptr(g_y.device), flops=flops, nbytes=nbytes), "mtrssm_residual_bwd1x1")
     g_w = None if sunk is not None else dwp[:o, :, :c].reshape(o, 1, 1, c).permute(0, 3, 1, 2)
-    return g_h, g_w, (None if bias_sunk is not None else dbias)
+    return g_h, g_w, (None if bias_sunk is not None else dbias), (None if bias3_sunk is not None else dbias3)
 
 
 class _ResidualBlock(torch.autograd.Function):
@@ -706,15 +745,20 @@
         p3, p1 = w3.shape[2] // 2, w1.shape[2] // 2
         b3, b1 = ctx.biases
         g1 = _bwd1x1_geom(g_y, h, w1, act)
+        pk = g1 is not None and _bwd3x3_pieces(h, x, w3, act)
+        g_b3 = None
         if g1 is not None:
-            g_h, g_w1, g_b1 = _bwd1x1_fused(g1, g_y, h, w1, b1)
+            g_h, g_w1, g_b1, g_b3 = _bwd1x1_fused(g1, g_y, h, w1, b1, b3 if pk else None)
         else:
             g_h = _conv_transposed_gather(g_y, w1, None, 1, p1, (h.shape[2], h.shape[3]), False, act, actgrad_in=h)
             g_w1, g_b1 = _weight_grad(g_y, h, None, w1.shape[2], w1.shape[3], 1, p1, False, True, act, want_bias=True, weight=w1, bias=b1)
         g_x = None
         if ctx.needs_input_grad[0]:
-            g_x = _conv_transposed_gather(g_h, w3, None, 1, p3, (x.shape[2], x.shape[3]), False, act, actgrad_in=x, add_in=g_y)
-        g_w3, g_b3 = _weight_grad(g_h, x, None, w3.shape[2], w3.shape[3], 1, p3, False, True, act, want_bias=True, weight=w3, bias=b3)
+            g_x = _conv_transposed_gather(g_h, w3, None, 1, p3, (x.shape[2], x.shape[3]), False, act, actgrad_in=x, add_in=g_y, y_pieces=pk)
+        if pk:
+            g_w3, _ = _weight_grad(g_h, x, None, w3.shape[2], w3.shape[3], 1, p3, False, True, act, weight=w3, a_pieces=True)
+        else:
+            g_w3, g_b3 = _weight_grad(g_h, x, None, w3.shape[2], w3.shape[3], 1, p3, False, True, act, want_bias=True, weight=w3, bias=b3)
         return g_x, g_w3, g_b3, g_w1, g_b1, None
 
 
@@ -747,19 +791,31 @@
         b3a, b1a, b3v, b1v = ctx.biases
         g1a = _bwd1x1_geom(g_ya, ha, w1a, act)
         g1v = _bwd1x1_geom(g_yv, hv, w1v, act) if g1a is not None else None
-        if g1a is not None and g1v is not None:
-            g_ha, g_w1a, g_b1a = _bwd1x1_fused(g1a, g_ya, ha, w1a, b1a)
-            g_hv, g_w1v, g_b1v = _bwd1x1_fused(g1v, g_yv, hv, w1v, b1v)
+        fused = g1a is not None and g1v is not None
+        pka = fused and _bwd3x3_pieces(ha, xa, w3a, act)
+        pkv = fused and _bwd3x3_pieces(hv, xv, w3v, act)
+        g_b3a = g_b3v = None
+        if fused:
+            g_ha, g_w1a, g_b1a, g_b3a = _bwd1x1_fused(g1a, g_ya, ha, w1a, b1a, b3a if pka else None)
+            g_hv, g_w1v, g_b1v, g_b3v = _bwd1x1_fused(g1v, g_yv, hv, w1v, b1v, b3v if pkv else None)
         else:
             g_ha, g_hv = paired(lambda: _conv_transposed_gather(g_ya, w1a, None, 1, p1, (ha.shape[2], ha.shape[3]), False, act, actgrad_in=ha),
                                 lambda: _conv_transposed_gather(g_yv, w1v, None, 1, p1, (hv.shape[2], hv.shape[3]), False, act, actgrad_in=hv))
             g_w1a, g_b1a = _weight_grad(g_ya, ha, None, w1a.shape[2], w1a.shape[3], 1, p1, False, True, act, want_bias=True, weight=w1a, bias=b1a)
             g_w1v, g_b1v = _weight_grad(g_yv, hv, None, w1v.shape[2], w1v.shape[3], 1, p1, False, True, act, want_bias=True, weight=w1v, bias=b1v)
         g_xa, g_xv = paired(
-            lambda: _conv_transposed_gather(g_ha, w3a, None, 1, p3, (xa.shape[2], xa.shape[3]), False, act, actgrad_in=xa, add_in=g_ya),
-            lambda: _conv_transposed_gather(g_hv, w3v, None, 1, p3, (xv.shape[2], xv.shape[3]), False, act, actgrad_in=xv, add_in=g_yv))
-        g_w3a, g_b3a = _weight_grad(g_ha, xa, None, w3a.shape[2], w3a.shape[3], 1, p3, False, True, act, want_bias=True, weight=w3a, bias=b3a)
-        g_w3v, g_b3v = _weight_grad(g_hv, xv, None, w3v.shape[2], w3v.shape[3], 1, p3, False, True, act, want_bias=True, weight=w3v, bias=b3v)
+            lambda: _conv_transposed_gather(g_ha, w3a, None, 1, p3, (xa.shape[2], xa.shape[3]), False, act, actgrad_in=xa, add_in=g_ya,
+                                            y_pieces=pka),
+            lambda: _conv_transposed_gather(g_hv, w3v, None, 1, p3, (xv.shape[2], xv.shape[3]), False, act, actgrad_in=xv, add_in=g_yv,
+                                            y_pieces=pkv))
+        if pka:
+            g_w3a, _ = _weight_grad(g_ha, xa, None, w3a.shape[2], w3a.shape[3], 1, p3, False, True, act, weight=w3a, a_pieces=True)
+        else:
+            g_w3a, g_b3a = _weight_grad(g_ha, xa, None, w3a.shape[2], w3a.shape[3], 1, p3, False, True, act, want_bias=True, weight=w3a, bias=b3a)
+        if pkv:
+            g_w3v, _ = _weight_grad(g_hv, xv, None, w3v.shape[2], w3v.shape[3], 1, p3, False, True, act, weight=w3v, a_pieces=True)
+        else:
+            g_w3v, g_b3v = _weight_grad(g_hv, xv, None, w3v.shape[2], w3v.shape[3], 1, p3, False, True, act, want_bias=True, weight=w3v, bias=b3v)
         return g_xa, g_w3a, g_b3a, g_w1a, g_b1a, g_xv, g_w3v, g_b3v, g_w1v, g_b1v, None
 
 
diff --git a/multimodal_mtrssm_amd/csrc/capi.hip b/multimodal_mtrssm_amd/csrc/capi.hip
--- a/multimodal_mtrssm_amd/csrc/capi.hip
+++ b/multimodal_mtrssm_amd/csrc/capi.hip
@@ -50,7 +50,10 @@
 int conv_weight_grad_deferred_launch(const MtrssmConvGeom*, const float*, const float*, const float*, int, float*, float*, void*, size_t, hipStream_t);
 int conv_weight_grad_reduce_flush(hipStream_t);
 int conv_residual_bwd1x1_supported(const MtrssmConvGeom*);
-int conv_residual_bwd1x1_launch(const MtrssmConvGeom*, const float*, const float*, const unsigned short*, float*, float*, float*, void*, size_t, int,
+int conv_gather_pieces_supported(const MtrssmConvGeom*);
+int conv_resident_raw_set(int);
+int conv_weight_grad_pieces_supported(const MtrssmConvGeom*);
+int conv_residual_bwd1x1_launch(const MtrssmConvGeom*, const float*, const float*, const unsigned short*, float*, float*, float*, void*, size_t, int, int, float*,
                                 hipStream_t);
 int conv_weight_grad_src_bias_supported(const MtrssmConvGeom*, int);
 int conv_weight_grad_src_bias_launch(const MtrssmConvGeom*, const float*, const float*, int, float*, float*, void*, size_t, int, hipStream_t);
@@ -329,9 +332,18 @@
 MTRSSM_API int mtrssm_residual_bwd1x1_supported(const MtrssmConvGeom* g) { return conv_residual_bwd1x1_supported(g) != 0; }
 MTRSSM_API int mtrssm_residual_bwd1x1(const MtrssmConvGeom* g, const float* gy, const float* h, const uint16_t* wq1t, float* gh, float* dwp,
                                       float* dbias, void* workspace, int64_t workspace_bytes, int32_t defer, void* stream) {
-  return conv_residual_bwd1x1_launch(g, gy, h, wq1t, gh, dwp, dbias, workspace, workspace_bytes < 0 ? 0 : (size_t)workspace_bytes, defer,
-                                     static_cast<hipStream_t>(stream));
-}
+  return conv_residual_bwd1x1_launch(g, gy, h, wq1t, gh, dwp, dbias, workspace, workspace_bytes < 0 ? 0 : (size_t)workspace_bytes, defer, 0,
+                                     nullptr, static_cast<hipStream_t>(stream));
+}
+MTRSSM_API int mtrssm_residual_bwd1x1_pieces(const MtrssmConvGeom* g, const float* gy, const float* h, const uint16_t* wq1t, uint32_t* gh_pieces,
+                                             float* dwp, float* dbias, float* dbias3, void* workspace, int64_t workspace_bytes, int32_t defer,
+                                             void* stream) {
+  return conv_residual_bwd1x1_launch(g, gy, h, wq1t, reinterpret_cast<float*>(gh_pieces), dwp, dbias, workspace,
+                                     workspace_bytes < 0 ? 0 : (size_t)workspace_bytes, defer, 1, dbias3, static_cast<hipStream_t>(stream));
+}
+MTRSSM_API int mtrssm_conv_resident_raw(int32_t on) { return conv_resident_raw_set(on); }
+MTRSSM_API int mtrssm_conv_gather_pieces_supported(const MtrssmConvGeom* g) { return conv_gather_pieces_supported(g); }
+MTRSSM_API int mtrssm_conv_weight_grad_pieces_supported(const MtrssmConvGeom* g) { return conv_weight_grad_pieces_supported(g); }
 MTRSSM_API int mtrssm_conv_weight_grad_src_bias_supported(const MtrssmConvGeom* g, int32_t pre_act_a) {
   return conv_weight_grad_src_bias_supported(g, pre_act_a);
 }
diff --git a/multimodal_mtrssm_amd/csrc/conv.hip b/multimodal_mtrssm_amd/csrc/conv.hip
--- a/multimodal_mtrssm_amd/csrc/conv.hip
+++ b/multimodal_mtrssm_amd/csrc/conv.hip
@@ -594,6 +594,7 @@
   const float4* part;
   float* dwp;
   float* dbias;
+  float* dbias3;
   int S, cpad, variant, gx, gy;
   __host__ int variant_gy() const { return gy; }
 };
@@ -607,8 +608,8 @@
   switch (j.variant) {
     case kRedRes64: wgrad_reduce_partials_body<64>(j.part, j.S, j.cpad, j.dwp, j.dbias, bx, by); break;
     case kRedRes32: wgrad_reduce_partials_body<32>(j.part, j.S, j.cpad, j.dwp, j.dbias, bx, by); break;
-    case kRed1x1_64: wgrad_reduce_partials1x1_body<64>(j.part, j.S, j.cpad, j.dwp, j.dbias, bx, by); break;
-    case kRed1x1_128: wgrad_reduce_partials1x1_body<128>(j.part, j.S, j.cpad, j.dwp, j.dbias, bx, by); break;
+    case kRed1x1_64: wgrad_reduce_partials1x1_body<64>(j.part, j.S, j.cpad, j.dwp, j.dbias, bx, by, j.dbias3); break;
+    case kRed1x1_128: wgrad_reduce_partials1x1_body<128>(j.part, j.S, j.cpad, j.dwp, j.dbias, bx, by, j.dbias3); break;
     case kRedThin: wgrad_reduce_partials_thin_body(j.part, j.S, j.cpad, j.dwp, j.dbias, bx, by); break;
     case kRedThinT: wgrad_reduce_partials_thint_body(j.part, j.S, j.cpad, j.dwp, j.dbias, bx, by); break;
     case kRedS2: wgrad_reduce_partials_s2_body(j.part, j.S, j.cpad, j.dwp, j.dbias, bx, by); break;
@@ -660,8 +661,9 @@
   return reduce_flush_locked(it->second, stream);
 }
 
-static int reduce_now_or_later(int variant, dim3 rgrid, const float* part, int S, int cpad, float* dwp, float* dbias, hipStream_t stream) {
-  ReduceJob j{reinterpret_cast<const float4*>(part), dwp, dbias, S, cpad, variant, (int)rgrid.x, (int)rgrid.y};
+static int reduce_now_or_later(int variant, dim3 rgrid, const float* part, int S, int cpad, float* dwp, float* dbias, hipStream_t stream,
+                               float* dbias3 = nullptr) {
+  ReduceJob j{reinterpret_cast<const float4*>(part), dwp, dbias, dbias3, S, cpad, variant, (int)rgrid.x, (int)rgrid.y};
   if (tl_defer_reduce) {
     std::lock_guard<std::mutex> lock(g_reduce_mutex);
     auto& jobs = g_reduce_jobs[reduce_key(stream)];
@@ -1189,6 +1191,10 @@
     set_error("%s: mfma_split must be 0 (fp32 MFMA) or 1..3 bf16 pieces, got %d", who, g->mfma_split);
     return MTRSSM_EINVAL;
   }
+  if (g->src_pieces != 0 && g->src_pieces != 1) {
+    set_error("%s: src_pieces must be 0 or 1, got %d", who, g->src_pieces);
+    return MTRSSM_EINVAL;
+  }
   return MTRSSM_OK;
 }
 
@@ -1206,9 +1212,10 @@
   int tco = 0, ny = 0, nx = 0, sp = 0, pit = 0, tgs = 0, ngroups = 0;
   int res = 0;
   int stream = 0;
+  int pieces = 0;
   size_t lds = 0;
   bool same_kernel(const SplitPlan& o) const {
-    if (kind == 3) return o.kind == 3 && res == o.res;
+    if (kind == 3) return o.kind == 3 && res == o.res && pieces == o.pieces;
     return kind == o.kind && kind != 0 && tco == o.tco && ny == o.ny && sp == o.sp && pit == o.pit && tgs == o.tgs && ngroups == o.ngroups;
   }
 };
@@ -1216,6 +1223,17 @@
 static bool resident_enabled() {
   static const bool on = [] { const char* e = getenv("MTRSSM_CONV_RESIDENT"); return !(e && e[0] == '0'); }();
   return on;
+}
+
+static int g_resident_raw = -1;
+static bool resident_raw_enabled() {
+  if (g_resident_raw < 0) { const char* e = getenv("MTRSSM_CONV_RESIDENT_RAW"); g_resident_raw = !(e && e[0] == '0'); }
+  return g_resident_raw != 0;
+}
+int conv_resident_raw_set(int on) {
+  const int prev = resident_raw_enabled();
+  if (on >= 0) g_resident_raw = on != 0;
+  return prev;
 }
 
 static bool patch_limit_768() {
@@ -1241,6 +1259,7 @@
 static SplitPlan plan_split(const MtrssmConvGeom* g, bool has_wq) {
   SplitPlan pl;
   if (!(g->mfma_split > 0 && has_wq) || !((g->TS == 1 || g->TS == -1) && g->KH * g->KW > 0 && plane_fits_26bit(g))) return pl;
+  if (g->src_pieces && !(g->mfma_split == 2 && g->pre_act == 0 && (g->C * 1000 + g->Cout == 128064 || g->C * 1000 + g->Cout == 64064))) return pl;
   if (g->Wq > kTP || kTP % g->Wq) return pl;
   const PatchGeom pg(*g, kTP);
   const bool tiles = (g->Hq % pg.rpg == 0) || (pg.rpg % g->Hq == 0);
@@ -1260,12 +1279,14 @@
     if ((key == 64064 || key == 64128 || key == 128064 || key == 32064 || key == 64032) && g->N % fpt == 0) {
       pl.kind = 3;
       pl.res = key;
+      pl.pieces = g->src_pieces != 0;
       pl.nx = g->N;
       pl.lds = key == 64032 ? res_lds_bytes<64, 1, 2>() : key == 64064 ? res_lds_bytes<64, 2, 1>() : key == 64128 ? res_lds_bytes<64, 4, 1>() : key == 128064 ? res_lds_bytes<128, 2, 2>()
                                                                                                      : res_lds_bytes<32, 2, 1>();
       return pl;
     }
   }
+  if (g->src_pieces) return SplitPlan();
   if (taps == 1 && g->SS == 1 && g->OS == 1 && g->OFFY == 0 && g->OFFX == 0 && g->C2 == 0 && g->Hs == g->Hq && g->Ws == g->Wq &&
       g->Ho == g->Hq && g->Wo == g->Wq && g->Cpad % 64 == 0) {
     pl.kind = 1;
@@ -1321,21 +1342,36 @@
       qb.nx = (int)(ncu - na < tb ? ncu - na : tb);
     }
     const dim3 rgrid((unsigned)(qa.nx + qb.nx));
-#define MTRSSM_RES_LAUNCH_E(CIN_, NCT_, KS_, EPI_)                                                                   \
+    if (pl.pieces && !epi_a) {
+      set_error("conv_gather_gemm: a piece-word source needs the backward-data form (an epilogue operand)");
+      return MTRSSM_EINVAL;
+    }
+    const int srcf = pl.pieces ? kResSrcPieces : (epi_a && resident_raw_enabled() && pa.g.pre_act == 0 && (pb.nx == 0 || pb.g.pre_act == 0) ? kResSrcRaw : kResSrcAct);
+#define MTRSSM_RES_LAUNCH_E(CIN_, NCT_, KS_, EPI_, SRC_, TAG_)                                                        \
   {                                                                                                                   \
     static bool attr_done_dev[64] = {}; bool& attr_done = attr_done_dev[device_slot()];                                                                                    \
     const size_t rl = res_lds_bytes<CIN_, NCT_, KS_>();                                                               \
     if (!attr_done) {                                                                                                 \
-      (void)hipFuncSetAttribute(reinterpret_cast<const void*>(conv3x3_resident_kernel<CIN_, NCT_, KS_, EPI_>),        \
+      (void)hipFuncSetAttribute(reinterpret_cast<const void*>(conv3x3_resident_kernel<CIN_, NCT_, KS_, EPI_, false, SRC_>), \
                                 hipFuncAttributeMaxDynamicSharedMemorySize, (int)rl);                                 \
       attr_done = true;                                                                                               \
     }                                                                                                                 \
-    set_last_kernel("mtrssm::conv3x3_resident_kernel<" #CIN_ ", " #NCT_ ", " #KS_ ", " #EPI_ ">");                      \
-    hipLaunchKernelGGL((conv3x3_resident_kernel<CIN_, NCT_, KS_, EPI_>), rgrid, dim3(kResThreads), rl, stream, qa, qb); \
+    set_last_kernel("mtrssm::conv3x3_resident_kernel<" #CIN_ ", " #NCT_ ", " #KS_ ", " #EPI_ TAG_ ">");                 \
+    hipLaunchKernelGGL((conv3x3_resident_kernel<CIN_, NCT_, KS_, EPI_, false, SRC_>), rgrid, dim3(kResThreads), rl, stream, qa, qb); \
     return launched("conv_gather_gemm(resident)");                                                                    \
   }
-#define MTRSSM_RES_LAUNCH(CIN_, NCT_, KS_) \
-  { if (epi_a) MTRSSM_RES_LAUNCH_E(CIN_, NCT_, KS_, true) else MTRSSM_RES_LAUNCH_E(CIN_, NCT_, KS_, false) }
+#define MTRSSM_RES_LAUNCH(CIN_, NCT_, KS_)                                                  \
+  {                                                                                         \
+    if (srcf == kResSrcRaw) MTRSSM_RES_LAUNCH_E(CIN_, NCT_, KS_, true, kResSrcRaw, ", raw")  \
+    else if (epi_a) MTRSSM_RES_LAUNCH_E(CIN_, NCT_, KS_, true, kResSrcAct, "")               \
+    else MTRSSM_RES_LAUNCH_E(CIN_, NCT_, KS_, false, kResSrcAct, "")                         \
+  }
+    if (pl.pieces) {
+      if (pl.res == 64064) MTRSSM_RES_LAUNCH_E(64, 2, 1, true, kResSrcPieces, ", pieces")
+      if (pl.res == 128064) MTRSSM_RES_LAUNCH_E(128, 2, 2, true, kResSrcPieces, ", pieces")
+      set_error("conv_gather_gemm: no piece-word kernel for this plan");
+      return MTRSSM_EINVAL;
+    }
     if (pl.res == 64064) MTRSSM_RES_LAUNCH(64, 2, 1)
     if (pl.res == 64128) MTRSSM_RES_LAUNCH(64, 4, 1)
     if (pl.res == 128064) MTRSSM_RES_LAUNCH(128, 2, 2)
@@ -1538,12 +1574,30 @@
   return launched("conv_gather_gemm(s2 k4 band)");
 }
 
+int conv_gather_pieces_supported(const MtrssmConvGeom* g) {
+  if (!g || check_geom(g, "conv_gather_pieces_supported")) return 0;
+  MtrssmConvGeom q = *g;
+  q.src_pieces = 1;
+  const SplitPlan pl = plan_split(&q, true);
+  return pl.kind == 3 && pl.pieces ? 1 : 0;
+}
+
 int conv_gather_gemm_launch(const MtrssmConvGeom* g, const float* src, const float* src2, const float* wp, const unsigned short* wq,
                             const float* bias, const float* actgrad_in, const float* add_in, float* out, hipStream_t stream) {
   if (int rc = check_geom(g, "conv_gather_gemm")) return rc;
   if (!src || !wp || !out || (g->C2 > 0 && !src2)) { set_error("conv_gather_gemm: null pointer"); return MTRSSM_EINVAL; }
   if ((uintptr_t)wp & 15) { set_error("conv_gather_gemm: packed weights must be 16-byte aligned"); return MTRSSM_EINVAL; }
   const long ptot = (long)g->N * g->Hq * g->Wq;
+  if (g->src_pieces) {
+    if (!conv_gather_pieces_supported(g) || !wq || !(actgrad_in || add_in)) {
+      set_error("conv_gather_gemm: src_pieces without a piece-word kernel for this geometry (query mtrssm_conv_gather_pieces_supported first)");
+      return MTRSSM_EINVAL;
+    }
+    const SplitPlan pl = plan_split(g, true);
+    GatherProblem none{};
+    none.nx = 0;
+    return launch_split(pl, pl.lds, make_problem(g, pl, src, src2, wq, bias, actgrad_in, add_in, out), none, stream);
+  }
   if (s2_band_covers(g, wq != nullptr, actgrad_in || add_in)) {
     GatherProblem p{};
     p.g = *g; p.src = src; p.src2 = src2; p.wq = wq; p.bias = bias; p.out = out;
@@ -1819,16 +1873,26 @@
   return rc;
 }
 
+int conv_weight_grad_pieces_supported(const MtrssmConvGeom* g) {
+  if (!g || check_geom(g, "conv_weight_grad_pieces_supported")) return 0;
+  MtrssmConvGeom q = *g;
+  q.src_pieces = 1;
+  size_t need = 0;
+  return conv_weight_grad_launch_ex(&q, nullptr, nullptr, nullptr, 0, nullptr, nullptr, nullptr, 0, &need, nullptr, nullptr) == MTRSSM_OK;
+}
+
 int conv_residual_bwd1x1_supported(const MtrssmConvGeom* g) {
   static const bool on = [] { const char* e = getenv("MTRSSM_BWD1X1_FUSED"); return !(e && e[0] == '0'); }();
-  if (!g || !on || !wgrad_1x1_staged_enabled()) return 0;
+  if (!g || !on || !wgrad_1x1_staged_enabled() || g->src_pieces != 0) return 0;
   return g->mfma_split == 2 && g->KH == 1 && g->KW == 1 && g->SS == 1 && g->OFFY == 0 && g->OFFX == 0 && g->C2 == 0 && g->Hs == g->Hq &&
          g->Ws == g->Wq && g->Hq * g->Wq == 64 && (g->C == 64 || g->C == 128) && g->Cout == 64 && g->Cpad >= g->C && g->N >= 1 &&
          g->OS == 1 && g->QY == 0 && g->QX == 0 && g->pre_act != 0 &&
          (g->act == MTRSSM_ACT_IDENTITY || g->act == MTRSSM_ACT_ELU || g->act == MTRSSM_ACT_RELU);
 }
 int conv_residual_bwd1x1_launch(const MtrssmConvGeom* g, const float* gy, const float* h, const unsigned short* wq1t, float* gh, float* dwp,
-                                float* dbias, void* workspace, size_t workspace_bytes, int defer, hipStream_t stream) {
+                                float* dbias, void* workspace, size_t workspace_bytes, int defer, int pieces, float* dbias3,
+                                hipStream_t stream) {
+  if (!pieces && dbias3) { set_error("residual_bwd1x1: the channel sums of g_h come with the piece-word form only"); return MTRSSM_EINVAL; }
   if (!conv_residual_bwd1x1_supported(g)) {
     set_error("residual_bwd1x1: shape without a fused kernel (query mtrssm_residual_bwd1x1_supported first)");
     return MTRSSM_EINVAL;
@@ -1844,25 +1908,26 @@
   const dim3 grid((unsigned)((g->N + per - 1) / per));
   float* part = nullptr;
   if (wgrad_partials_enabled() && workspace && workspace_bytes >= (size_t)grid.x * kWg1x1SetFloats * sizeof(float)) part = static_cast<float*>(workspace);
-#define MTRSSM_BW1_LAUNCH(C_)                                                                                                   \
+#define MTRSSM_BW1_LAUNCH(C_, PK_)                                                                                              \
   {                                                                                                                             \
     static bool attr_done_dev[64] = {}; bool& attr_done = attr_done_dev[device_slot()];                                         \
     constexpr int lds_b = bwd1x1_lds_bytes<C_>();                                                                               \
     if (!attr_done) {                                                                                                           \
-      (void)hipFuncSetAttribute(reinterpret_cast<const void*>(conv1x1_bwd_fused_kernel<C_>),                                    \
+      (void)hipFuncSetAttribute(reinterpret_cast<const void*>(conv1x1_bwd_fused_kernel<C_, PK_>),                               \
                                 hipFuncAttributeMaxDynamicSharedMemorySize, lds_b);                                             \
       attr_done = true;                                                                                                         \
     }                                                                                                                           \
     set_last_kernel("mtrssm::conv1x1_bwd_fused_kernel<" #C_ ">");                                                               \
-    hipLaunchKernelGGL((conv1x1_bwd_fused_kernel<C_>), grid, dim3(512), lds_b, stream, *g, gy, h, wq1t, gh, dwp, part, dbias,   \
-                       per);                                                                                                    \
-  }
-  if (g->C == 64) MTRSSM_BW1_LAUNCH(64) else MTRSSM_BW1_LAUNCH(128)
+    hipLaunchKernelGGL((conv1x1_bwd_fused_kernel<C_, PK_>), grid, dim3(512), lds_b, stream, *g, gy, h, wq1t, gh, dwp, part,     \
+                       dbias, dbias3, per);                                                                                     \
+  }
+  if (pieces) { if (g->C == 64) MTRSSM_BW1_LAUNCH(64, true) else MTRSSM_BW1_LAUNCH(128, true) }
+  else { if (g->C == 64) MTRSSM_BW1_LAUNCH(64, false) else MTRSSM_BW1_LAUNCH(128, false) }
 #undef MTRSSM_BW1_LAUNCH
   if (part) {
-    const dim3 rgrid((unsigned)(2 * (g->C / 32) * 256 / 32 + (dbias ? 1 : 0)), 1);
+    const dim3 rgrid((unsigned)(2 * (g->C / 32) * 256 / 32 + (dbias || dbias3 ? 1 : 0) + (dbias3 ? 1 : 0)), 1);
     tl_defer_reduce = defer != 0;
-    const int rc = reduce_now_or_later(g->C == 64 ? kRed1x1_64 : kRed1x1_128, rgrid, part, (int)grid.x, g->Cpad, dwp, dbias, stream);
+    const int rc = reduce_now_or_later(g->C == 64 ? kRed1x1_64 : kRed1x1_128, rgrid, part, (int)grid.x, g->Cpad, dwp, dbias, stream, dbias3);
     tl_defer_reduce = false;
     if (rc) return rc;
   }
@@ -1879,6 +1944,15 @@
   const long ptot = (long)g->N * g->Hq * g->Wq;
   const int taps = g->KH * g->KW;
   const int ctot = g->C + g->C2;
+  const bool res3 = (g->mfma_split == 1 || g->mfma_split == 2) && g->KH == 3 && g->KW == 3 && g->SS == 1 && g->TS == 1 && g->OFFY == -1 && g->OFFX == -1 &&
+      g->C2 == 0 && g->Hs == g->Hq && g->Ws == g->Wq && (g->Wq == 8 || g->Wq == 4) && g->Hq * g->Wq == 64 && (g->C == 64 || (g->C == 32 && wgrad_resident_c32())) &&
+      g->Cout % 64 == 0 && g->Cout <= 65535 * 64 && g->Cpad >= g->C && !pre_act_a &&
+      (g->act == MTRSSM_ACT_IDENTITY || g->act == MTRSSM_ACT_ELU || g->act == MTRSSM_ACT_RELU) && !((uintptr_t)a & 15) &&
+      !((uintptr_t)src & 15) && !((uintptr_t)dwp & 15) && wgrad_resident_enabled() && !no_direct_wgrad();
+  if (g->src_pieces && !(res3 && g->mfma_split == 2 && g->C == 64 && !dbias && !sb)) {
+    set_error("conv_weight_grad: src_pieces without a piece-word kernel for this geometry, or with dbias (the producer of the pieces sums the bias gradient)");
+    return MTRSSM_EINVAL;
+  }
   if ((g->mfma_split == 1 || g->mfma_split == 2) && taps == 1 && g->SS == 1 && g->OFFY == 0 && g->OFFX == 0 && g->C2 == 0 && g->Hs == g->Hq &&
       g->Ws == g->Wq && g->Hq * g->Wq == 64 && (g->C == 64 || g->C == 128) && g->Cout % 64 == 0 && g->Cout <= 65535 * 64 && g->Cpad >= g->C &&
       !pre_act_a && (g->act == MTRSSM_ACT_IDENTITY || g->act == MTRSSM_ACT_ELU || g->act == MTRSSM_ACT_RELU) && !((uintptr_t)a & 15) &&
@@ -1931,11 +2005,7 @@
     else hipLaunchKernelGGL((conv1x1_weight_grad_split_kernel<1>), grid, block, 0, stream, *g, a, src, pre_act_a, dwp, dbias, tiles_ci, per);
     return launched("conv_weight_grad(1x1 split)");
   }
-  if ((g->mfma_split == 1 || g->mfma_split == 2) && g->KH == 3 && g->KW == 3 && g->SS == 1 && g->TS == 1 && g->OFFY == -1 && g->OFFX == -1 &&
-      g->C2 == 0 && g->Hs == g->Hq && g->Ws == g->Wq && (g->Wq == 8 || g->Wq == 4) && g->Hq * g->Wq == 64 && (g->C == 64 || (g->C == 32 && wgrad_resident_c32())) &&
-      g->Cout % 64 == 0 && g->Cout <= 65535 * 64 && g->Cpad >= g->C && !pre_act_a &&
-      (g->act == MTRSSM_ACT_IDENTITY || g->act == MTRSSM_ACT_ELU || g->act == MTRSSM_ACT_RELU) && !((uintptr_t)a & 15) &&
-      !((uintptr_t)src & 15) && !((uintptr_t)dwp & 15) && wgrad_resident_enabled() && !no_direct_wgrad()) {
+  if (res3) {
     const int cogroups = g->Cout / 64;
     int wgs = (g->C == 64 ? cu_count() : 2 * cu_count()) / cogroups;
     if (wgs < 1) wgs = 1;
@@ -1944,21 +2014,24 @@
     const dim3 grid((unsigned)((g->N + per - 1) / per), cogroups);
     const size_t set_floats = (size_t)wgres_set_floats(g->C);
     MTRSSM_WGRAD_PART((size_t)grid.x * cogroups * set_floats * sizeof(float))
-#define MTRSSM_WGRES_LAUNCH(SP_, C_, W_)                                                                                         \
+#define MTRSSM_WGRES_LAUNCH_P(SP_, C_, W_, APK_, TAG_)                                                                           \
   {                                                                                                                             \
     static bool attr_done_dev[64] = {}; bool& attr_done = attr_done_dev[device_slot()];        \
     constexpr int lds_b = wgres_lds_bytes<SP_, C_, W_>();                                                                       \
     if (!attr_done) {                                                                                                           \
-      (void)hipFuncSetAttribute(reinterpret_cast<const void*>(conv3x3_wgrad_resident_kernel<SP_, C_, W_>),                       \
+      (void)hipFuncSetAttribute(reinterpret_cast<const void*>(conv3x3_wgrad_resident_kernel<SP_, C_, W_, APK_>),                 \
                                 hipFuncAttributeMaxDynamicSharedMemorySize, lds_b);                                             \
       attr_done = true;                                                                                                         \
     }                                                                                                                           \
-    set_last_kernel("mtrssm::conv3x3_wgrad_resident_kernel<" #SP_ ", " #C_ ", " #W_ ">");                                        \
-    hipLaunchKernelGGL((conv3x3_wgrad_resident_kernel<SP_, C_, W_>), grid, dim3(64 * 2 * (C_ / 32)), lds_b, stream, *g, a, src,  \
-                       dwp, part, dbias, per);                                                                                  \
-  }
+    set_last_kernel("mtrssm::conv3x3_wgrad_resident_kernel<" #SP_ ", " #C_ ", " #W_ TAG_ ">");                                   \
+    hipLaunchKernelGGL((conv3x3_wgrad_resident_kernel<SP_, C_, W_, APK_>), grid, dim3(64 * 2 * (C_ / 32)), lds_b, stream, *g, a, \
+                       src, dwp, part, dbias, per);                                                                             \
+  }
+#define MTRSSM_WGRES_LAUNCH(SP_, C_, W_) MTRSSM_WGRES_LAUNCH_P(SP_, C_, W_, false, "")
     const int sp = g->mfma_split;
-    if (g->C == 64) {
+    if (g->src_pieces) {
+      if (g->Wq == 8) MTRSSM_WGRES_LAUNCH_P(2, 64, 8, true, ", pieces") else MTRSSM_WGRES_LAUNCH_P(2, 64, 4, true, ", pieces")
+    } else if (g->C == 64) {
       if (g->Wq == 8) { if (sp == 2) MTRSSM_WGRES_LAUNCH(2, 64, 8) else MTRSSM_WGRES_LAUNCH(1, 64, 8) }
       else { if (sp == 2) MTRSSM_WGRES_LAUNCH(2, 64, 4) else MTRSSM_WGRES_LAUNCH(1, 64, 4) }
     } else {
@@ -1966,6 +2039,7 @@
       else { if (sp == 2) MTRSSM_WGRES_LAUNCH(2, 32, 4) else MTRSSM_WGRES_LAUNCH(1, 32, 4) }
     }
 #undef MTRSSM_WGRES_LAUNCH
+#undef MTRSSM_WGRES_LAUNCH_P
     if (part) {
       const dim3 rgrid((unsigned)(wgres_tile_floats(g->C) / 4 / 32 + (dbias ? 1 : 0)), cogroups);
       if (int rc = reduce_now_or_later(g->C == 64 ? kRedRes64 : kRedRes32, rgrid, part, (int)grid.x, g->Cpad, dwp, dbias, stream)) return rc;
diff --git a/multimodal_mtrssm_amd/csrc/conv_resident.h b/multimodal_mtrssm_amd/csrc/conv_resident.h
--- a/multimodal_mtrssm_amd/csrc/conv_resident.h
+++ b/multimodal_mtrssm_amd/csrc/conv_resident.h
@@ -45,10 +45,12 @@
   return (size_t)NCT * (CIN / 32) * 2 * 2 * 64 * 16 + (size_t)4 * (NCT == 2 ? 16 : CIN / 2) * 64 * sizeof(float);
 }
 
-template <int CIN, int NCT, int KS, bool EPI, bool FUSE = false>
+constexpr int kResSrcAct = 0, kResSrcRaw = 1, kResSrcPieces = 2;
+
+template <int CIN, int NCT, int KS, bool EPI, bool FUSE = false, int SRC = kResSrcAct>
 __global__ __launch_bounds__(kResThreads, 1) void conv3x3_resident_kernel(const GatherProblem pa, const GatherProblem pb) {
   static_assert(NCT * KS == 4 || NCT * KS == 2 || NCT * KS == 1, "4 waves");
-  static_assert(!FUSE || (KS == 1 && !EPI && CIN % 32 == 0), "fused block: whole K per wave, no epilogue operands");
+  static_assert(!FUSE || (KS == 1 && !EPI && CIN % 32 == 0 && SRC == kResSrcAct), "fused block: whole K per wave, no epilogue operands");
   constexpr int NPG = 4 / (NCT * KS);
   constexpr int CW = CIN / KS;
   constexpr int CB = CW / 16;
@@ -214,14 +216,28 @@
   auto stage_store_chunk = [&](int buf, int c) {
     const int it = c / 4, u2 = c % 4;
     const int q = wave * NIT + it, fi = q / OCT, o = q % OCT;
-    unsigned short p0[2], p1[2];
-    split_bf16<2>(act_fwd_sel(pv[it][2 * u2]), p0);
-    split_bf16<2>(act_fwd_sel(pv[it][2 * u2 + 1]), p1);
+    unsigned hi, lo;
+    if constexpr (SRC == kResSrcPieces) {
+      const unsigned w0 = __builtin_bit_cast(unsigned, pv[it][2 * u2]), w1 = __builtin_bit_cast(unsigned, pv[it][2 * u2 + 1]);
+      hi = __builtin_amdgcn_perm(w1, w0, 0x07060302u);
+      lo = __builtin_amdgcn_perm(w1, w0, 0x05040100u);
+    } else {
+      unsigned short p0[2], p1[2];
+      if constexpr (SRC == kResSrcRaw) {
+        split_bf16<2>(pv[it][2 * u2], p0);
+        split_bf16<2>(pv[it][2 * u2 + 1], p1);
+      } else {
+        split_bf16<2>(act_fwd_sel(pv[it][2 * u2]), p0);
+        split_bf16<2>(act_fwd_sel(pv[it][2 * u2 + 1]), p1);
+      }
+      hi = (unsigned)p0[0] | ((unsigned)p1[0] << 16);
+      lo = (unsigned)p0[1] | ((unsigned)p1[1] << 16);
+    }
     int opaque = 0;
     asm volatile("" : "+s"(opaque));
     unsigned char* dst = patch + (size_t)buf * 2 * IMG + (fi * kResPos + spos + opaque) * RB + o * 16 + u2 * 4;
-    *reinterpret_cast<unsigned*>(dst) = (unsigned)p0[0] | ((unsigned)p1[0] << 16);
-    *reinterpret_cast<unsigned*>(dst + IMG) = (unsigned)p0[1] | ((unsigned)p1[1] << 16);
+    *reinterpret_cast<unsigned*>(dst) = hi;
+    *reinterpret_cast<unsigned*>(dst + IMG) = lo;
   };
   constexpr int NSC = NIT * 4;
 
diff --git a/multimodal_mtrssm_amd/csrc/conv_wgrad_resident.h b/multimodal_mtrssm_amd/csrc/conv_wgrad_resident.h
--- a/multimodal_mtrssm_amd/csrc/conv_wgrad_resident.h
+++ b/multimodal_mtrssm_amd/csrc/conv_wgrad_resident.h
@@ -13,7 +13,8 @@
 __host__ __device__ constexpr int wgres_lds_bytes() { return 2 * (wgres_xbuf_bytes<SPLIT, C, W>() + wgres_abuf_bytes<SPLIT>()); }
 __host__ __device__ constexpr int wgres_tile_floats(int c) { return 2 * (c / 32) * 9 * 1024; }
 __host__ __device__ constexpr int wgres_set_floats(int c) { return wgres_tile_floats(c) + 64; }
-constexpr int kWg1x1SetFloats = 8 * 1024 + 64;
+constexpr int kWg1x1BiasOff = 8 * 1024, kWg1x1Bias3Off = 8 * 1024 + 64;
+constexpr int kWg1x1SetFloats = 8 * 1024 + 64 + 128;
 
 using wg_bf16x2 = __attribute__((ext_vector_type(2))) __bf16;
 using wg_f32x2 = __attribute__((ext_vector_type(2))) float;
@@ -27,11 +28,21 @@
   }
 }
 
-template <int SPLIT, int C, int W>
+__device__ __forceinline__ void wg_words_to_pairs(const unsigned w0, const unsigned w1, unsigned (&d)[2]) {
+  d[0] = __builtin_amdgcn_perm(w1, w0, 0x07060302u);
+  d[1] = __builtin_amdgcn_perm(w1, w0, 0x05040100u);
+}
+__device__ __forceinline__ void wg_pairs_to_words(const unsigned (&d)[2], unsigned& w0, unsigned& w1) {
+  w0 = __builtin_amdgcn_perm(d[0], d[1], 0x05040100u);
+  w1 = __builtin_amdgcn_perm(d[0], d[1], 0x07060302u);
+}
+
+template <int SPLIT, int C, int W, bool APK = false>
 __global__ __launch_bounds__(64 * 2 * (C / 32), 1) void conv3x3_wgrad_resident_kernel(
     const MtrssmConvGeom g, const float* __restrict__ a, const float* __restrict__ src, float* __restrict__ dwp,
     float* __restrict__ part, float* __restrict__ dbias, const int frames_per_wg) {
   static_assert(SPLIT == 1 || SPLIT == 2, "one or two bf16 pieces");
+  static_assert(!APK || SPLIT == 2, "piece words hold two pieces");
   constexpr int NW = 2 * (C / 32), NT = 64 * NW;
   constexpr int RB = 2 * W;
   constexpr int PITCH = wgres_pitch<W>(), COPYB = C * PITCH, XBUFB = wgres_xbuf_bytes<SPLIT, C, W>();
@@ -80,10 +91,15 @@
 #pragma unroll
   for (int j = 0; j < AI; ++j) bsum[j] = 0.f;
   auto stage_a = [&](const float4 v, const int j, const unsigned bufoff, const float keep) __attribute__((always_inline)) {
-    bsum[j] += keep * ((v.x + v.y) + (v.z + v.w));
     unsigned d0[SPLIT], d1[SPLIT];
-    wg_split_pair<SPLIT>(v.x, v.y, d0);
-    wg_split_pair<SPLIT>(v.z, v.w, d1);
+    if constexpr (APK) {
+      wg_words_to_pairs(__builtin_bit_cast(unsigned, v.x), __builtin_bit_cast(unsigned, v.y), d0);
+      wg_words_to_pairs(__builtin_bit_cast(unsigned, v.z), __builtin_bit_cast(unsigned, v.w), d1);
+    } else {
+      bsum[j] += keep * ((v.x + v.y) + (v.z + v.w));
+      wg_split_pair<SPLIT>(v.x, v.y, d0);
+      wg_split_pair<SPLIT>(v.z, v.w, d1);
+    }
 #pragma unroll
     for (int p = 0; p < SPLIT; ++p)
       *reinterpret_cast<uint2*>(lds_a + bufoff + wofs_a + (unsigned)(j * (NT / 16) * kWgresAPitch) + (unsigned)(p * APIECEB)) = make_uint2(d0[p], d1[p]);
@@ -240,7 +256,7 @@
       }
     }
   }
-  if (dbias != nullptr) {
+  if (!APK && dbias != nullptr) {
 #pragma unroll
     for (int j = 0; j < AI; ++j) {
       float v = bsum[j];
@@ -468,7 +484,8 @@
 
 template <int C>
 __device__ __forceinline__ void wgrad_reduce_partials1x1_body(const float4* __restrict__ part, const int S, const int cpad,
-                                                                       float* __restrict__ dwp, float* __restrict__ dbias, const int bx, const int by) {
+                                                                       float* __restrict__ dwp, float* __restrict__ dbias, const int bx, const int by,
+                                                                       float* __restrict__ dbias3 = nullptr) {
   constexpr int NTILE = 2 * (C / 32), KS = 8 / NTILE, TILE4 = 256, SET4 = kWg1x1SetFloats / 4;
   constexpr int NL = 32, NG = 8;
   __shared__ float4 red[NG][NL];
@@ -476,7 +493,9 @@
   const int f = bx * NL + li;
   const bool bias = f >= NTILE * TILE4;
   const int tile = f / TILE4, ft = f - tile * TILE4;
-  const float4* const p = part + (size_t)by * S * SET4 + (bias ? (size_t)(8 * TILE4 + (f - NTILE * TILE4 < 16 ? f - NTILE * TILE4 : 15)) : (size_t)tile * TILE4 + ft);
+  const int fb = f - NTILE * TILE4;
+  const int fb4 = fb < 32 ? (fb < 16 ? fb : 15) : 16 + (fb - 32 < C / 4 ? fb - 32 : C / 4 - 1);
+  const float4* const p = part + (size_t)by * S * SET4 + (bias ? (size_t)(8 * TILE4 + fb4) : (size_t)tile * TILE4 + ft);
   float4 acc4[4];
 #pragma unroll
   for (int u = 0; u < 4; ++u) acc4[u] = make_float4(0.f, 0.f, 0.f, 0.f);
@@ -503,8 +522,11 @@
 #pragma unroll
     for (int k = 1; k < NG; ++k) { v.x += red[k][li].x; v.y += red[k][li].y; v.z += red[k][li].z; v.w += red[k][li].w; }
     if (bias) {
-      if (f - NTILE * TILE4 < 16) {
-        float* const o = dbias + by * 64 + 4 * (f - NTILE * TILE4);
+      if (fb < 16 && dbias != nullptr) {
+        float* const o = dbias + by * 64 + 4 * fb;
+        o[0] += v.x; o[1] += v.y; o[2] += v.z; o[3] += v.w;
+      } else if (fb >= 32 && fb - 32 < C / 4 && dbias3 != nullptr) {
+        float* const o = dbias3 + 4 * (fb - 32);
         o[0] += v.x; o[1] += v.y; o[2] += v.z; o[3] += v.w;
       }
       return;
@@ -524,10 +546,11 @@
 template <int C>
 __host__ __device__ constexpr int bwd1x1_lds_bytes() { return wg1x1_lds_bytes<2, C>() + 2 * 2 * 64 * kWgresAPitch; }
 
-template <int C>
+template <int C, bool PK = false>
 __global__ __launch_bounds__(512, 1) void conv1x1_bwd_fused_kernel(
     const MtrssmConvGeom g, const float* __restrict__ a, const float* __restrict__ src, const unsigned short* __restrict__ wq,
-    float* __restrict__ gh, float* __restrict__ dwp, float* __restrict__ part, float* __restrict__ dbias, const int frames_per_wg) {
+    float* __restrict__ gh, float* __restrict__ dwp, float* __restrict__ part, float* __restrict__ dbias, float* __restrict__ dbias3,
+    const int frames_per_wg) {
   static_assert(C == 64 || C == 128, "mid channels");
   constexpr int SPLIT = 2, NT = 512, P = kWgresAPitch;
   constexpr int XI = C * 16 / NT, AI = 2, NI = XI + AI;
@@ -589,6 +612,9 @@
   const float* const hop = src + (size_t)(bct * 32 + 4 * kl) * 64 + bhalf * 32 + il;
   float* const ghp = gh + (size_t)(bct * 32 + 4 * kl) * 64 + bhalf * 32 + il;
   float opv[2][16];
+  float bs3[PK ? 16 : 1];
+#pragma unroll
+  for (int r = 0; r < (PK ? 16 : 1); ++r) bs3[r] = 0.f;
   auto op_load = [&](const int os, const int n) __attribute__((always_inline)) {
 #pragma unroll
     for (int r = 0; r < 16; ++r) {
@@ -678,12 +704,28 @@
     op_wait(par);
     if (bstore) {
       float* const o = ghp + (size_t)n * (C * 64);
+      float val[16];
 #pragma unroll
       for (int r = 0; r < 16; ++r) {
         const float x = opv[par][r];
         const float e = __expf(x);
         const float neg = act_elu ? e : (act_relu ? 0.f : 1.f);
-        o[((r & 3) + 8 * (r >> 2)) * 64] = accb[r] * (x > 0.f ? 1.f : neg);
+        val[r] = accb[r] * (x > 0.f ? 1.f : neg);
+      }
+      if constexpr (PK) {
+#pragma unroll
+        for (int r = 0; r < 16; r += 2) {
+          bs3[r] = __fadd_rn(bs3[r], val[r]);
+          bs3[r + 1] = __fadd_rn(bs3[r + 1], val[r + 1]);
+          unsigned d[2], w0, w1;
+          wg_split_pair<2>(val[r], val[r + 1], d);
+          wg_pairs_to_words(d, w0, w1);
+          o[((r & 3) + 8 * (r >> 2)) * 64] = __builtin_bit_cast(float, w0);
+          o[(((r + 1) & 3) + 8 * ((r + 1) >> 2)) * 64] = __builtin_bit_cast(float, w1);
+        }
+      } else {
+#pragma unroll
+        for (int r = 0; r < 16; ++r) o[((r & 3) + 8 * (r >> 2)) * 64] = val[r];
       }
     }
   };
@@ -720,8 +762,30 @@
       v += dpp_move<0x140, 0xF>(0.f, v);
       if ((tid & 15) == 0) {
         const int ch = (tid >> 4) + j * 32;
-        if (part) part[(size_t)blockIdx.x * kWg1x1SetFloats + 8 * 1024 + ch] = v;
+        if (part) part[(size_t)blockIdx.x * kWg1x1SetFloats + kWg1x1BiasOff + ch] = v;
         else atomicAdd(&dbias[ch], v);
+      }
+    }
+  }
+  if constexpr (PK) {
+    if (dbias3 != nullptr) {
+      __syncthreads();
+      float* const red3 = reinterpret_cast<float*>(lds);
+#pragma unroll
+      for (int r = 0; r < 16; ++r) {
+        float v = bs3[r];
+        v += dpp_move<0xB1, 0xF>(0.f, v);
+        v += dpp_move<0x4E, 0xF>(0.f, v);
+        v += dpp_move<0x141, 0xF>(0.f, v);
+        v += dpp_move<0x140, 0xF>(0.f, v);
+        v += dpp_move<0x142, 0xA>(0.f, v);
+        if (bstore && il == 16) red3[bhalf * C + bct * 32 + 4 * kl + (r & 3) + 8 * (r >> 2)] = v;
+      }
+      __syncthreads();
+      if (tid < C) {
+        const float v = red3[tid] + red3[C + tid];
+        if (part) part[(size_t)blockIdx.x * kWg1x1SetFloats + kWg1x1Bias3Off + tid] = v;
+        else atomicAdd(&dbias3[tid], v);
       }
     }
   }
```
